# NW-JEFF/Geometric-Message-Passing

Hardware: AMD Instinct MI355X
Metric: edges/sec forward+backward, EGNN & MACE L=2, 1M-edge radius graph, 1/2/4/8 GPU (higher is better)
Workload: dtype f32

## Files before the change

### geometric-message-passing_amd/csrc/gmp_egnn.hip

```cpp
#include <mutex>
#include <set>
#include <tuple>

#include "gmp_egnn_common.h"

namespace gmp {
namespace {

template <int D, int ACT, bool MSG_MEAN, bool SAVE, bool HF, bool POSB>
__global__ __launch_bounds__(fwd_waves<HF>() * 64, fwd_waves<HF>() / 4) void egnn_fwd_kernel(
    int64_t n_nodes, int64_t n_edges, const float* __restrict__ AB, const float* __restrict__ pos,
    const int64_t* __restrict__ rowptr, const int64_t* __restrict__ recv,
    const int64_t* __restrict__ send, gmp_egnn_params P, float eps, int64_t n_waves,
    float* __restrict__ m_aggr, float* __restrict__ pos_aggr, float* __restrict__ xsave,
    float* __restrict__ rsave, int save_planes) {
  constexpr int T = Cfg<D>::T, LDW = Cfg<D>::LDW;
  extern __shared__ __attribute__((aligned(16))) float smem[];
  const float* sW2 = smem;
  const float* sW3 = smem + D * LDW;
  _Float16* hW = reinterpret_cast<_Float16*>(smem + smem_mats_off<D, fwd_waves<HF>(), HF>());
  const _Float16* hW2 = hW;
  const _Float16* hW3 = hW + HCfg<D>::MAT;
  float* sVw = smem + smem_vec_off<D, fwd_waves<HF>(), HF>();
  const float* sV = sVw;
// ... 57 lines not shown
        gemm_h2s<D, false>(hW3, ex3, m, x, li, g);
        r3 = ln_rms<D>(x, eps, ex3 + sw3);
      } else {
        load_vec<D>(x, sV, V_B3, g);
        gemm_wx<D>(sW3, m, x, li, g);
        r3 = ln_normalize<D, false>(x, eps);
      }
      if (SAVE) {
        if (save_planes == 3)
          store_row_w<D, kAuxNT>(rows_window(xsave + 2 * ED, base, ne, D), eoff, x, g);
        store3_w<kAuxNT>(rows_window(rsave, base, ne, 3), (g == 0 && c.valid) ? li * 12u : kOob,
                         r1, r2, r3);
      }
      affine_act<D, ACT>(x, sV, V_LN3W, V_LN3B, g);
      float sp = 0.f;
#pragma unroll
      for (int p = 0; p < T; ++p) {
        const f32x4 w = vec4<D>(sV, V_W4, p, g);
        sp += w[0] * x[p][0] + w[1] * x[p][1] + w[2] * x[p][2] + w[3] * x[p][3];
      }
      s_e = sum_groups(sp) + b4;
    } else if (SAVE) {
      store2_w<kAuxNT>(rows_window(rsave, base, ne, 3), (g == 0 && c.valid) ? li * 12u : kOob, r1,
                       r2);
    }

    const int head = c.valid ? (int)((c.seg0 > base) ? (c.seg0 - base) : 0) : li;
    const bool is_end = c.valid && (c.e == c.seg1 - 1);
    const bool take = (li == 0) && c.valid && (c.i == carry_node);
    float pv[3] = {c.rx * s_e, c.ry * s_e, c.rz * s_e};
    carry_apply<D, POSB>(cbuf, m, pv, take);
    seg_scan<T>(m, li, head);
    if constexpr (POSB) {
      f32x4 pw[1] = {{pv[0], pv[1], pv[2], 0.f}};
      seg_scan<1>(pw, li, head);
      pv[0] = pw[0][0]; pv[1] = pw[0][1]; pv[2] = pw[0][2];
    }
    {
      const float deg = (float)(c.seg1 - c.seg0);
      const float rdeg = HF ? __builtin_amdgcn_rcpf(deg) : 1.f / deg;
      if (MSG_MEAN) {
        const float sc = is_end ? rdeg : 1.f;
#pragma unroll
        for (int p = 0; p < T; ++p) m[p] *= sc;
      }
      const int nn = max(i1 - i0 + 1, 0);
      store_row_w<D, 0>(rows_window(m_aggr, i0, nn, D), is_end ? (unsigned)((c.i - i0) * D * 4) : kOob,
                        m, g);
      if constexpr (POSB)
        store3_w<0>(rows_window(pos_aggr, i0, nn, 3),
                    (is_end && g == 0) ? (unsigned)((c.i - i0) * 12) : kOob,
                    HF ? pv[0] * rdeg : pv[0] / deg, HF ? pv[1] * rdeg : pv[1] / deg,
                    HF ? pv[2] * rdeg : pv[2] / deg);
    }
    if (li == 15) carry_store<D, POSB>(cbuf, m, pv);
    carry_node = __builtin_amdgcn_readlane(c.i, 15);
  }
}

template <int D>
__device__ __forceinline__ void fold_max(unsigned* word, const f32x4 (&x)[D / 16], int lane) {
  float v = 0.f;
#pragma unroll
  for (int p = 0; p < D / 16; ++p)
    v = fmaxf(v, fmaxf(fmaxf(fabsf(x[p][0]), fabsf(x[p][1])), fmaxf(fabsf(x[p][2]), fabsf(x[p][3]))));
  v = fmaxf(v, dpp<0x128>(v));
  v = fmaxf(v, dpp<0x124>(v));
  v = fmaxf(v, dpp<0x122>(v));
  v = fmaxf(v, dpp<0x121>(v));
  v = max_groups(v);
  if (lane == 0) atomicMax(word, __float_as_uint(v));
}

constexpr int NVG = 8;
enum GradVec { G_LN1W = 0, G_LN1B, G_LN2W, G_LN2B, G_LN3W, G_LN3B, G_W4, G_W1D };

template <int D>
__device__ __forceinline__ float slot(const f32x4 (&x)[D / 16], int s) { return x[s >> 2][s & 3]; }
template <int D>
__device__ __forceinline__ float vslot(const float* sV, int v, int s, int g) {
  return sV[v * D + featq(s, g)];
}

template <int D, int ACT, bool MSG_MEAN, bool HF, bool AMAX, int RC, bool POSB, bool GPOS>
__global__ __launch_bounds__(kBwdWaves * 64, 2) void egnn_bwd_kernel(
    int64_t n_nodes, int64_t n_edges, const float* __restrict__ pos,
    const int64_t* __restrict__ rowptr, const int64_t* __restrict__ recv,
    const int64_t* __restrict__ send, gmp_egnn_params P, int64_t n_waves,
    const float* __restrict__ xsave, const float* __restrict__ rsave,
    const float* __restrict__ g_maggr, const float* __restrict__ g_paggr, float* __restrict__ dA,
    float* __restrict__ dpos_recv, float* __restrict__ dpre1_out, float* __restrict__ gdiff_out,
    float* __restrict__ dpre2_out, float* __restrict__ dpre3_out, float* __restrict__ partials,
    unsigned* __restrict__ amax) {
  constexpr int T = Cfg<D>::T, LDW = Cfg<D>::LDW, K = VecAcc<D>::K;
  extern __shared__ __attribute__((aligned(16))) float smem[];
  const float* sW2t = smem;
  const float* sW3t = smem + D * LDW;
  _Float16* hW = reinterpret_cast<_Float16*>(smem + smem_mats_off<D, kBwdWaves, HF>());
  const _Float16* hW2t = hW;
  const _Float16* hW3t = hW + HCfg<D>::MAT;
  float* sVw = smem + smem_vec_off<D, kBwdWaves, HF>();
  const float* sV = sVw;
  constexpr int NMAT = POSB ? 2 : 1;
  if constexpr (HF)
    load_params_hf<D, true, POSB ? 2 : 0, ACT, NMAT>(sVw, hW, smem + smem_carry_off<D, kBwdWaves, HF>(), P);
  else load_params_to_lds<D, true, NMAT>(smem, P);
  __syncthreads();
  const int sw2 = HF ? (int)sV[NV * D] : 0, sw3 = HF ? (int)sV[NV * D + 1] : 0;
  const int ex3 = HF ? (int)sV[NV * D + 3] : 0;
  (void)sW3t; (void)hW3t; (void)sw3; (void)ex3;
  const float* xr1 = xsave;
  const float* xr2 = xsave + (size_t)n_edges * D;
  unsigned* lmx = reinterpret_cast<unsigned*>(const_cast<float*>(sV) + NV * D + 10);
  if (AMAX) {
    if (threadIdx.x < 2) lmx[threadIdx.x] = 0u;
    __syncthreads();
  }

  const int lane = threadIdx.x & 63, li = lane & 15, g = lane >> 4;
  const int wid = __builtin_amdgcn_readfirstlane(threadIdx.x >> 6);
  float* cbuf = smem + smem_carry_off<D, kBwdWaves, HF>() + (wid * 4 + g) * carry_stride<D>();
  carry_clear<D>(smem + smem_carry_off<D, kBwdWaves, HF>() + wid * 4 * carry_stride<D>(), lane);
  const WaveRange wr = wave_range(rowptr, n_nodes, n_edges, n_waves, wid, kBwdWaves);
  zero_isolated<D, GPOS>(wr, rowptr, dA, dpos_recv, lane);
  const float b4 = POSB ? P.b4[0] : 0.f;
  const size_t ED = (size_t)n_edges * D;

  float vacc[NVG][K];
#pragma unroll
  for (int v = 0; v < NVG; ++v)
#pragma unroll
    for (int k = 0; k < K; ++k) vacc[v][k] = 0.f;
  float db4 = 0.f;
  int carry_node = -1;
  EdgeIJ nxt = load_ij(wr.e_lo, li, wr.e_hi, recv, send);
  asm volatile("" ::"v"(nxt.i), "v"(nxt.j));

  for (int base = wr.e_lo; base < wr.e_hi; base += 16) {
    asm volatile("" ::: "memory");
    const EdgeIJ cur = nxt;
    nxt = load_ij(base + 16, li, wr.e_hi, recv, send);
    EdgeCtx c = edge_ctx(cur, base, li, wr.e_hi, (int)n_nodes, rowptr, pos);
    const float rs1 = rsave[3 * (size_t)c.ec + 0];
    const float rs2 = rsave[3 * (size_t)c.ec + 1];
    float rs3 = 0.f, gp0 = 0.f, gp1 = 0.f, gp2 = 0.f;
    f32x4 x[T], xh2[T], z[T];
    if constexpr (POSB) {
      rs3 = rsave[3 * (size_t)c.ec + 2];
      gp0 = g_paggr[3 * c.i + 0], gp1 = g_paggr[3 * c.i + 1], gp2 = g_paggr[3 * c.i + 2];
      if constexpr (RC == 1) load_row<D>(x, rowp(xsave + ED, c.ec, D), g);
      else load_row<D>(z, rowp(xsave + 2 * ED, c.ec, D), g);
    } else {
      load_row<D>(xh2, rowp(g_maggr, c.i, D), g);
    }
    __builtin_amdgcn_sched_barrier(0);
    edge_geom<HF, true>(c);
    const float rstd1 = c.valid ? rs1 : 0.f;
    const float rstd2 = c.valid ? rs2 : 0.f;
    const float rstd3 = c.valid ? rs3 : 0.f;
    if constexpr (POSB && RC == 1) {
      if constexpr (HF) {
        affine_act<D, ACT>(x, sV, V_LN2W, V_LN2B, g);
        load_vec<D>(z, sV, V_B3S, g);
        gemm_h2s_tr<D, false>(hW3t, ex3, x, z, lane, g);
        const float r = ldexpf(rs3, -(ex3 + sw3));
#pragma unroll
        for (int p = 0; p < T; ++p) z[p] *= r;
      } else {
        affine_act<D, ACT>(x, sV, V_LN2W, V_LN2B, g);
        load_vec<D>(z, sV, V_B3, g);
        gemm_wtx<D>(sW3t, x, z, li, g);
        ln_recenter<D>(z, rs3);
      }
    }

    const float inv_deg = c.valid ? 1.f / (float)(c.seg1 - c.seg0) : 0.f;
    const float gscale = MSG_MEAN ? inv_deg : (c.valid ? 1.f : 0.f);
    const float gpx = gp0 * inv_deg;
    const float gpy = gp1 * inv_deg;
    const float gpz = gp2 * inv_deg;
    auto chunk_window = [&](int& ne, int& i0, int& i1, unsigned& eoff) {
      ne = __builtin_amdgcn_readfirstlane(min(16, wr.e_hi - base));
      i0 = __builtin_amdgcn_readfirstlane(c.i);
      i1 = __builtin_amdgcn_readlane(c.i, 15);
      eoff = c.valid ? (unsigned)(li * D * 4) : kOob;
    };
    int ne, i0, i1;
    unsigned eoff;
    float s_e = 0.f;
    if constexpr (!POSB) {
      chunk_window(ne, i0, i1, eoff);
    } else {
      const float ds = gpx * c.rx + gpy * c.ry + gpz * c.rz;
      if (g == 0) db4 += ds;

      float sp = 0.f;
#pragma unroll
      for (int p = 0; p < T; ++p) {
        const f32x4 w3 = vec4<D>(sV, V_LN3W, p, g), b3 = vec4<D>(sV, V_LN3B, p, g);
        const f32x4 w4 = vec4<D>(sV, V_W4, p, g);
#pragma unroll
        for (int q = 0; q < 4; ++q) {
          const float zz = z[p][q] * w3[q] + b3[q];
          sp += w4[q] * act_f<ACT>(zz);
          x[p][q] = ds * w4[q] * act_df<ACT>(zz);
        }
      }
// ... 12 lines not shown
      chunk_window(ne, i0, i1, eoff);
      store_row_w<D, kAuxNT>(rows_window(dpre3_out, base, ne, D), eoff, x, g);
    }

#pragma unroll
    for (int p = 0; p < T; ++p) z[p] = xh2[p] * gscale;
    load_row<D>(xh2, rowp(xr2, c.ec, D), g);
    if constexpr (POSB) {
      if constexpr (HF) gemm_h2<D, true>(hW3t, sw3, 0, x, z, li, g);
      else gemm_wx<D, 2>(sW3t, x, z, li, g);
    }
#pragma unroll
    for (int p = 0; p < T; ++p) {
      const f32x4 w = vec4<D>(sV, V_LN2W, p, g), b = vec4<D>(sV, V_LN2B, p, g);
#pragma unroll
      for (int q = 0; q < 4; ++q) z[p][q] *= act_df<ACT>(xh2[p][q] * w[q] + b[q]);
    }
    accumulate_vec<D>([&](int s) { return slot<D>(z, s) * slot<D>(xh2, s); }, vacc[G_LN2W], li);
    accumulate_vec<D>([&](int s) { return slot<D>(z, s); }, vacc[G_LN2B], li);
#pragma unroll
    for (int p = 0; p < T; ++p) z[p] *= vec4<D>(sV, V_LN2W, p, g);
    ln_backward<D>(z, xh2, rstd2);
    if (AMAX) fold_max<D>(lmx, z, lane);
    store_row_w<D, kAuxNT>(rows_window(dpre2_out, base, ne, D), eoff, z, g);

    load_row<D>(xh2, rowp(xr1, c.ec, D), g);
#pragma unroll
    for (int p = 0; p < T; ++p) x[p] = f32x4{0.f, 0.f, 0.f, 0.f};
    if constexpr (HF) gemm_h2<D, true>(hW2t, sw2, 0, z, x, li, g);
    else gemm_wx<D, 2>(sW2t, z, x, li, g);
#pragma unroll
    for (int p = 0; p < T; ++p) {
      const f32x4 w = vec4<D>(sV, V_LN1W, p, g), b = vec4<D>(sV, V_LN1B, p, g);
#pragma unroll
      for (int q = 0; q < 4; ++q) x[p][q] *= act_df<ACT>(xh2[p][q] * w[q] + b[q]);
    }
    accumulate_vec<D>([&](int s) { return slot<D>(x, s) * slot<D>(xh2, s); }, vacc[G_LN1W], li);
    accumulate_vec<D>([&](int s) { return slot<D>(x, s); }, vacc[G_LN1B], li);
#pragma unroll
    for (int p = 0; p < T; ++p) x[p] *= vec4<D>(sV, V_LN1W, p, g);
    ln_backward<D>(x, xh2, rstd1);
    store_row_w<D, kAuxNT>(rows_window(dpre1_out, base, ne, D), eoff, x, g);

    const float dist = c.dist;
    float gd[3] = {0.f, 0.f, 0.f};
    if constexpr (GPOS) {
      float dd = 0.f;
#pragma unroll
      for (int p = 0; p < T; ++p) {
        const f32x4 w = vec4<D>(sV, V_W1D, p, g);
        dd += w[0] * x[p][0] + w[1] * x[p][1] + w[2] * x[p][2] + w[3] * x[p][3];
      }
      dd = sum_groups(dd);
      accumulate_vec<D>([&](int s) { return slot<D>(x, s) * dist; }, vacc[G_W1D], li);

      const float rinv = (c.dist > 0.f) ? dd / c.dist : 0.f;
      if constexpr (POSB) {
        gd[0] = gpx * s_e + rinv * c.rx;
        gd[1] = gpy * s_e + rinv * c.ry;
        gd[2] = gpz * s_e + rinv * c.rz;
      } else {
        gd[0] = rinv * c.rx;
        gd[1] = rinv * c.ry;
        gd[2] = rinv * c.rz;
      }
      store3_w<kAuxNT>(rows_window(gdiff_out, base, ne, 3), (c.valid && g == 0) ? li * 12u : kOob,
                       gd[0], gd[1], gd[2]);
    } else {
      accumulate_vec<D>([&](int s) { return slot<D>(x, s) * dist; }, vacc[G_W1D], li);
    }

    const int head = c.valid ? (int)((c.seg0 > base) ? (c.seg0 - base) : 0) : li;
    const bool is_end = c.valid && (c.e == c.seg1 - 1);
    const bool take = (li == 0) && c.valid && (c.i == carry_node);
    carry_apply<D, GPOS>(cbuf, x, gd, take);
    seg_scan<T>(x, li, head);
    if constexpr (GPOS) {
      f32x4 pw[1] = {{gd[0], gd[1], gd[2], 0.f}};
      seg_scan<1>(pw, li, head);
      gd[0] = pw[0][0]; gd[1] = pw[0][1]; gd[2] = pw[0][2];
    }
    {
      const int nn = max(i1 - i0 + 1, 0);
      store_row_w<D, 0>(rows_window(dA, i0, nn, D), is_end ? (unsigned)((c.i - i0) * D * 4) : kOob,
                        x, g);
      if constexpr (GPOS)
        store3_w<0>(rows_window(dpos_recv, i0, nn, 3),
                    (is_end && g == 0) ? (unsigned)((c.i - i0) * 12) : kOob, gd[0], gd[1], gd[2]);
    }
    if (li == 15) carry_store<D, GPOS>(cbuf, x, gd);
    carry_node = __builtin_amdgcn_readlane(c.i, 15);
  }

  __syncthreads();
  if (AMAX && threadIdx.x == 0 && ((POSB && GPOS) || amax)) {
    atomicMax(&amax[0], lmx[0]);
    if (POSB) atomicMax(&amax[1], lmx[1]);
  }
  __syncthreads();
  float* red = smem;
  constexpr int RW = NVG * D + 1;
  for (int t = lane; t < RW; t += 64) red[wid * RW + t] = 0.f;
  __syncthreads();
  if (acc_owner<D>(li)) {
#pragma unroll
    for (int v = 0; v < NVG; ++v)
#pragma unroll
      for (int k = 0; k < K; ++k) red[wid * RW + v * D + featq(acc_slot<D>(li, k), g)] = vacc[v][k];
  }
  float t4 = db4;
#pragma unroll
  for (int off = 32; off >= 1; off >>= 1) t4 += __shfl_xor(t4, off);
  if (lane == 0) red[wid * RW + NVG * D] = t4;
  __syncthreads();
  for (int t = threadIdx.x; t < RW; t += blockDim.x) {
    float sacc = 0.f;
    for (int w = 0; w < kBwdWaves; ++w) sacc += red[w * RW + t];
    partials[(int64_t)blockIdx.x * RW + t] = sacc;
  }
}

int64_t n_waves_for(int64_t n_edges, int nwb) {
  int64_t w = ceil_div(n_edges, 128);
  const int64_t cap = (int64_t)device_cu_count() * nwb;
  if (w > cap) w = cap;
  if (w < 1) w = 1;
  return ceil_div(w, nwb) * nwb;
}

template <int D, int ACT, bool MEAN, bool POSB>
int launch_fwd(int64_t N, int64_t E, const float* AB, const float* pos, const int64_t* rowptr,
               const int64_t* recv, const int64_t* send, const gmp_egnn_params& P, float eps,
               float* m_aggr, float* pos_aggr, float* xsave, int save_planes, float* rsave,
               hipStream_t s) {
  const bool hf = !egnn_f32();
  const int nwb = hf ? fwd_waves<true>() : fwd_waves<false>();
  const int64_t W = n_waves_for(E, nwb);
  constexpr int NMAT = POSB ? 2 : 1;
  const size_t smem = hf ? smem_total<D, fwd_waves<true>(), true, NMAT>()
                         : smem_total<D, fwd_waves<false>(), false, NMAT>();
  auto k = rsave ? (hf ? egnn_fwd_kernel<D, ACT, MEAN, true, true, POSB>
                       : egnn_fwd_kernel<D, ACT, MEAN, true, false, POSB>)
                 : (hf ? egnn_fwd_kernel<D, ACT, MEAN, false, true, POSB>
                       : egnn_fwd_kernel<D, ACT, MEAN, false, false, POSB>);
  int rc = prep_kernel(k, smem);
  if (rc) return rc;
  k<<<(unsigned)(W / nwb), nwb * 64, smem, s>>>(N, E, AB, pos, rowptr, recv, send, P,
                                                           eps, W, m_aggr, pos_aggr, xsave, rsave,
                                                           save_planes);
  return launch_status();
}

template <int D, int ACT, bool MEAN, bool POSB, bool GPOS>
int launch_bwd(int64_t N, int64_t E, const float* pos, const int64_t* rowptr,
               const int64_t* recv, const int64_t* send, const gmp_egnn_params& P,
               const float* xsave, int save_planes, const float* rsave, const float* gm,
               const float* gp, float* dA, float* dpos_recv, float* dpre1, float* gdiff,
               float* dpre2, float* dpre3, float* partials, unsigned* amax, hipStream_t s) {
  const int64_t W = n_waves_for(E, kBwdWaves);
  const bool hf = !egnn_f32();
  constexpr int NMAT = POSB ? 2 : 1;
  constexpr bool FULL = POSB && GPOS;
  constexpr int RC0 = POSB ? 0 : 1;
  const size_t smem = hf ? smem_total<D, kBwdWaves, true, NMAT>()
                         : smem_total<D, kBwdWaves, false, NMAT>();
  const bool ax = !FULL || amax;
#define LAUNCH_BWD_K(RC)                                                              \
  (hf ? (ax ? egnn_bwd_kernel<D, ACT, MEAN, true, true, RC, POSB, GPOS>              \
            : egnn_bwd_kernel<D, ACT, MEAN, true, !FULL, RC, POSB, GPOS>)            \
      : (ax ? egnn_bwd_kernel<D, ACT, MEAN, false, true, RC, POSB, GPOS>             \
            : egnn_bwd_kernel<D, ACT, MEAN, false, !FULL, RC, POSB, GPOS>))
  auto k = save_planes == 3 ? LAUNCH_BWD_K(RC0) : LAUNCH_BWD_K(1);
#undef LAUNCH_BWD_K
  int rc = prep_kernel(k, smem);
  if (rc) return rc;
  k<<<(unsigned)(W / kBwdWaves), kBwdWaves * 64, smem, s>>>(N, E, pos, rowptr, recv, send, P, W,
                                                           xsave, rsave, gm, gp, dA, dpos_recv,
                                                           dpre1, gdiff, dpre2, dpre3, partials,
                                                           amax);
  return launch_status();
}

bool params_ok(const gmp_egnn_params* P) {
  return P && P->w1d && P->b1 && P->ln1_w && P->ln1_b && P->W2 && P->b2 && P->ln2_w &&
         P->ln2_b && P->W3 && P->b3 && P->ln3_w && P->ln3_b && P->w4 && P->b4;
}

}

int prep_kernel_once(const void* k, size_t smem) {
  static std::mutex mu;
  static std::set<std::tuple<int, const void*, size_t>> done;
  int dev = 0;
  if (hipGetDevice(&dev) != hipSuccess) return GMP_ERR_HIP;
  std::lock_guard<std::mutex> lk(mu);
  if (done.count({dev, k, smem})) return GMP_OK;
  const int rc = hip_check(hipFuncSetAttribute(k, hipFuncAttributeMaxDynamicSharedMemorySize,
                                               (int)smem));
  if (!rc) done.insert({dev, k, smem});
  return rc;
}

int g_egnn_f32 = 0;

bool egnn_f32() { return g_egnn_f32 == 1; }

}

using namespace gmp;

#define LAUNCH_EGNN_DISPATCH(CALL)                                                                \
  do {                                                                                         \
    if (d == 128) {                                                                            \
      if (act == 0) { if (msg_mean) CALL(128, 0, true); else CALL(128, 0, false); }            \
      else          { if (msg_mean) CALL(128, 1, true); else CALL(128, 1, false); }            \
    } else if (d == 64) {                                                                      \
      if (act == 0) { if (msg_mean) CALL(64, 0, true); else CALL(64, 0, false); }              \
      else          { if (msg_mean) CALL(64, 1, true); else CALL(64, 1, false); }              \
    } else {                                                                                   \
      if (act == 0) { if (msg_mean) CALL(32, 0, true); else CALL(32, 0, false); }              \
      else          { if (msg_mean) CALL(32, 1, true); else CALL(32, 1, false); }              \
    }                                                                                          \
  } while (0)

extern "C" {

int gmp_egnn_set_f32_mfma(int on) {
  const int prev = egnn_f32() ? 1 : 0;
  g_egnn_f32 = on ? 1 : 0;
  return prev;
}

int gmp_egnn_edge_fwd_ex_f32(int64_t n_nodes, int64_t n_edges, int64_t d, const float* AB,
                             const float* pos, const int64_t* rowptr, const int64_t* recv,
                             const int64_t* send, const gmp_egnn_params* params, int act,
                             int msg_mean, float ln_eps, float* m_aggr, float* pos_aggr,
                             float* save_xhat, int save_planes, float* save_rstd, uint32_t flags,
                             void* stream) {
  if (!(d == 32 || d == 64 || d == 128)) return GMP_ERR_UNSUPPORTED;
  GMP_CHECK_ARG((flags & ~(uint32_t)GMP_EGNN_NO_POS_BRANCH) == 0);
  const bool posb = !(flags & GMP_EGNN_NO_POS_BRANCH);
  GMP_CHECK_ARG(n_nodes >= 0 && n_edges >= 0 && (act == 0 || act == 1));
  GMP_CHECK_ARG(n_nodes < INT32_MAX && n_edges < INT32_MAX);
  GMP_CHECK_ARG(params_ok(params) && m_aggr && (pos_aggr || !posb) && rowptr);
  GMP_CHECK_ARG((save_rstd == nullptr) == (save_xhat == nullptr));
  GMP_CHECK_ARG(save_xhat == nullptr || save_planes == 2 || save_planes == 3);
  hipStream_t s = as_stream(stream);
  if (n_nodes == 0) return GMP_OK;
  int rc = GMP_OK;
  if (n_edges == 0) {
    rc = hip_check(hipMemsetAsync(m_aggr, 0, n_nodes * d * sizeof(float), s));
    if (!rc && posb) rc = hip_check(hipMemsetAsync(pos_aggr, 0, n_nodes * 3 * sizeof(float), s));
    return rc;
  }
  GMP_CHECK_ARG(AB && pos && recv && send && aligned16(AB) && aligned16(m_aggr));
  GMP_CHECK_ARG(aligned16(params->W2) && aligned16(params->W3));
  GMP_CHECK_ARG(save_xhat == nullptr || aligned16(save_xhat));
#define LAUNCH_CALL_FWD(DD, AA, MM)                                                              \
  rc = posb ? launch_fwd<DD, AA, MM, true>(n_nodes, n_edges, AB, pos, rowptr, recv, send,      \
                                           *params, ln_eps, m_aggr, pos_aggr, save_xhat,        \
                                           save_planes, save_rstd, s)                           \
            : launch_fwd<DD, AA, MM, false>(n_nodes, n_edges, AB, pos, rowptr, recv, send,     \
                                            *params, ln_eps, m_aggr, pos_aggr, save_xhat,       \
                                            save_planes, save_rstd, s)
  LAUNCH_EGNN_DISPATCH(LAUNCH_CALL_FWD);
#undef LAUNCH_CALL_FWD
  return rc;
}

int gmp_egnn_edge_fwd_f32(int64_t n_nodes, int64_t n_edges, int64_t d, const float* AB,
                          const float* pos, const int64_t* rowptr, const int64_t* recv,
                          const int64_t* send, const gmp_egnn_params* params, int act,
                          int msg_mean, float ln_eps, float* m_aggr, float* pos_aggr,
                          float* save_xhat, int save_planes, float* save_rstd, void* stream) {
  return gmp_egnn_edge_fwd_ex_f32(n_nodes, n_edges, d, AB, pos, rowptr, recv, send, params, act,
                                  msg_mean, ln_eps, m_aggr, pos_aggr, save_xhat, save_planes,
                                  save_rstd, 0u, stream);
}

int64_t gmp_egnn_edge_bwd_partials_rows(int64_t n_edges, int64_t d) {
  (void)d;
  return n_waves_for(n_edges, kBwdWaves) / kBwdWaves;
}

int gmp_egnn_edge_bwd_ex_f32(int64_t n_nodes, int64_t n_edges, int64_t d, const float* pos,
                             const int64_t* rowptr, const int64_t* recv, const int64_t* send,
                             const gmp_egnn_params* params, int act, int msg_mean,
                             const float* save_xhat, int save_planes, const float* save_rstd,
                             const float* g_m_aggr, const float* g_pos_aggr, float* dA,
                             float* dpos_recv, float* dpre1, float* gdiff, float* dpre2,
                             float* dpre3, float* vec_partials, uint32_t* amax, uint32_t flags,
                             void* stream) {
  if (!(d == 32 || d == 64 || d == 128)) return GMP_ERR_UNSUPPORTED;
  GMP_CHECK_ARG((flags & ~(uint32_t)(GMP_EGNN_NO_POS_BRANCH | GMP_EGNN_NO_POS_GRAD)) == 0);
  const bool posb = !(flags & GMP_EGNN_NO_POS_BRANCH), gpos = !(flags & GMP_EGNN_NO_POS_GRAD);
  GMP_CHECK_ARG(n_nodes >= 0 && n_edges >= 0 && (act == 0 || act == 1));
  GMP_CHECK_ARG(n_nodes < INT32_MAX && n_edges < INT32_MAX);
  GMP_CHECK_ARG(params_ok(params) && dA && (dpos_recv || !gpos) && rowptr && vec_partials);
  GMP_CHECK_ARG(save_planes == 2 || save_planes == 3);
  hipStream_t s = as_stream(stream);
  int rc = GMP_OK;
  if (n_nodes > 0 && n_edges == 0) {
    rc = hip_check(hipMemsetAsync(dA, 0, n_nodes * d * sizeof(float), s));
    if (!rc && gpos) rc = hip_check(hipMemsetAsync(dpos_recv, 0, n_nodes * 3 * sizeof(float), s));
  }
  if (rc) return rc;
  if (n_edges == 0 || n_nodes == 0) {
    return hip_check(hipMemsetAsync(
        vec_partials, 0,
        gmp_egnn_edge_bwd_partials_rows(n_edges, d) * (8 * d + 1) * sizeof(float), s));
  }
  GMP_CHECK_ARG(pos && recv && send && save_xhat && save_rstd && g_m_aggr && dpre1 && dpre2);
  GMP_CHECK_ARG(!posb || (g_pos_aggr && dpre3));
  GMP_CHECK_ARG(!gpos || gdiff);
  GMP_CHECK_ARG(aligned16(save_xhat) && aligned16(dA) && aligned16(g_m_aggr) &&
                aligned16(dpre1) && aligned16(dpre2) && (!posb || aligned16(dpre3)));
  GMP_CHECK_ARG(aligned16(params->W2) && aligned16(params->W3));
#define LAUNCH_BWD_V(DD, AA, MM, PB, GP)                                                        \
  launch_bwd<DD, AA, MM, PB, GP>(n_nodes, n_edges, pos, rowptr, recv, send, *params, save_xhat, \
                                 save_planes, save_rstd, g_m_aggr, g_pos_aggr, dA, dpos_recv,   \
                                 dpre1, gdiff, dpre2, dpre3, vec_partials, amax, s)
#define LAUNCH_CALL_BWD(DD, AA, MM)                                                              \
  rc = posb ? (gpos ? LAUNCH_BWD_V(DD, AA, MM, true, true) : LAUNCH_BWD_V(DD, AA, MM, true, false)) \
            : (gpos ? LAUNCH_BWD_V(DD, AA, MM, false, true)                                     \
                    : LAUNCH_BWD_V(DD, AA, MM, false, false))
  LAUNCH_EGNN_DISPATCH(LAUNCH_CALL_BWD);
#undef LAUNCH_CALL_BWD
#undef LAUNCH_BWD_V
  return rc;
}

int gmp_egnn_edge_bwd_amax_f32(int64_t n_nodes, int64_t n_edges, int64_t d, const float* pos,
                               const int64_t* rowptr, const int64_t* recv, const int64_t* send,
                               const gmp_egnn_params* params, int act, int msg_mean,
                               const float* save_xhat, int save_planes, const float* save_rstd,
                               const float* g_m_aggr, const float* g_pos_aggr, float* dA,
                               float* dpos_recv, float* dpre1, float* gdiff, float* dpre2,
                               float* dpre3, float* vec_partials, uint32_t* amax, void* stream) {
  return gmp_egnn_edge_bwd_ex_f32(n_nodes, n_edges, d, pos, rowptr, recv, send, params, act,
                                  msg_mean, save_xhat, save_planes, save_rstd, g_m_aggr,
                                  g_pos_aggr, dA, dpos_recv, dpre1, gdiff, dpre2, dpre3,
                                  vec_partials, amax, 0u, stream);
}

int gmp_egnn_edge_bwd_f32(int64_t n_nodes, int64_t n_edges, int64_t d, const float* pos,
                          const int64_t* rowptr, const int64_t* recv, const int64_t* send,
                          const gmp_egnn_params* params, int act, int msg_mean,
                          const float* save_xhat, int save_planes, const float* save_rstd,
                          const float* g_m_aggr, const float* g_pos_aggr, float* dA,
                          float* dpos_recv, float* dpre1, float* gdiff, float* dpre2, float* dpre3,
                          float* vec_partials, void* stream) {
  return gmp_egnn_edge_bwd_amax_f32(n_nodes, n_edges, d, pos, rowptr, recv, send, params, act,
                                    msg_mean, save_xhat, save_planes, save_rstd, g_m_aggr,
                                    g_pos_aggr, dA, dpos_recv, dpre1, gdiff, dpre2, dpre3,
                                    vec_partials, nullptr, stream);
}

}
```

### geometric-message-passing_amd/csrc/gmp_egnn_common.h

```cpp
#pragma once
#include <stdlib.h>

#include "gmp_common.h"

namespace gmp {

typedef float f32x4 __attribute__((ext_vector_type(4)));

constexpr int kFwdWaves = 12;
template <bool HF>
constexpr int fwd_waves() { return kFwdWaves; }
constexpr int kBwdWaves = 8;

template <int D>
struct Cfg {
  static constexpr int T = D / 16;
  static constexpr int N = D / 4;
  static constexpr int LDW = D + 4;
};

__device__ __forceinline__ constexpr int featq(int s, int g) { return 16 * (s >> 2) + 4 * g + (s & 3); }

enum VecId {
  V_W1D = 0, V_B1, V_LN1W, V_LN1B, V_B2, V_LN2W, V_LN2B, V_B3, V_LN3W, V_LN3B, V_W4, NVB,
// ... 119 lines not shown
  if (threadIdx.x >= 2 * D + 64 && threadIdx.x < 2 * D + 128) {
    unsigned a = 0u, b = 0u, c = 0u, e = 0u;
    for (int k = threadIdx.x - 2 * D - 64; k < D; k += 64) {
      a = max(a, __float_as_uint(fabsf(P.ln1_w[k])));
      b = max(b, __float_as_uint(fabsf(P.ln1_b[k])));
      c = max(c, __float_as_uint(fabsf(P.ln2_w[k])));
      e = max(e, __float_as_uint(fabsf(P.ln2_b[k])));
    }
    atomicMax(&mxw[2], a);
    atomicMax(&mxw[3], b);
    atomicMax(&mxw[4], c);
    atomicMax(&mxw[5], e);
  }
  __syncthreads();
  const int s2 = scale_exp(__uint_as_float(mxw[0])), s3 = scale_exp(__uint_as_float(mxw[1]));
  const float rd = sqrtf((float)D);
  const int ex2 = clamp_in_exp(scale_exp(rd * __uint_as_float(mxw[2]) + __uint_as_float(mxw[3])), s2);
  const int ex3 = clamp_in_exp(scale_exp(rd * __uint_as_float(mxw[4]) + __uint_as_float(mxw[5])), s3);
  __syncthreads();
#pragma unroll 8
  for (int i = threadIdx.x; i < NMAT * D * D; i += blockDim.x) {
    const int mat = i / (D * D), e = i - mat * D * D;
    const int o = e / D, k = e - o * D;
    const float w = ldexpf((mat ? P.W3 : P.W2)[e] - scratch[mat * D + k], mat ? s3 : s2);
    const int r = TRANSPOSE ? k : o, c = TRANSPOSE ? o : k;
    const _Float16 hi = (_Float16)w;
    _Float16* dst = hW + mat * H::MAT + r * H::LDH + hf_pos(c);
    dst[0] = hi;
    dst[H::PLANE] = (_Float16)(w - (float)hi);
  }
  const float* vsrc[NVB] = {P.w1d, P.b1, P.ln1_w, P.ln1_b, P.b2, P.ln2_w,
                            P.ln2_b, P.b3, P.ln3_w, P.ln3_b, P.w4};
  for (int i = threadIdx.x; i < NVB * D; i += blockDim.x) sV[i] = vsrc[i / D][i % D];
  for (int k = threadIdx.x; k < D; k += blockDim.x) {
    sV[V_B2S * D + k] = ldexpf(P.b2[k] - scratch[2 * D], ex2 + s2);
    sV[V_B3S * D + k] = ldexpf(P.b3[k] - scratch[2 * D + 1], ex3 + s3);
    const int e1 = ACT == GMP_ACT_RELU ? ex2 : 0;
    sV[V_LN1WS * D + k] = ldexpf(P.ln1_w[k], e1);
    sV[V_LN1BS * D + k] = ldexpf(P.ln1_b[k], e1);
  }
  if (threadIdx.x == 0) {
    sV[NV * D + 0] = (float)s2;
    sV[NV * D + 1] = (float)s3;
    sV[NV * D + 2] = (float)ex2;
    sV[NV * D + 3] = (float)ex3;
  }
}

template <int D>
__device__ __forceinline__ f32x4 vec4(const float* sV, int v, int p, int g) {
  return *reinterpret_cast<const f32x4*>(sV + v * D + 16 * p + 4 * g);
}

template <int D>
__device__ __forceinline__ void load_vec(f32x4 (&x)[D / 16], const float* sV, int v, int g) {
#pragma unroll
  for (int p = 0; p < D / 16; ++p) x[p] = vec4<D>(sV, v, p, g);
}

template <int D>
__device__ __forceinline__ void load_row(f32x4 (&x)[D / 16], const float* __restrict__ row, int g) {
#pragma unroll
  for (int p = 0; p < D / 16; ++p) x[p] = *reinterpret_cast<const f32x4*>(row + 16 * p + 4 * g);
}
template <int D>
__device__ __forceinline__ void store_row(float* __restrict__ row, const f32x4 (&x)[D / 16], int g) {
#pragma unroll
  for (int p = 0; p < D / 16; ++p) *reinterpret_cast<f32x4*>(row + 16 * p + 4 * g) = x[p];
}
template <int D>
__device__ __forceinline__ void stream_row(float* __restrict__ row, const f32x4 (&x)[D / 16], int g) {
#pragma unroll
  for (int p = 0; p < D / 16; ++p)
    __builtin_nontemporal_store(x[p], reinterpret_cast<f32x4*>(row + 16 * p + 4 * g));
}

typedef __amdgpu_buffer_rsrc_t rsrc_t;
constexpr unsigned kOob = 0x40000000u;
constexpr int kAuxNT = 2;

__device__ __forceinline__ rsrc_t rows_window(const float* base, int r0, int n, int ld) {
  return __builtin_amdgcn_make_buffer_rsrc(const_cast<float*>(base) + (size_t)(unsigned)r0 * ld, 0,
                                           n * ld * 4, 0x00020000);
}
template <int D, int AUX>
__device__ __forceinline__ void store_row_w(rsrc_t w, unsigned off, const f32x4 (&x)[D / 16], int g) {
#pragma unroll
  for (int p = 0; p < D / 16; ++p)
    __builtin_amdgcn_raw_buffer_store_b128(__builtin_bit_cast(__attribute__((ext_vector_type(4))) unsigned, x[p]),
                                           w, off + (16 * p + 4 * g) * 4, 0, AUX);
}
template <int AUX>
__device__ __forceinline__ void store2_w(rsrc_t w, unsigned off, float a, float b) {
  __builtin_amdgcn_raw_buffer_store_b32(__float_as_uint(a), w, off, 0, AUX);
  __builtin_amdgcn_raw_buffer_store_b32(__float_as_uint(b), w, off + 4, 0, AUX);
}
template <int AUX>
__device__ __forceinline__ void store3_w(rsrc_t w, unsigned off, float a, float b, float c) {
  __builtin_amdgcn_raw_buffer_store_b32(__float_as_uint(a), w, off, 0, AUX);
  __builtin_amdgcn_raw_buffer_store_b32(__float_as_uint(b), w, off + 4, 0, AUX);
  __builtin_amdgcn_raw_buffer_store_b32(__float_as_uint(c), w, off + 8, 0, AUX);
}

__device__ __forceinline__ void gemm_fence() { __builtin_amdgcn_sched_barrier(0); }
template <int D, int SPLIT = 1>
__device__ __forceinline__ void gemm_wx(const float* __restrict__ sW, const f32x4 (&x)[D / 16],
                                        f32x4 (&y)[D / 16], int i, int g) {
  constexpr int T = Cfg<D>::T, LDW = Cfg<D>::LDW;
  constexpr int TS = (T % SPLIT == 0) ? T / SPLIT : T;
#pragma unroll
  for (int p = 0; p < T; ++p) {
#pragma unroll
    for (int t0 = 0; t0 < T; t0 += TS) {
      f32x4 a[TS];
#pragma unroll
      for (int t = 0; t < TS; ++t)
        a[t] = *reinterpret_cast<const f32x4*>(sW + (16 * (t0 + t) + i) * LDW + 16 * p + 4 * g);
#pragma unroll
      for (int c = 0; c < 4; ++c)
#pragma unroll
        for (int t = 0; t < TS; ++t)
          y[t0 + t] = __builtin_amdgcn_mfma_f32_16x16x4f32(a[t][c], x[p][c], y[t0 + t], 0, 0, 0);
      gemm_fence();
    }
  }
}

typedef _Float16 h16x8 __attribute__((ext_vector_type(8)));
typedef _Float16 h16x2 __attribute__((ext_vector_type(2)));
typedef unsigned u32x4 __attribute__((ext_vector_type(4)));
constexpr int kTilesPerFence = 2;

__device__ __forceinline__ void split8(const f32x4& a, const f32x4& b, h16x8& bh, h16x8& bl) {
  const h16x2 p0 = {(_Float16)a[0], (_Float16)a[1]}, p1 = {(_Float16)a[2], (_Float16)a[3]};
  const h16x2 p2 = {(_Float16)b[0], (_Float16)b[1]}, p3 = {(_Float16)b[2], (_Float16)b[3]};
  const unsigned u0 = __builtin_bit_cast(unsigned, p0), u1 = __builtin_bit_cast(unsigned, p1);
  const unsigned u2 = __builtin_bit_cast(unsigned, p2), u3 = __builtin_bit_cast(unsigned, p3);
  unsigned l0, l1, l2, l3;
  const float one = 1.0f;
  asm("v_fma_mixlo_f16 %0, %4, %16, -%12 op_sel_hi:[0,0,1]\n\t"
      "v_fma_mixhi_f16 %0, %5, %16, -%12 op_sel:[0,0,1] op_sel_hi:[0,0,1]\n\t"
      "v_fma_mixlo_f16 %1, %6, %16, -%13 op_sel_hi:[0,0,1]\n\t"
      "v_fma_mixhi_f16 %1, %7, %16, -%13 op_sel:[0,0,1] op_sel_hi:[0,0,1]\n\t"
      "v_fma_mixlo_f16 %2, %8, %16, -%14 op_sel_hi:[0,0,1]\n\t"
      "v_fma_mixhi_f16 %2, %9, %16, -%14 op_sel:[0,0,1] op_sel_hi:[0,0,1]\n\t"
      "v_fma_mixlo_f16 %3, %10, %16, -%15 op_sel_hi:[0,0,1]\n\t"
      "v_fma_mixhi_f16 %3, %11, %16, -%15 op_sel:[0,0,1] op_sel_hi:[0,0,1]\n\t"
      "s_nop 1"
      : "=&v"(l0), "=&v"(l1), "=&v"(l2), "=&v"(l3)
      : "v"(a[0]), "v"(a[1]), "v"(a[2]), "v"(a[3]), "v"(b[0]), "v"(b[1]), "v"(b[2]), "v"(b[3]),
        "v"(u0), "v"(u1), "v"(u2), "v"(u3), "s"(one));
  bh = __builtin_bit_cast(h16x8, (u32x4){u0, u1, u2, u3});
  bl = __builtin_bit_cast(h16x8, (u32x4){l0, l1, l2, l3});
}

__device__ __forceinline__ float max_groups(float v) {
  const auto a = __builtin_amdgcn_permlane16_swap(__float_as_uint(v), __float_as_uint(v), false,
                                                  false);
  v = fmaxf(__uint_as_float(a[0]), __uint_as_float(a[1]));
  const auto b = __builtin_amdgcn_permlane32_swap(__float_as_uint(v), __float_as_uint(v), false,
                                                  false);
  return fmaxf(__uint_as_float(b[0]), __uint_as_float(b[1]));
}

template <int D, bool DYN>
__device__ __forceinline__ void gemm_h2(const _Float16* __restrict__ hW, int sw, int sx_static,
// ... 363 lines not shown
  r.i = reinterpret_cast<const int*>(recv)[2 * ec];
  r.j = reinterpret_cast<const int*>(send)[2 * ec];
  return r;
}

__device__ __forceinline__ EdgeCtx edge_ctx(EdgeIJ ij, int base, int lane_e, int e_hi,
                                            int n_nodes, const int64_t* __restrict__ rowptr,
                                            const float* __restrict__ pos) {
  EdgeCtx c;
  c.e = base + lane_e;
  c.ec = clamp_edge(c.e, e_hi);
  c.valid = c.e < e_hi;
  c.i = ((unsigned)ij.i < (unsigned)n_nodes) ? ij.i : 0;
  c.j = ((unsigned)ij.j < (unsigned)n_nodes) ? ij.j : c.i;
  const int* rp = reinterpret_cast<const int*>(rowptr);
  c.seg0 = rp[2 * c.i];
  c.seg1 = rp[2 * c.i + 2];
  c.rx = pos[3 * c.i + 0];
  c.ry = pos[3 * c.i + 1];
  c.rz = pos[3 * c.i + 2];
  c.dist = 0.f;
  c.pjx = pos[3 * c.j + 0];
  c.pjy = pos[3 * c.j + 1];
  c.pjz = pos[3 * c.j + 2];
  return c;
}
template <bool FAST = false, bool BWD = false>
__device__ __forceinline__ void edge_geom(EdgeCtx& c) {
#pragma clang fp contract(off)
  c.rx -= c.pjx;
  c.ry -= c.pjy;
  c.rz -= c.pjz;
  const float xx = c.rx * c.rx, yy = c.ry * c.ry, zz = c.rz * c.rz;
  const float q = BWD ? __builtin_fmaf(c.ry, c.ry, xx) + zz : __builtin_fmaf(c.rz, c.rz, xx + yy);
  c.dist = FAST ? __builtin_amdgcn_sqrtf(q) : sqrtf(q);
}

template <int D, bool FAST, class Ctx>
__device__ __forceinline__ void load_pre1(f32x4 (&x)[D / 16], const float* arow, const float* brow,
                                          const float* sV, Ctx& c, int g) {
  f32x4 b[D / 16];
#pragma unroll
  for (int p = 0; p < D / 16; ++p) {
    x[p] = *reinterpret_cast<const f32x4*>(arow + 16 * p + 4 * g);
    b[p] = *reinterpret_cast<const f32x4*>(brow + 16 * p + 4 * g);
  }
  __builtin_amdgcn_sched_barrier(0);
  edge_geom<FAST>(c);
  const float dist = c.dist;
#pragma unroll
  for (int p = 0; p < D / 16; ++p)
    x[p] = (x[p] + b[p]) + (vec4<D>(sV, V_W1D, p, g) * dist + vec4<D>(sV, V_B1, p, g));
}

__device__ __forceinline__ const float* rowp(const float* base, int r, int ld) {
  return base + (size_t)(unsigned)r * (size_t)ld;
}
__device__ __forceinline__ float* rowp(float* base, int r, int ld) {
  return base + (size_t)(unsigned)r * (size_t)ld;
}

struct WaveRange {
  int e_lo, e_hi, n_lo, n_hi;
};
__device__ __forceinline__ WaveRange wave_range(const int64_t* __restrict__ rowptr, int64_t n_nodes,
                                                int64_t n_edges, int64_t n_waves, int wid,
                                                int nwb) {
  const int64_t wave = (int64_t)blockIdx.x * nwb + wid;
  const int64_t nb = node_begin(rowptr, n_nodes, n_edges, wave, n_waves);
  const int64_t ne = node_begin(rowptr, n_nodes, n_edges, wave + 1, n_waves);
  WaveRange r;
  r.e_lo = (nb < ne) ? (int)rowptr[nb] : 0;
  r.e_hi = (nb < ne) ? (int)rowptr[ne] : 0;
  r.e_lo = __builtin_amdgcn_readfirstlane(r.e_lo);
  r.e_hi = __builtin_amdgcn_readfirstlane(r.e_hi);
  r.n_lo = __builtin_amdgcn_readfirstlane((int)nb);
  r.n_hi = __builtin_amdgcn_readfirstlane((int)ne);
  return r;
}

template <int D, bool R3 = true>
__device__ __forceinline__ void zero_isolated(const WaveRange& wr, const int64_t* __restrict__ rowptr,
                                              float* __restrict__ rows, float* __restrict__ rows3,
                                              int lane) {
  const int* rp = reinterpret_cast<const int*>(rowptr);
  for (int n = wr.n_lo + lane; n < wr.n_hi; n += 64) {
    if (rp[2 * n] == rp[2 * n + 2]) {
      float4* r = reinterpret_cast<float4*>(rows + (size_t)n * D);
#pragma unroll
      for (int k = 0; k < D / 4; ++k) r[k] = float4{0.f, 0.f, 0.f, 0.f};
      if (R3) {
        rows3[3 * (size_t)n] = 0.f;
        rows3[3 * (size_t)n + 1] = 0.f;
        rows3[3 * (size_t)n + 2] = 0.f;
      }
    }
  }
}


bool egnn_f32();

int prep_kernel_once(const void* k, size_t smem);
template <class K>
inline int prep_kernel(K k, size_t smem) {
  return prep_kernel_once((const void*)k, smem);
}

inline bool aligned16(const void* p) { return reinterpret_cast<uintptr_t>(p) % 16 == 0; }

}
```

### geometric-message-passing_amd/csrc/gmp_index.hip

```cpp
#include <hipcub/hipcub.hpp>

#include <map>
#include <mutex>
#include <utility>

#include "gmp_common.h"

namespace gmp {

thread_local int g_last_hip_error = 0;

int device_cu_count() {
  static int cus = 0;
  if (cus == 0) {
    int dev = 0;
    hipDeviceProp_t prop;
    if (hipGetDevice(&dev) == hipSuccess && hipGetDeviceProperties(&prop, dev) == hipSuccess)
      cus = prop.multiProcessorCount;
    if (cus <= 0) cus = 256;
  }
  return cus;
}

namespace {

constexpr size_t kAlign = 256;
inline size_t align_up(size_t x) { return (x + kAlign - 1) / kAlign * kAlign; }

int key_bits(int64_t n_seg) {
  int b = 1;
  while ((int64_t(1) << b) <= n_seg) ++b;
  return b;
}

size_t cub_sort_bytes(int64_t n) {
  size_t bytes = 0;
  (void)hipcub::DeviceRadixSort::SortPairs(nullptr, bytes, (const uint32_t*)nullptr, (uint32_t*)nullptr,
                                     (const uint32_t*)nullptr, (uint32_t*)nullptr, (int)n, 0, 32,
                                     (hipStream_t)0);
  return bytes;
}

__global__ void csr_prepare_keys(const int64_t* __restrict__ index, int64_t n, int64_t n_seg,
                                 uint32_t* __restrict__ keys, uint32_t* __restrict__ vals,
                                 int32_t* __restrict__ err_flag) {
  for (int64_t i = blockIdx.x * (int64_t)blockDim.x + threadIdx.x; i < n;
       i += (int64_t)gridDim.x * blockDim.x) {
    int64_t k = index[i];
    bool ok = (k >= 0) && (k < n_seg);
    if (!ok && err_flag) *err_flag = 1;
    keys[i] = ok ? (uint32_t)k : (uint32_t)n_seg;
    vals[i] = (uint32_t)i;
  }
}

__global__ void csr_finish(const uint32_t* __restrict__ keys_sorted,
                           const uint32_t* __restrict__ vals_sorted, int64_t n, int64_t n_seg,
                           const int64_t* __restrict__ payload, int64_t* __restrict__ perm,
                           int64_t* __restrict__ rowptr, int64_t* __restrict__ index_sorted,
                           int64_t* __restrict__ payload_out) {
  for (int64_t k = blockIdx.x * (int64_t)blockDim.x + threadIdx.x; k <= n;
       k += (int64_t)gridDim.x * blockDim.x) {
    int64_t prev = (k == 0) ? -1 : (int64_t)keys_sorted[k - 1];
    int64_t cur = (k == n) ? n_seg : (int64_t)keys_sorted[k];
    for (int64_t s = prev + 1; s <= cur && s <= n_seg; ++s) rowptr[s] = k;
    if (k < n) {
      int64_t p = vals_sorted[k];
      if (perm) perm[k] = p;
      if (index_sorted) index_sorted[k] = (cur < n_seg) ? cur : -1;
      if (payload_out) payload_out[k] = payload[p];
    }
  }
}

template <int VEC>
__global__ void gather_rows_kernel(const float* __restrict__ src, int64_t n_rows, int64_t F,
                                   const int64_t* __restrict__ index, int64_t n_index,
                                   float* __restrict__ out, int32_t* __restrict__ err_flag) {
  const int64_t fv = F / VEC;
  const int64_t total = n_index * fv;
  for (int64_t t = blockIdx.x * (int64_t)blockDim.x + threadIdx.x; t < total;
       t += (int64_t)gridDim.x * blockDim.x) {
    int64_t e = t / fv, c = t - e * fv;
    int64_t r = index[e];
    if constexpr (VEC == 4) {
      float4 v = make_float4(0.f, 0.f, 0.f, 0.f);
      if (r >= 0 && r < n_rows) v = reinterpret_cast<const float4*>(src + r * F)[c];
      else if (err_flag) *err_flag = 1;
      reinterpret_cast<float4*>(out + e * F)[c] = v;
    } else {
      float v = 0.f;
      if (r >= 0 && r < n_rows) v = src[r * F + c];
      else if (err_flag) *err_flag = 1;
      out[e * F + c] = v;
    }
  }
}

struct RedVal {
  float v;
  int64_t arg;
};

template <int REDUCE>
__device__ __forceinline__ void red_combine(float& acc, int64_t& arg, float x, int64_t xa) {
  if (REDUCE == GMP_REDUCE_MAX) {
    if (x > acc || (x == acc && xa < arg)) { acc = x; arg = xa; }
  } else {
    acc += x;
  }
}

template <int VEC, int REDUCE>
__device__ __forceinline__ void wave_reduce_rows(const float* __restrict__ src, int64_t F,
                                                 const int64_t* __restrict__ perm, int64_t k_beg,
                                                 int64_t k_end, int64_t n_items, int64_t c,
                                                 int lpr, float (&acc)[VEC], int64_t (&arg)[VEC]) {
  const int lane = threadIdx.x & 63;
  const int R = 64 / lpr, sub = lane / lpr;
#pragma unroll
  for (int v = 0; v < VEC; ++v) {
    acc[v] = (REDUCE == GMP_REDUCE_MAX) ? -INFINITY : 0.f;
    arg[v] = n_items;
  }
  const bool active = c < F / VEC;
  int64_t k = k_beg + sub;
  for (; k + 3 * R < k_end; k += 4 * R) {
    int64_t it[4];
    float x[4][VEC];
#pragma unroll
    for (int u = 0; u < 4; ++u) it[u] = perm ? perm[k + u * R] : (k + u * R);
#pragma unroll
    for (int u = 0; u < 4; ++u) {
      const float* p = src + it[u] * F + c * VEC;
      if (!active) {
#pragma unroll
        for (int v = 0; v < VEC; ++v) x[u][v] = 0.f;
      } else if constexpr (VEC == 4) {
        float4 q = *reinterpret_cast<const float4*>(p);
        x[u][0] = q.x; x[u][1] = q.y; x[u][2] = q.z; x[u][3] = q.w;
      } else if constexpr (VEC == 2) {
        float2 q = *reinterpret_cast<const float2*>(p);
        x[u][0] = q.x; x[u][1] = q.y;
      } else {
        x[u][0] = p[0];
      }
    }
#pragma unroll
    for (int u = 0; u < 4; ++u)
#pragma unroll
      for (int v = 0; v < VEC; ++v) red_combine<REDUCE>(acc[v], arg[v], x[u][v], it[u]);
  }
  for (; k < k_end; k += R) {
    const int64_t i = perm ? perm[k] : k;
    if (active) {
      const float* p = src + i * F + c * VEC;
#pragma unroll
      for (int v = 0; v < VEC; ++v) red_combine<REDUCE>(acc[v], arg[v], p[v], i);
    }
  }
  for (int m = lpr; m < 64; m <<= 1) {
#pragma unroll
    for (int v = 0; v < VEC; ++v) {
      const float ox = __shfl_xor(acc[v], m);
      const int64_t oa = __shfl_xor(arg[v], m);
      if (REDUCE == GMP_REDUCE_MAX) {
        if (ox > acc[v] || (ox == acc[v] && oa < arg[v])) { acc[v] = ox; arg[v] = oa; }
      } else {
        const bool upper = (lane & m) != 0;
        acc[v] = upper ? ox + acc[v] : acc[v] + ox;
      }
    }
  }
}

__device__ __forceinline__ int lanes_per_row(int64_t cpr) {
  int l = 1;
  while (l < cpr && l < 64) l <<= 1;
  return l;
}

template <int VEC, int REDUCE>
__global__ __launch_bounds__(256) void segment_reduce_wave(
    const float* __restrict__ src, int64_t n_items, int64_t F, const int64_t* __restrict__ perm,
    const int64_t* __restrict__ rowptr, int64_t n_seg, float* __restrict__ out,
    int64_t* __restrict__ argmax) {
  const int lane = threadIdx.x & 63;
  const int64_t seg = blockIdx.x * (int64_t)(blockDim.x / 64) + (threadIdx.x >> 6);
  if (seg >= n_seg) return;
  const int64_t k0 = rowptr[seg], k1 = rowptr[seg + 1];
  const int64_t cpr = F / VEC;
  const int lpr = lanes_per_row(cpr);
  for (int64_t cb = 0; cb < cpr; cb += 64) {
    const int64_t c = cb + lane % lpr;
    float acc[VEC];
    int64_t arg[VEC];
    wave_reduce_rows<VEC, REDUCE>(src, F, perm, k0, k1, n_items, c, lpr, acc, arg);
    const int64_t cnt = k1 - k0;
    if (lane < lpr && c < cpr) {
#pragma unroll
      for (int v = 0; v < VEC; ++v) {
        float r = acc[v];
        if (REDUCE == GMP_REDUCE_MEAN) r = r / (float)(cnt > 0 ? cnt : 1);
        if (REDUCE == GMP_REDUCE_MAX && cnt == 0) r = 0.f;
        out[seg * F + c * VEC + v] = r;
        if (REDUCE == GMP_REDUCE_MAX && argmax) argmax[seg * F + c * VEC + v] = arg[v];
      }
    }
  }
}

template <int VEC, int REDUCE>
__global__ __launch_bounds__(256) void segment_reduce_split(
    const float* __restrict__ src, int64_t n_items, int64_t F, const int64_t* __restrict__ perm,
    const int64_t* __restrict__ rowptr, int64_t n_seg, int64_t S, float* __restrict__ partial) {
  __shared__ float red[4][256];
  const int lane = threadIdx.x & 63, w = threadIdx.x >> 6;
  const int64_t seg = blockIdx.x / S, part = blockIdx.x % S;
  const int64_t k0 = rowptr[seg], k1 = rowptr[seg + 1], len = k1 - k0;
  const int64_t pb = k0 + len * part / S, pe = k0 + len * (part + 1) / S;
  const int64_t wb = pb + (pe - pb) * w / 4, we = pb + (pe - pb) * (w + 1) / 4;
  const int64_t cpr = F / VEC;
  const int lpr = lanes_per_row(cpr);
  for (int64_t cb = 0; cb < cpr; cb += 64) {
    const int64_t c = cb + lane % lpr;
    float acc[VEC];
    int64_t arg[VEC];
    wave_reduce_rows<VEC, REDUCE>(src, F, perm, wb, we, n_items, c, lpr, acc, arg);
    if (lane < lpr) {
#pragma unroll
      for (int v = 0; v < VEC; ++v) red[w][lane * VEC + v] = acc[v];
    }
    __syncthreads();
    if (w == 0 && lane < lpr && c < cpr) {
#pragma unroll
      for (int v = 0; v < VEC; ++v) {
        const float t = ((red[0][lane * VEC + v] + red[1][lane * VEC + v]) + red[2][lane * VEC + v]) +
                        red[3][lane * VEC + v];
        partial[(seg * S + part) * F + c * VEC + v] = t;
      }
    }
    __syncthreads();
  }
}

template <int REDUCE>
__global__ void segment_split_finish(const float* __restrict__ partial, const int64_t* __restrict__ rowptr,
                                     int64_t n_seg, int64_t S, int64_t F, float* __restrict__ out) {
  for (int64_t t = blockIdx.x * (int64_t)blockDim.x + threadIdx.x; t < n_seg * F;
       t += (int64_t)gridDim.x * blockDim.x) {
    const int64_t seg = t / F, f = t - seg * F;
    float s = 0.f;
    for (int64_t p = 0; p < S; ++p) s += partial[(seg * S + p) * F + f];
    if (REDUCE == GMP_REDUCE_MEAN) {
      const int64_t cnt = rowptr[seg + 1] - rowptr[seg];
      s = s / (float)(cnt > 0 ? cnt : 1);
    }
    out[t] = s;
  }
}

template <int REDUCE>
// ... 83 lines not shown

using namespace gmp;

extern "C" {

int gmp_abi_version(void) { return GMP_ABI_VERSION; }

const char* gmp_error_string(int code) {
  switch (code) {
    case GMP_OK: return "ok";
    case GMP_ERR_ARG: return "invalid argument";
    case GMP_ERR_HIP: return "HIP runtime error";
    case GMP_ERR_UNSUPPORTED: return "unsupported shape for this kernel";
    case GMP_ERR_WORKSPACE: return "workspace too small";
    default: return "unknown error";
  }
}

int gmp_last_hip_error(void) { return g_last_hip_error; }

size_t gmp_csr_workspace_size(int64_t n_items, int64_t n_seg) {
  (void)n_seg;
  if (n_items <= 0) return kAlign;
  size_t n = (size_t)n_items;
  return 4 * align_up(n * sizeof(uint32_t)) + align_up(cub_sort_bytes(n_items)) + kAlign;
}

int gmp_csr_build(const int64_t* index, int64_t n_items, int64_t n_seg, const int64_t* payload,
                  int64_t* perm, int64_t* rowptr, int64_t* index_sorted, int64_t* payload_out,
                  int32_t* err_flag, void* workspace, size_t workspace_bytes, void* stream) {
  GMP_CHECK_ARG(n_items >= 0 && n_seg >= 0 && rowptr != nullptr);
  GMP_CHECK_ARG(n_items < (int64_t(1) << 31) && n_seg < (int64_t(1) << 31) - 1);
  GMP_CHECK_ARG(n_items == 0 || index != nullptr);
  GMP_CHECK_ARG(payload_out == nullptr || payload != nullptr);
  hipStream_t s = as_stream(stream);
  if (n_items == 0) {
    int rc = hip_check(hipMemsetAsync(rowptr, 0, (n_seg + 1) * sizeof(int64_t), s));
    return rc;
  }
  if (workspace_bytes < gmp_csr_workspace_size(n_items, n_seg) || workspace == nullptr)
    return GMP_ERR_WORKSPACE;
  char* ws = reinterpret_cast<char*>(
      (reinterpret_cast<uintptr_t>(workspace) + kAlign - 1) / kAlign * kAlign);
  size_t nb = align_up((size_t)n_items * sizeof(uint32_t));
  uint32_t* keys_in = reinterpret_cast<uint32_t*>(ws);
  uint32_t* keys_out = reinterpret_cast<uint32_t*>(ws + nb);
  uint32_t* vals_in = reinterpret_cast<uint32_t*>(ws + 2 * nb);
  uint32_t* vals_out = reinterpret_cast<uint32_t*>(ws + 3 * nb);
  void* temp = ws + 4 * nb;
  size_t temp_bytes = cub_sort_bytes(n_items);

  csr_prepare_keys<<<grid_for(n_items, 256), 256, 0, s>>>(index, n_items, n_seg, keys_in, vals_in,
                                                          err_flag);
  int rc = launch_status();
  if (rc) return rc;
  rc = hip_check(hipcub::DeviceRadixSort::SortPairs(temp, temp_bytes, keys_in, keys_out, vals_in,
                                                    vals_out, (int)n_items, 0, key_bits(n_seg), s));
  if (rc) return rc;
  csr_finish<<<grid_for(n_items + 1, 256), 256, 0, s>>>(keys_out, vals_out, n_items, n_seg,
                                                        payload, perm, rowptr, index_sorted,
                                                        payload_out);
  return launch_status();
}

int gmp_gather_rows_f32(const float* src, int64_t n_rows, int64_t F, const int64_t* index,
                        int64_t n_index, float* out, int32_t* err_flag, void* stream) {
  GMP_CHECK_ARG(n_rows >= 0 && F >= 0 && n_index >= 0);
  if (n_index == 0 || F == 0) return GMP_OK;
  GMP_CHECK_ARG(src && index && out);
  hipStream_t s = as_stream(stream);
  bool v4 = (F % 4 == 0) && (reinterpret_cast<uintptr_t>(src) % 16 == 0) &&
            (reinterpret_cast<uintptr_t>(out) % 16 == 0);
  if (v4) {
    gather_rows_kernel<4><<<grid_for(n_index * F / 4, 256), 256, 0, s>>>(src, n_rows, F, index,
                                                                         n_index, out, err_flag);
  } else {
    gather_rows_kernel<1><<<grid_for(n_index * F, 256), 256, 0, s>>>(src, n_rows, F, index,
                                                                     n_index, out, err_flag);
  }
  return launch_status();
}

static int64_t split_parts(int64_t n_items, int64_t n_seg, int reduce) {
  if (reduce == GMP_REDUCE_MAX || n_seg <= 0) return 1;
  const int64_t avg = n_items / n_seg;
  int64_t S = avg < 2048 ? 1 : ceil_div(avg, 1024);
  if (n_seg < 2048 && n_items >= 16384)
    S = std::max<int64_t>(S, std::min<int64_t>(ceil_div(2048, n_seg), 64));
  return S > 4096 ? 4096 : S;
}

size_t gmp_segment_reduce_workspace_size(int64_t n_items, int64_t n_seg, int64_t F, int reduce) {
  const int64_t S = split_parts(n_items, n_seg, reduce);
  return S > 1 ? (size_t)(n_seg * S * F) * sizeof(float) : 0;
}

int gmp_segment_reduce_f32(const float* src, int64_t n_items, int64_t F, const int64_t* perm,
                           const int64_t* rowptr, int64_t n_seg, int reduce, float* out,
                           int64_t* argmax, void* workspace, size_t workspace_bytes,
                           void* stream) {
  GMP_CHECK_ARG(n_items >= 0 && F >= 0 && n_seg >= 0);
  GMP_CHECK_ARG(reduce == GMP_REDUCE_SUM || reduce == GMP_REDUCE_MEAN || reduce == GMP_REDUCE_MAX);
  if (n_seg == 0 || F == 0) return GMP_OK;
  GMP_CHECK_ARG(rowptr && out && (n_items == 0 || src));
  hipStream_t s = as_stream(stream);
  const bool a16 = (reinterpret_cast<uintptr_t>(src) % 16 == 0);
  const bool a8 = (reinterpret_cast<uintptr_t>(src) % 8 == 0);
  const int vec = (F % 4 == 0 && a16) ? 4 : (F % 2 == 0 && a8) ? 2 : 1;
  const int64_t S = split_parts(n_items, n_seg, reduce);
  if (S > 1 && workspace && workspace_bytes >= gmp_segment_reduce_workspace_size(n_items, n_seg, F, reduce)) {
    float* part = reinterpret_cast<float*>(workspace);
    const unsigned g = (unsigned)(n_seg * S);
#define LAUNCH_SPLIT(V, RED) segment_reduce_split<V, RED><<<g, 256, 0, s>>>(src, n_items, F, perm, rowptr, n_seg, S, part)
    if (reduce == GMP_REDUCE_SUM) {
      if (vec == 4) LAUNCH_SPLIT(4, GMP_REDUCE_SUM); else if (vec == 2) LAUNCH_SPLIT(2, GMP_REDUCE_SUM); else LAUNCH_SPLIT(1, GMP_REDUCE_SUM);
    } else {
      if (vec == 4) LAUNCH_SPLIT(4, GMP_REDUCE_MEAN); else if (vec == 2) LAUNCH_SPLIT(2, GMP_REDUCE_MEAN); else LAUNCH_SPLIT(1, GMP_REDUCE_MEAN);
    }
#undef LAUNCH_SPLIT
    int rc = launch_status();
    if (rc) return rc;
    if (reduce == GMP_REDUCE_SUM)
      segment_split_finish<GMP_REDUCE_SUM><<<grid_for(n_seg * F, 256), 256, 0, s>>>(part, rowptr, n_seg, S, F, out);
    else
      segment_split_finish<GMP_REDUCE_MEAN><<<grid_for(n_seg * F, 256), 256, 0, s>>>(part, rowptr, n_seg, S, F, out);
    return launch_status();
  }
#define LAUNCH_SEG_LAUNCH(VEC, RED)                                                            \
  segment_reduce_wave<VEC, RED><<<(unsigned)ceil_div(n_seg, 4), 256, 0, s>>>(              \
      src, n_items, F, perm, rowptr, n_seg, out, argmax)
#define LAUNCH_SEG_DISPATCH(RED)                                                               \
  do {                                                                                      \
    if (F < 4 && n_items < 64 * n_seg)                                                      \
      segment_reduce_thread<RED><<<grid_for(n_seg * F, 256), 256, 0, s>>>(                 \
          src, n_items, F, perm, rowptr, n_seg, out, argmax);                               \
    else if (vec == 4) LAUNCH_SEG_LAUNCH(4, RED);                                              \
    else if (vec == 2) LAUNCH_SEG_LAUNCH(2, RED);                                              \
    else LAUNCH_SEG_LAUNCH(1, RED);                                                            \
  } while (0)
  if (reduce == GMP_REDUCE_SUM) LAUNCH_SEG_DISPATCH(GMP_REDUCE_SUM);
  else if (reduce == GMP_REDUCE_MEAN) LAUNCH_SEG_DISPATCH(GMP_REDUCE_MEAN);
  else LAUNCH_SEG_DISPATCH(GMP_REDUCE_MAX);
#undef LAUNCH_SEG_DISPATCH
#undef LAUNCH_SEG_LAUNCH
  return launch_status();
}

int gmp_segment_reduce_bwd_f32(const float* grad_out, int64_t n_seg, int64_t F,
                               const int64_t* index, int64_t n_items, const int64_t* rowptr,
                               int reduce, const int64_t* argmax, float* grad_src, void* stream) {
  GMP_CHECK_ARG(n_items >= 0 && F >= 0 && n_seg >= 0);
  GMP_CHECK_ARG(reduce == GMP_REDUCE_SUM || reduce == GMP_REDUCE_MEAN || reduce == GMP_REDUCE_MAX);
  if (n_items == 0 || F == 0) return GMP_OK;
  GMP_CHECK_ARG(grad_out && index && grad_src);
  GMP_CHECK_ARG(reduce != GMP_REDUCE_MEAN || rowptr);
  GMP_CHECK_ARG(reduce != GMP_REDUCE_MAX || argmax);
  hipStream_t s = as_stream(stream);
  const bool vec4 = reduce != GMP_REDUCE_MAX && F % 4 == 0 && n_items * F / 4 < INT32_MAX &&
                    n_seg < INT32_MAX && reinterpret_cast<uintptr_t>(grad_out) % 16 == 0 &&
                    reinterpret_cast<uintptr_t>(grad_src) % 16 == 0;
  if (vec4) {
    const int total = (int)(n_items * F / 4);
    const int gv = grid_for(total, 256);
    auto go = reinterpret_cast<const float4*>(grad_out);
    auto gs = reinterpret_cast<float4*>(grad_src);
    if (reduce == GMP_REDUCE_SUM)
      segment_reduce_bwd_vec4_kernel<GMP_REDUCE_SUM><<<gv, 256, 0, s>>>(go, (int)n_seg, (int)(F / 4),
                                                                        index, total, rowptr, gs);
    else
      segment_reduce_bwd_vec4_kernel<GMP_REDUCE_MEAN><<<gv, 256, 0, s>>>(go, (int)n_seg, (int)(F / 4),
                                                                         index, total, rowptr, gs);
    return launch_status();
  }
  int g = grid_for(n_items * F, 256);
  if (reduce == GMP_REDUCE_SUM)
    segment_reduce_bwd_kernel<GMP_REDUCE_SUM><<<g, 256, 0, s>>>(grad_out, n_seg, F, index, n_items,
                                                                rowptr, argmax, grad_src);
  else if (reduce == GMP_REDUCE_MEAN)
    segment_reduce_bwd_kernel<GMP_REDUCE_MEAN><<<g, 256, 0, s>>>(grad_out, n_seg, F, index,
                                                                 n_items, rowptr, argmax, grad_src);
  else
    segment_reduce_bwd_kernel<GMP_REDUCE_MAX><<<g, 256, 0, s>>>(grad_out, n_seg, F, index, n_items,
                                                                rowptr, argmax, grad_src);
  return launch_status();
}

}
```

### geometric-message-passing_amd/csrc/torch/gmp_torch.cpp

```cpp
#include <ATen/hip/impl/HIPGuardImplMasqueradingAsCUDA.h>
#include <ATen/hip/impl/HIPStreamMasqueradingAsCUDA.h>
#include <ATen/ATen.h>
#include <torch/library.h>

#include <algorithm>
#include <string>
#include <vector>

#include "../../../include/gmp.h"

namespace {

using at::Tensor;
using c10::optional;

thread_local int g_op_device = -1;

struct OpGuard {
  c10::hip::HIPGuardMasqueradingAsCUDA guard;
  int prev;
  static c10::Device dev_of(const Tensor& t, const char* op) {
    TORCH_CHECK(t.defined() && t.is_cuda(), "gmp.", op,
                ": inputs must be HIP device tensors (no CPU fallback)");
    return t.device();
// ... 192 lines not shown
      P[l].W1n = w1->data_ptr<float>();
      P[l].ld1 = w1->stride(0);
    }
  }
  const size_t bytes = gmp_egnn_node_image_bytes(d);
  TORCH_CHECK(bytes > 0, "gmp.egnn_node_image: d must be 32, 64 or 128");
  Tensor img = at::empty({L, (int64_t)bytes}, W0s[0].options().dtype(at::kByte));
  check_rc(gmp_egnn_node_image_f32(d, L, P.data(), img.data_ptr(), cur_stream()),
           "gmp_egnn_node_image_f32");
  return img;
}

std::tuple<Tensor, Tensor, Tensor, Tensor> egnn_node_fwd(
    const Tensor& h, const Tensor& m_aggr, const std::vector<Tensor>& vecs, const Tensor& image,
    bool with_ab, int64_t act, bool residual, double eps, bool train) {
  OpGuard g(h, "egnn_node_fwd");
  f32(h, "h");
  f32(m_aggr, "m_aggr");
  TORCH_CHECK(h.dim() == 2 && m_aggr.sizes() == h.sizes(), "gmp.egnn_node_fwd: h, m_aggr (N, d)");
  const int64_t N = h.size(0), d = h.size(1);
  TORCH_CHECK(vecs.size() == 6, "gmp.egnn_node_fwd: 6 parameter vectors expected");
  for (int k = 0; k < 6; ++k) {
    f32(vecs[k], "egnn_node parameter");
    numel(vecs[k], d, "egnn_node parameter");
  }
  TORCH_CHECK(image.scalar_type() == at::kByte && image.is_contiguous() &&
                  image.numel() == (int64_t)gmp_egnn_node_image_bytes(d) &&
                  image.device() == h.device(),
              "gmp.egnn_node_fwd: image must be one layer's row of egnn_node_image");
  gmp_egnn_node_params P{};
  P.b0 = fp(vecs[0]); P.ln1_w = fp(vecs[1]); P.ln1_b = fp(vecs[2]);
  P.b3 = fp(vecs[3]); P.ln2_w = fp(vecs[4]); P.ln2_b = fp(vecs[5]);
  Tensor ho = at::empty({N, d}, h.options());
  Tensor abo = at::empty({with_ab ? N : 0, 2 * d}, h.options());
  Tensor xh = at::empty({train ? 2 : 0, N, d}, h.options());
  Tensor rs = at::empty({train ? 2 : 0, N}, h.options());
  check_rc(gmp_egnn_node_fwd_f32(N, d, fp(h), fp(m_aggr), &P, image.data_ptr(), (int)act,
                                 residual ? 1 : 0, (float)eps, fp(ho),
                                 with_ab ? fp(abo) : nullptr, train ? fp(xh) : nullptr,
                                 train ? fp(rs) : nullptr, cur_stream()),
           "gmp_egnn_node_fwd_f32");
  return {ho, abo, xh, rs};
}

void egnn_graph_checks(const Tensor& pos, const Tensor& rowptr, const Tensor& recv,
                       const Tensor& send) {
  f32(pos, "pos");
  i64(rowptr, "rowptr");
  i64(recv, "recv");
  i64(send, "send");
  TORCH_CHECK(pos.dim() == 2 && pos.size(1) == 3, "gmp.egnn: pos must be (N, 3)");
  numel(rowptr, pos.size(0) + 1, "rowptr");
  numel(send, recv.numel(), "send");
}

std::tuple<Tensor, Tensor, Tensor, Tensor> egnn_edge_fwd(
    const Tensor& AB, const Tensor& pos, const Tensor& rowptr, const Tensor& recv,
    const Tensor& send, const std::vector<Tensor>& params, int64_t act, bool msg_mean, double eps,
    bool train, int64_t xhat_planes, bool need_pos) {
  OpGuard g(AB, "egnn_edge_fwd");
  TORCH_CHECK(xhat_planes == 2 || xhat_planes == 3, "gmp.egnn_edge_fwd: xhat_planes is 2 or 3");
  f32(AB, "AB");
  egnn_graph_checks(pos, rowptr, recv, send);
  TORCH_CHECK(AB.dim() == 2 && AB.size(1) % 2 == 0 && AB.size(0) == pos.size(0),
              "gmp.egnn_edge_fwd: AB must be (N, 2d)");
  const int64_t N = pos.size(0), E = recv.numel(), d = AB.size(1) / 2;
  gmp_egnn_params P = egnn_params(params, d);
  Tensor m = at::empty({N, d}, fopt(AB)), pa = at::empty({need_pos ? N : 0, 3}, fopt(AB));
  Tensor xh = at::empty({train ? xhat_planes : 0, E, d}, fopt(AB));
  Tensor rs = at::empty({train ? E : 0, 3}, fopt(AB));
  check_rc(gmp_egnn_edge_fwd_ex_f32(N, E, d, fp(AB), fp(pos), ip(rowptr), ip(recv), ip(send), &P,
                                    (int)act, msg_mean, (float)eps, fp(m),
                                    need_pos ? fp(pa) : nullptr, train ? fp(xh) : nullptr,
                                    (int)xhat_planes, train ? fp(rs) : nullptr,
                                    need_pos ? 0u : GMP_EGNN_NO_POS_BRANCH, cur_stream()),
           "gmp_egnn_edge_fwd_ex_f32");
  return {m, pa, xh, rs};
}

std::tuple<Tensor, Tensor, Tensor, Tensor, Tensor, Tensor, Tensor> egnn_edge_bwd(
    const Tensor& pos, const Tensor& rowptr, const Tensor& recv, const Tensor& send,
    const std::vector<Tensor>& params, int64_t act, bool msg_mean, const Tensor& xhat,
    const Tensor& rstd, const Tensor& g_m, const Tensor& g_p, const optional<Tensor>& amax,
    bool pos_branch, bool pos_grad) {
  OpGuard g(pos, "egnn_edge_bwd");
  egnn_graph_checks(pos, rowptr, recv, send);
  f32(xhat, "xhat");
  f32(rstd, "rstd");
  f32(g_m, "g_m_aggr");
  f32(g_p, "g_pos_aggr");
  TORCH_CHECK(xhat.dim() == 3 && (xhat.size(0) == 2 || xhat.size(0) == 3),
              "gmp.egnn_edge_bwd: xhat must be the forward's (2 or 3, E, d) planes");
  const int64_t N = pos.size(0), E = recv.numel(), d = xhat.size(2);
  shape(xhat, {xhat.size(0), E, d}, "xhat");
  shape(rstd, {E, 3}, "rstd");
  shape(g_m, {N, d}, "g_m_aggr");
  if (pos_branch) shape(g_p, {N, 3}, "g_pos_aggr");
  gmp_egnn_params P = egnn_params(params, d);
  if (amax.has_value()) {
    i32(*amax, "amax");
    TORCH_CHECK(amax->numel() >= 2, "gmp.egnn_edge_bwd: amax has 2 words");
  }
  auto o = fopt(pos);
  Tensor dA = at::empty({N, d}, o), dpr = at::empty({pos_grad ? N : 0, 3}, o);
  Tensor dp1 = at::empty({E, d}, o), gd = at::empty({pos_grad ? E : 0, 3}, o);
  Tensor dp2 = at::empty({E, d}, o), dp3 = at::empty({pos_branch ? E : 0, d}, o);
  Tensor part = at::empty({gmp_egnn_edge_bwd_partials_rows(E, d), 8 * d + 1}, o);
  check_rc(gmp_egnn_edge_bwd_ex_f32(
               N, E, d, fp(pos), ip(rowptr), ip(recv), ip(send), &P, (int)act, msg_mean,
               E > 0 ? fp(xhat) : nullptr, (int)xhat.size(0), fp(rstd), fp(g_m),
               pos_branch ? fp(g_p) : nullptr, fp(dA), pos_grad ? fp(dpr) : nullptr, fp(dp1),
               pos_grad ? fp(gd) : nullptr, fp(dp2), pos_branch ? fp(dp3) : nullptr, fp(part),
               amax.has_value() ? reinterpret_cast<uint32_t*>(amax->data_ptr<int32_t>())
                                : nullptr,
               (pos_branch ? 0u : GMP_EGNN_NO_POS_BRANCH) | (pos_grad ? 0u : GMP_EGNN_NO_POS_GRAD),
               cur_stream()),
           "gmp_egnn_edge_bwd_ex_f32");
  return {dA, dpr, dp1, gd, dp2, dp3, part};
}

Tensor cfconv_aggregate(const Tensor& x, const Tensor& xidx, const Tensor& w, const Tensor& perm,
                        const Tensor& rowptr, int64_t n_seg, const optional<Tensor>& escale) {
  OpGuard g(x, "cfconv_aggregate");
  f32(x, "x");
  f32(w, "w");
  i64(xidx, "xidx");
  i64(perm, "perm");
  i64(rowptr, "rowptr");
  TORCH_CHECK(x.dim() == 2 && w.dim() == 2 && w.size(1) == x.size(1),
              "gmp.cfconv_aggregate: x (N, F), w (E, F)");
  const int64_t E = w.size(0);
  numel(xidx, E, "xidx");
  numel(perm, E, "perm");
  numel(rowptr, n_seg + 1, "rowptr");
  opt_f32(escale, {E}, "escale");
  Tensor out = at::empty({n_seg, x.size(1)}, x.options());
  Tensor err = at::zeros({1}, x.options().dtype(at::kInt));
  check_rc(gmp_cfconv_aggregate_scaled_f32(fp(x), x.size(0), ip(xidx), fp(w), cfp(escale), E,
                                           x.size(1), ip(perm), ip(rowptr), n_seg, fp(out),
                                           err.data_ptr<int32_t>(), cur_stream()),
           "gmp_cfconv_aggregate_scaled_f32");
  return out;
}

Tensor cfconv_wgrad(const Tensor& gr, const Tensor& gidx, const Tensor& x, const Tensor& xidx,
                    const optional<Tensor>& escale) {
  OpGuard g(gr, "cfconv_wgrad");
  f32(gr, "g");
  f32(x, "x");
  i64(gidx, "gidx");
  i64(xidx, "xidx");
  TORCH_CHECK(gr.dim() == 2 && x.dim() == 2 && gr.size(1) == x.size(1),
              "gmp.cfconv_wgrad: g (N, F), x (N, F)");
  const int64_t E = gidx.numel();
  numel(xidx, E, "xidx");
  opt_f32(escale, {E}, "escale");
  Tensor dw = at::empty({E, x.size(1)}, x.options());
  Tensor err = at::zeros({1}, x.options().dtype(at::kInt));
  check_rc(gmp_cfconv_wgrad_scaled_f32(fp(gr), gr.size(0), ip(gidx), fp(x), x.size(0), ip(xidx),
                                       cfp(escale), E, x.size(1), fp(dw),
                                       err.data_ptr<int32_t>(), cur_stream()),
           "gmp_cfconv_wgrad_scaled_f32");
  return dw;
}

Tensor ssp_fwd(const Tensor& x, double shift) {
  OpGuard g(x, "ssp_fwd");
  f32(x, "x");
  Tensor y = at::empty_like(x);
  check_rc(gmp_ssp_fwd_f32(fp(x), x.numel(), (float)shift, fp(y), cur_stream()), "gmp_ssp_fwd_f32");
  return y;
}

Tensor ssp_bwd(const Tensor& x, const Tensor& gy) {
  OpGuard g(x, "ssp_bwd");
  f32(x, "x");
  f32(gy, "grad_y");
  shape(gy, x.sizes(), "grad_y");
  Tensor gx = at::empty_like(x);
  check_rc(gmp_ssp_bwd_f32(fp(x), fp(gy), x.numel(), fp(gx), cur_stream()), "gmp_ssp_bwd_f32");
  return gx;
}

std::tuple<Tensor, Tensor> cfconv_cgrad(const Tensor& gr, const Tensor& gidx, const Tensor& x,
                                        const Tensor& xidx, const Tensor& w,
                                        const optional<Tensor>& escale) {
  OpGuard g(gr, "cfconv_cgrad");
  f32(gr, "g");
  f32(x, "x");
  f32(w, "w");
  i64(gidx, "gidx");
  i64(xidx, "xidx");
  TORCH_CHECK(gr.dim() == 2 && x.dim() == 2 && w.dim() == 2 && gr.size(1) == x.size(1) &&
                  w.size(1) == x.size(1),
              "gmp.cfconv_cgrad: g (N, F), x (N, F), w (E, F)");
  const int64_t E = w.size(0);
  numel(gidx, E, "gidx");
  numel(xidx, E, "xidx");
  opt_f32(escale, {E}, "escale");
  Tensor dc = at::empty({E}, x.options());
  Tensor err = at::zeros({1}, x.options().dtype(at::kInt));
// ... 1558 lines not shown
Tensor triplet_interact1_fwd(const Tensor& src, const Tensor& S, const Tensor& w,
                             const Tensor& gidx, const optional<Tensor>& perm,
                             const Tensor& rowptr) {
  OpGuard g(src, "triplet_interact1_fwd");
  interact1_args(S, w);
  const int64_t T = S.size(0), I = w.size(0);
  const int64_t* pp = interact_fwd_args("triplet_interact1_fwd", src, T, I, gidx, perm, rowptr);
  const int64_t n_seg = rowptr.numel() - 1;
  Tensor out = at::empty({n_seg, I}, src.options());
  check_rc(gmp_triplet_interact1_fwd_f32(n_seg, src.size(0), T, I, (int)S.size(1), fp(src), fp(S),
                                         fp(w), ip(gidx), pp, ip(rowptr), fp(out), cur_stream()),
           "gmp_triplet_interact1_fwd_f32");
  return out;
}

std::tuple<Tensor, Tensor> triplet_interact1_bwd(const Tensor& gm, const Tensor& xd,
                                                 const Tensor& S, const Tensor& w,
                                                 const Tensor& idx_kj, const Tensor& offs) {
  OpGuard g(gm, "triplet_interact1_bwd");
  interact1_args(S, w);
  const int64_t T = S.size(0), I = w.size(0), b = S.size(1);
  const int64_t E = interact_bwd_args("triplet_interact1_bwd", gm, xd, T, I, idx_kj, offs);
  TORCH_CHECK(b <= 16, "gmp.triplet_interact1_bwd: basis_emb_size <= 16");
  auto o = gm.options();
  Tensor gS = at::empty({T, b}, o), gw = at::empty({I, b}, o);
  Tensor part = at::empty({gmp_triplet_interact1_bwd_partial_rows(E), I * b}, o);
  check_rc(gmp_triplet_interact1_bwd_f32(E, T, I, (int)b, fp(gm), fp(xd), fp(S), fp(w),
                                         ip(idx_kj), ip(offs), fp(gS), fp(gw), fp(part),
                                         cur_stream()),
           "gmp_triplet_interact1_bwd_f32");
  return {gS, gw};
}

namespace meta {
std::tuple<Tensor, Tensor, Tensor, Tensor, Tensor> csr_build(const Tensor& index, int64_t n_seg,
                                                             const optional<Tensor>& payload) {
  auto o = index.options();
  const int64_t n = index.numel();
  return {at::empty({n}, o), at::empty({n_seg + 1}, o), at::empty({n}, o),
          at::empty({payload.has_value() ? n : 0}, o), at::empty({1}, o.dtype(at::kInt))};
}
Tensor gather_rows(const Tensor& src, const Tensor& index) {
  return at::empty({index.numel(), src.size(1)}, src.options());
}
std::tuple<Tensor, Tensor> segment_reduce(const Tensor& src, const optional<Tensor>&,
                                          const Tensor& rowptr, int64_t n_seg,
                                          const std::string& reduce) {
  const bool mx = reduce_code(reduce) == GMP_REDUCE_MAX;
  return {at::empty({n_seg, src.size(1)}, src.options()),
          at::empty({mx ? n_seg : 0, src.size(1)}, rowptr.options())};
}
Tensor segment_reduce_bwd(const Tensor& grad_out, const Tensor&, const Tensor&, const std::string&,
                          const optional<Tensor>&, int64_t n_items) {
  return at::empty({n_items, grad_out.size(1)}, grad_out.options());
}
std::tuple<Tensor, Tensor, Tensor, Tensor> egnn_edge_fwd(const Tensor& AB, const Tensor& pos,
                                                         const Tensor&, const Tensor& recv,
                                                         const Tensor&, const std::vector<Tensor>&,
                                                         int64_t, bool, double, bool train,
                                                         int64_t xhat_planes, bool need_pos) {
  const int64_t N = pos.size(0), E = recv.numel(), d = AB.size(1) / 2;
  auto o = AB.options();
  return {at::empty({N, d}, o), at::empty({need_pos ? N : 0, 3}, o),
          at::empty({train ? xhat_planes : 0, E, d}, o), at::empty({train ? E : 0, 3}, o)};
}
Tensor egnn_node_image(const std::vector<Tensor>& W0s, const std::vector<Tensor>&,
                       const std::vector<optional<Tensor>>&) {
  const int64_t d = W0s[0].size(0);
  return at::empty({(int64_t)W0s.size(), (int64_t)gmp_egnn_node_image_bytes(d)},
                   W0s[0].options().dtype(at::kByte));
}
std::tuple<Tensor, Tensor, Tensor, Tensor> egnn_node_fwd(const Tensor& h, const Tensor&,
                                                         const std::vector<Tensor>&, const Tensor&,
                                                         bool with_ab, int64_t, bool, double,
                                                         bool train) {
  const int64_t N = h.size(0), d = h.size(1);
  auto o = h.options();
  return {at::empty({N, d}, o), at::empty({with_ab ? N : 0, 2 * d}, o),
          at::empty({train ? 2 : 0, N, d}, o), at::empty({train ? 2 : 0, N}, o)};
}
std::tuple<Tensor, Tensor, Tensor, Tensor, Tensor, Tensor, Tensor> egnn_edge_bwd(
    const Tensor& pos, const Tensor&, const Tensor& recv, const Tensor&,
    const std::vector<Tensor>&, int64_t, bool, const Tensor& xhat, const Tensor&, const Tensor&,
    const Tensor&, const optional<Tensor>&, bool pos_branch, bool pos_grad) {
  const int64_t N = pos.size(0), E = recv.numel(), d = xhat.size(2);
  auto o = pos.options();
  return {at::empty({N, d}, o), at::empty({pos_grad ? N : 0, 3}, o), at::empty({E, d}, o),
          at::empty({pos_grad ? E : 0, 3}, o), at::empty({E, d}, o),
          at::empty({pos_branch ? E : 0, d}, o),
          at::empty({gmp_egnn_edge_bwd_partials_rows(E, d), 8 * d + 1}, o)};
}
Tensor cfconv_aggregate(const Tensor& x, const Tensor&, const Tensor&, const Tensor&,
                        const Tensor&, int64_t n_seg, const optional<Tensor>&) {
  return at::empty({n_seg, x.size(1)}, x.options());
}
Tensor cfconv_wgrad(const Tensor&, const Tensor& gidx, const Tensor& x, const Tensor&,
                    const optional<Tensor>&) {
  return at::empty({gidx.numel(), x.size(1)}, x.options());
}
Tensor ssp_fwd(const Tensor& x, double) { return at::empty_like(x); }
Tensor ssp_bwd(const Tensor& x, const Tensor&) { return at::empty_like(x); }
std::tuple<Tensor, Tensor> cfconv_cgrad(const Tensor&, const Tensor&, const Tensor& x,
                                        const Tensor&, const Tensor& w, const optional<Tensor>&) {
  return {at::empty({w.size(0)}, x.options()), at::empty({1}, x.options().dtype(at::kInt))};
}
std::tuple<Tensor, Tensor> ssp_bwd2(const Tensor& x, const Tensor&, const Tensor&) {
  return {at::empty_like(x), at::empty_like(x)};
}
std::tuple<Tensor, Tensor, Tensor> ln_act_fwd(const Tensor& x, const Tensor&, const Tensor&, double,
                                              int64_t) {
  return {at::empty_like(x), at::empty_like(x), at::empty({x.numel() / x.size(-1)}, x.options())};
}
std::tuple<Tensor, Tensor> ln_act_bwd(const Tensor&, const Tensor& xhat, const Tensor&,
                                      const Tensor&, const Tensor&, int64_t) {
  return {at::empty_like(xhat), at::empty({2 * xhat.size(-1)}, xhat.options())};
}
Tensor edge_xyz_dot(const Tensor& A, const Tensor&) {
  return at::empty({A.size(1) / 3}, A.options());
}
Tensor vec_norm_fwd(const Tensor& v) { return at::empty_like(v); }
Tensor vec_norm_bwd(const Tensor& v, const Tensor&) { return at::empty_like(v); }
Tensor xyz_norm_fwd(const Tensor& vh) { return at::empty({vh.size(0), vh.size(2)}, vh.options()); }
Tensor xyz_norm_bwd(const Tensor& vh, const Tensor&) { return at::empty_like(vh); }
std::tuple<Tensor, Tensor> edge_featurize(const Tensor& pos, const Tensor& ei,
                                          at::ArrayRef<double> w, double, double, double,
                                          int64_t lmax, const optional<Tensor>&) {
  return {at::empty({ei.size(1), (lmax + 1) * (lmax + 1)}, pos.options()),
          at::empty({ei.size(1), (int64_t)w.size()}, pos.options())};
}
Tensor edge_featurize_bwd(const Tensor& pos, const Tensor& ei, at::ArrayRef<double>, double,
                          double, double, const optional<Tensor>&, const optional<Tensor>&,
                          int64_t, const optional<Tensor>&) {
  return at::empty({ei.size(1), 3}, pos.options());
}
std::tuple<Tensor, Tensor> edge_featurize_gvp(const Tensor& pos, const Tensor& ei,
                                              at::ArrayRef<double> w, double, double, double) {
  return {at::empty({ei.size(1), (int64_t)w.size()}, pos.options()),
          at::empty({ei.size(1), 3}, pos.options())};
}
Tensor edge_featurize_gvp_bwd(const Tensor& pos, const Tensor& ei, at::ArrayRef<double>, double,
                              double, double, const optional<Tensor>&, const optional<Tensor>&) {
  return at::empty({ei.size(1), 3}, pos.options());
}
std::tuple<Tensor, Tensor, Tensor> schnet_featurize(const Tensor& pos, const Tensor& ei,
                                                    const Tensor& offsets, double, double,
                                                    const optional<Tensor>&) {
  const int64_t E = ei.size(1);
  return {at::empty({E}, pos.options()), at::empty({E, offsets.numel()}, pos.options()),
          at::empty({E}, pos.options())};
}
Tensor schnet_featurize_bwd(const Tensor& pos, const Tensor& ei, const Tensor&, double, double,
                            const optional<Tensor>&, const optional<Tensor>&,
                            const optional<Tensor>&, const optional<Tensor>&) {
  return at::empty({ei.size(1), 3}, pos.options());
}
Tensor edge_shift_vectors(const Tensor& sidx, const Tensor& cell, const optional<Tensor>&) {
  return at::empty({sidx.size(0), 3}, cell.options());
}
std::tuple<Tensor, Tensor, Tensor, Tensor> schnet_featurize_bwd2(
    const Tensor& pos, const Tensor& ei, const Tensor& offsets, double, double,
    const optional<Tensor>&, const optional<Tensor>&, const optional<Tensor>&, const Tensor&,
    bool want_dist, bool want_rbf, bool want_cut, bool want_vec, const optional<Tensor>&) {
  const int64_t E = ei.size(1);
  auto o = pos.options();
  return {at::empty({want_dist ? E : 0}, o), at::empty({want_rbf ? E : 0, offsets.numel()}, o),
          at::empty({want_cut ? E : 0}, o), at::empty({want_vec ? E : 0, 3}, o)};
}
Tensor gate_fwd(const Tensor& x, const Tensor& out_map, double, double) {
  return at::empty({x.size(0), out_map.size(0)}, x.options());
}
Tensor gate_bwd(const Tensor& x, const Tensor&, const Tensor&, double, double) {
  return at::empty_like(x);
}
// ... 178 lines not shown
    const Tensor& jb, const Tensor& angle, const Tensor&, const Tensor&, const Tensor&,
    const Tensor& w1t, const Tensor& w2t, int64_t n, int64_t k, int64_t, int64_t, int64_t,
    const Tensor&, const Tensor&, bool want_geometry) {
  const int64_t Tg = want_geometry ? angle.numel() : 0;
  auto o = jb.options();
  return {at::empty_like(w1t), at::empty_like(w2t), at::empty({Tg, n * k}, o), at::empty({Tg}, o),
          at::empty({Tg}, o)};
}
Tensor triplet_interact_fwd(const Tensor& src, const Tensor&, const Tensor&, const Tensor& wa,
                            const Tensor&, const Tensor&, const optional<Tensor>&,
                            const Tensor& rowptr) {
  return at::empty({rowptr.numel() - 1, wa.size(0)}, src.options());
}
std::tuple<Tensor, Tensor, Tensor, Tensor> triplet_interact_bwd(
    const Tensor&, const Tensor&, const Tensor& S, const Tensor& P, const Tensor& wa,
    const Tensor& wt, const Tensor&, const Tensor&) {
  return {at::empty_like(S), at::empty_like(P), at::empty_like(wa), at::empty_like(wt)};
}
constexpr auto& dime_edge_basis_fwd = sph_edge_basis_fwd;
constexpr auto& dime_edge_basis_bwd = sph_edge_basis_bwd;
Tensor dime_triplet_proj_fwd(const Tensor& sbe, const Tensor& angle, const Tensor&, const Tensor&,
                             const Tensor&, int64_t, int64_t, int64_t L, int64_t b) {
  return at::empty({L, angle.numel(), b}, sbe.options());
}
Tensor dime_triplet_emb(const Tensor& sbe, const Tensor& angle, const Tensor&, const Tensor&,
                        int64_t n, int64_t k) {
  return at::empty({angle.numel(), n * k}, sbe.options());
}
std::tuple<Tensor, Tensor, Tensor> dime_triplet_proj_bwd(
    const Tensor& sbe, const Tensor& angle, const Tensor&, const Tensor&, const Tensor& wt,
    int64_t n, int64_t k, int64_t, int64_t, const Tensor&, bool want_geometry) {
  const int64_t Tg = want_geometry ? angle.numel() : 0;
  auto o = sbe.options();
  return {at::empty_like(wt), at::empty({Tg, n * k}, o), at::empty({Tg}, o)};
}
std::tuple<Tensor, Tensor, Tensor, Tensor> dime_edge_basis_bwd2(
    const Tensor& dist, const Tensor& freq, const Tensor& zeros, const Tensor&, double, int64_t,
    const optional<Tensor>&, const optional<Tensor>&, const optional<Tensor>&,
    const optional<Tensor>&) {
  const int64_t E = dist.numel(), k = freq.numel();
  auto o = dist.options();
  return {at::empty({E, k}, o), at::empty({E, zeros.numel()}, o), at::empty({E}, o),
          at::empty({k}, o)};
}
std::tuple<Tensor, Tensor, Tensor, Tensor> dime_triplet_proj_bwd2(
    const Tensor& sbe, const Tensor& angle, const Tensor&, const Tensor&, const Tensor& wt,
    int64_t n, int64_t k, int64_t L, int64_t b, const Tensor&, const optional<Tensor>&,
    const optional<Tensor>&, const optional<Tensor>&, bool want_geometry) {
  const int64_t T = angle.numel(), Tg = want_geometry ? T : 0;
  auto o = sbe.options();
  return {at::empty({L, T, b}, o), at::empty_like(wt), at::empty({Tg, n * k}, o),
          at::empty({Tg}, o)};
}
Tensor triplet_interact1_fwd(const Tensor& src, const Tensor&, const Tensor& w, const Tensor&,
                             const optional<Tensor>&, const Tensor& rowptr) {
  return at::empty({rowptr.numel() - 1, w.size(0)}, src.options());
}
std::tuple<Tensor, Tensor> triplet_interact1_bwd(const Tensor&, const Tensor&, const Tensor& S,
                                                 const Tensor& w, const Tensor&, const Tensor&) {
  return {at::empty_like(S), at::empty_like(w)};
}
}

}

TORCH_LIBRARY(gmp, m) {
  m.def("csr_build(Tensor index, int n_seg, Tensor? payload=None) -> "
        "(Tensor perm, Tensor rowptr, Tensor sorted, Tensor payload_sorted, Tensor err)");
  m.def("gather_rows(Tensor src, Tensor index) -> Tensor");
  m.def("segment_reduce(Tensor src, Tensor? perm, Tensor rowptr, int n_seg, str reduce) -> "
        "(Tensor out, Tensor argmax)");
  m.def("segment_reduce_bwd(Tensor grad_out, Tensor index, Tensor rowptr, str reduce, "
        "Tensor? argmax, int n_items) -> Tensor");
  m.def("egnn_edge_fwd(Tensor AB, Tensor pos, Tensor rowptr, Tensor recv, Tensor send, "
        "Tensor[] params, int act, bool msg_mean, float eps, bool train, int xhat_planes=2, "
        "bool need_pos=True) -> "
        "(Tensor m_aggr, Tensor pos_aggr, Tensor xhat, Tensor rstd)");
  m.def("egnn_node_image(Tensor[] W0s, Tensor[] W3s, Tensor?[] W1ns) -> Tensor");
  m.def("egnn_node_fwd(Tensor h, Tensor m_aggr, Tensor[] vecs, Tensor image, bool with_ab, "
        "int act, bool residual, float eps, bool train) -> (Tensor h_out, Tensor ab, "
        "Tensor xhat, Tensor rstd)");
  m.def("egnn_edge_bwd(Tensor pos, Tensor rowptr, Tensor recv, Tensor send, Tensor[] params, "
        "int act, bool msg_mean, Tensor xhat, Tensor rstd, Tensor g_m_aggr, Tensor g_pos_aggr, "
        "Tensor(a!)? amax=None, bool pos_branch=True, bool pos_grad=True) -> (Tensor dA, "
        "Tensor dpos_recv, "
        "Tensor dpre1, Tensor gdiff, Tensor dpre2, Tensor dpre3, Tensor partials)");
  m.def("cfconv_aggregate(Tensor x, Tensor xidx, Tensor w, Tensor perm, Tensor rowptr, "
        "int n_seg, Tensor? escale=None) -> Tensor");
  m.def("cfconv_wgrad(Tensor g, Tensor gidx, Tensor x, Tensor xidx, Tensor? escale=None) -> "
        "Tensor");
  m.def("ssp_fwd(Tensor x, float shift) -> Tensor");
  m.def("ssp_bwd(Tensor x, Tensor grad_y) -> Tensor");
  m.def("cfconv_cgrad(Tensor g, Tensor gidx, Tensor x, Tensor xidx, Tensor w, "
        "Tensor? escale=None) -> (Tensor dc, Tensor err)");
  m.def("ssp_bwd2(Tensor x, Tensor grad_y, Tensor a) -> (Tensor gg, Tensor gx)");
  m.def("ln_act_fwd(Tensor x, Tensor gamma, Tensor beta, float eps, int act) -> "
        "(Tensor y, Tensor xhat, Tensor rstd)");
  m.def("ln_act_bwd(Tensor grad_y, Tensor xhat, Tensor rstd, Tensor gamma, Tensor beta, "
        "int act) -> (Tensor grad_x, Tensor grad_gamma_beta)");
  m.def("vec_norm_fwd(Tensor v) -> Tensor");
  m.def("vec_norm_bwd(Tensor v, Tensor grad_out) -> Tensor");
  m.def("xyz_norm_fwd(Tensor vh) -> Tensor");
  m.def("xyz_norm_bwd(Tensor vh, Tensor grad_out) -> Tensor");
  m.def("edge_featurize(Tensor pos, Tensor edge_index, float[] bessel_weights, float prefactor, "
        "float r_max, float p, int lmax=2, Tensor? shift=None) -> (Tensor sh, Tensor radial)");
  m.def("edge_featurize_bwd(Tensor pos, Tensor edge_index, float[] bessel_weights, "
        "float prefactor, float r_max, float p, Tensor? g_sh, Tensor? g_radial, int lmax=2, "
        "Tensor? shift=None) -> Tensor");
  m.def("edge_featurize_gvp(Tensor pos, Tensor edge_index, float[] bessel_weights, "
        "float prefactor, float r_max, float p) -> (Tensor radial, Tensor unit)");
  m.def("edge_featurize_gvp_bwd(Tensor pos, Tensor edge_index, float[] bessel_weights, "
        "float prefactor, float r_max, float p, Tensor? g_radial, Tensor? g_unit) -> Tensor");
  m.def("schnet_featurize(Tensor pos, Tensor edge_index, Tensor offsets, float coeff, "
        "float cutoff, Tensor? shift=None) -> (Tensor dist, Tensor rbf, Tensor cut)");
  m.def("schnet_featurize_bwd(Tensor pos, Tensor edge_index, Tensor offsets, float coeff, "
        "float cutoff, Tensor? g_dist, Tensor? g_rbf, Tensor? g_cut, Tensor? shift=None) -> "
        "Tensor");
  m.def("edge_shift_vectors(Tensor edge_shift_idx, Tensor cell, Tensor? edge_graph=None) -> "
        "Tensor");
  m.def("schnet_featurize_bwd2(Tensor pos, Tensor edge_index, Tensor offsets, float coeff, "
        "float cutoff, Tensor? g_dist, Tensor? g_rbf, Tensor? g_cut, Tensor a_vec, "
        "bool want_dist=True, bool want_rbf=True, bool want_cut=True, bool want_vec=True, "
        "Tensor? shift=None) -> (Tensor gg_dist, Tensor gg_rbf, Tensor gg_cut, Tensor h_vec)");
  m.def("gate_fwd(Tensor x, Tensor out_map, float c_act, float c_gate) -> Tensor");
  m.def("gate_bwd(Tensor x, Tensor grad_y, Tensor in_map, float c_act, float c_gate) -> Tensor");
  m.def("irreps_bn_fwd(Tensor x, Tensor col_chan, Tensor chan_col, Tensor chan_info, "
        "Tensor weight, Tensor? bias, Tensor(a!) running_mean, Tensor(b!) running_var, "
        "bool training, float momentum, float eps) -> (Tensor y, Tensor shift, Tensor invstd)");
  m.def("irreps_bn_bwd(Tensor x, Tensor grad_y, Tensor col_chan, Tensor chan_col, "
        "Tensor chan_info, Tensor weight, Tensor shift, Tensor invstd, bool training, "
        "int n_scalar) -> (Tensor grad_x, Tensor grad_weight, Tensor grad_bias)");
  m.def("symmetric_contraction_fwd(Tensor x, Tensor plan, int rows, Tensor coef) -> Tensor");
  m.def("symmetric_contraction_bwd(Tensor x, Tensor plan, int rows, Tensor coef, Tensor gout) "
        "-> (Tensor dx, Tensor dcoef_partials)");
  m.def("tp_edge_z(int[] desc, Tensor paths, Tensor cg, Tensor x, Tensor sh, Tensor src_sorted, "
        "Tensor perm, int e0, int e1) -> Tensor");
  m.def("tp_edge_z_bwd(int[] desc, Tensor paths, Tensor cg, Tensor x, Tensor sh, "
        "Tensor src_sorted, Tensor perm, int e0, int e1, Tensor dz) -> "
        "(Tensor dx_edge, Tensor dY_edge)");
  m.def("tp_conv_fwd(int layout, int[] desc, Tensor paths, Tensor cg, Tensor x, Tensor sh, "
        "Tensor W, Tensor src_sorted, Tensor perm, int c0, int c1, Tensor(a!) msg) -> ()");
  m.def("tp_conv_bwd(int layout, int[] desc, Tensor paths, Tensor cg, Tensor x, Tensor sh, "
        "Tensor W, Tensor recv_sorted, Tensor src_sorted, Tensor perm, int c0, int c1, "
        "Tensor gout, Tensor(a!) dx_edge, Tensor(b!) dY_edge) -> Tensor dW");
  m.def("tp_node_outer(Tensor eoff, Tensor Z, Tensor A, int w) -> (Tensor S, Tensor Sb)");
  m.def("tp_node_apply(Tensor eoff, Tensor Z, Tensor A, Tensor T, Tensor Tb, Tensor(a!) dA, "
        "Tensor(b!) dZ) -> ()");
  m.def("tp_split_w2(Tensor W2, Tensor b2, int off, int mul1, int mul_out, bool fwd) -> Tensor");
  m.def("tp_gemm_x3(Tensor A1, int K1, Tensor? A2, int K2, Tensor Bp, int ldb, int N, "
        "Tensor(a!) C, int c_offset, int cgrp, int cldg, int cldr, int cldn, bool accumulate) "
        "-> ()");
  m.def("tp_gemm_x3_widen(Tensor A, Tensor Bp, int N) -> Tensor");
  m.def("outer_sum_cols(Tensor A, Tensor B) -> Tensor");
  m.def("edge_outer_sum(Tensor A, Tensor B) -> (Tensor C, Tensor colsum)");
  m.def("edge_outer_sum_ex(Tensor A, Tensor B, Tensor(a!) C, Tensor(b!)? colsum, int act, "
        "Tensor? w, Tensor? b) -> ()");
  m.def("edge_outer_sum_ex2(Tensor A, Tensor B1, Tensor B2, Tensor(a!) C, Tensor(b!)? colsum) "
        "-> ()");
  m.def("edge_outer_sum_act(Tensor A, Tensor X, Tensor w, Tensor b, int act, Tensor? amax=None) "
        "-> (Tensor C, Tensor colsum)");
  m.def("egnn_node_bwd(Tensor g, Tensor xhat, Tensor rstd, Tensor W0, Tensor W3, Tensor[] vecs, "
        "int act, bool residual) -> Tensor[]");
  m.def("gvp_ff_fwd(Tensor s, Tensor v, Tensor[] W) -> Tensor[]");
  m.def("gvp_ff_bwd(Tensor v, Tensor[] W, Tensor gate1, Tensor B2, Tensor s2, Tensor ds, "
        "Tensor dv) -> Tensor[]");
  m.def("gvp_layer_fwd(Tensor s, Tensor v, Tensor[] W, bool relu) -> (Tensor s_out, "
        "Tensor v_out)");
  m.def("gvp_layer_bwd(Tensor s, Tensor v, Tensor[] W, Tensor ds, Tensor dv, bool relu, "
        "bool want_factors=True) -> "
        "Tensor[]");
  m.def("gvp_layer_fwd_agg(Tensor s, Tensor v, Tensor[] W, Tensor? perm, Tensor skey, "
        "Tensor rowptr, int n_nodes, str reduce) -> (Tensor s_agg, Tensor v_agg)");
  m.def("gvp_layer_bwd_agg(Tensor s, Tensor v, Tensor[] W, Tensor ds, Tensor dv, Tensor index, "
        "Tensor rowptr, str reduce, bool relu, bool want_factors=True) -> Tensor[]");
  m.def("edge_xyz_dot(Tensor A, Tensor v) -> Tensor");
  m.def("gvp_edge_embed_fwd(Tensor radial, Tensor unit, Tensor[] W, float eps) "
        "-> (Tensor es, Tensor ev)");
  m.def("gvp_edge_embed_bwd(Tensor radial, Tensor unit, Tensor[] W, float eps, Tensor grad_es, "
        "Tensor grad_ev) -> Tensor");
  m.def("gvp_msg0_fwd(Tensor send, Tensor recv, Tensor P, Tensor Q, Tensor es, Tensor ev, "
        "Tensor[] W) -> (Tensor s_out, Tensor v_out)");
  m.def("gvp_msg0_bwd(Tensor send, Tensor recv, Tensor P, Tensor Q, Tensor es, Tensor ev, "
        "Tensor[] W, Tensor ds, Tensor dv, bool want_factors=True) -> Tensor[]");
  m.def("gvp_msg0_bwd_agg(Tensor send, Tensor recv, Tensor P, Tensor Q, Tensor es, Tensor ev, "
        "Tensor[] W, Tensor ds, Tensor dv, Tensor? perm, Tensor rowptr, int n_nodes, "
        "bool want_factors=True) -> Tensor[]");
  m.def("sph_edge_basis_fwd(Tensor dist, Tensor freq, Tensor zeros, Tensor norm, float cutoff, "
        "int envelope_exponent) -> (Tensor rbf, Tensor jb)");
  m.def("sph_edge_basis_bwd(Tensor dist, Tensor freq, Tensor zeros, Tensor norm, float cutoff, "
        "int envelope_exponent, Tensor? grad_rbf, Tensor? grad_jb) -> "
        "(Tensor grad_dist, Tensor grad_freq)");
  m.def("sph_triplet_proj_fwd(Tensor jb, Tensor angle, Tensor torsion, Tensor idx_kj, Tensor pref, "
        "Tensor w_sbf1_t, Tensor w_t1_t, int num_spherical, int num_radial, int n_layers, int ba, "
        "int bt) -> (Tensor S, Tensor P)");
  m.def("sph_triplet_emb(Tensor jb, Tensor angle, Tensor torsion, Tensor idx_kj, Tensor pref, "
        "int num_spherical, int num_radial) -> (Tensor angle_emb, Tensor torsion_emb)");
  m.def("sph_triplet_proj_bwd(Tensor jb, Tensor angle, Tensor torsion, Tensor idx_kj, Tensor pref, "
        "Tensor w_sbf1_t, Tensor w_t1_t, int num_spherical, int num_radial, int n_layers, int ba, "
        "int bt, Tensor grad_S, Tensor grad_P, bool want_geometry) -> (Tensor grad_w_sbf1_t, "
        "Tensor grad_w_t1_t, Tensor grad_jb_rows, Tensor grad_angle, Tensor grad_torsion)");
  m.def("triplet_interact_fwd(Tensor src, Tensor S, Tensor P, Tensor w_sbf2, Tensor w_t2, "
        "Tensor gather_idx, Tensor? perm, Tensor rowptr) -> Tensor");
  m.def("triplet_interact_bwd(Tensor grad_m, Tensor xd, Tensor S, Tensor P, Tensor w_sbf2, "
        "Tensor w_t2, Tensor idx_kj, Tensor offsets) -> (Tensor grad_S, Tensor grad_P, "
        "Tensor grad_w_sbf2, Tensor grad_w_t2)");
  m.def("dime_edge_basis_fwd(Tensor dist, Tensor freq, Tensor zeros, Tensor norm, float cutoff, "
        "int envelope_exponent) -> (Tensor rbf, Tensor sbe)");
  m.def("dime_edge_basis_bwd(Tensor dist, Tensor freq, Tensor zeros, Tensor norm, float cutoff, "
        "int envelope_exponent, Tensor? grad_rbf, Tensor? grad_sbe) -> "
        "(Tensor grad_dist, Tensor grad_freq)");
  m.def("dime_triplet_proj_fwd(Tensor sbe, Tensor angle, Tensor idx_kj, Tensor pref, "
        "Tensor w_sbf1_t, int num_spherical, int num_radial, int n_layers, int b) -> Tensor");
  m.def("dime_triplet_emb(Tensor sbe, Tensor angle, Tensor idx_kj, Tensor pref, "
        "int num_spherical, int num_radial) -> Tensor");
  m.def("dime_triplet_proj_bwd(Tensor sbe, Tensor angle, Tensor idx_kj, Tensor pref, "
        "Tensor w_sbf1_t, int num_spherical, int num_radial, int n_layers, int b, Tensor grad_S, "
        "bool want_geometry) -> (Tensor grad_w_sbf1_t, Tensor grad_sbe_rows, Tensor grad_angle)");
  m.def("dime_edge_basis_bwd2(Tensor dist, Tensor freq, Tensor zeros, Tensor norm, float cutoff, "
        "int envelope_exponent, Tensor? grad_rbf, Tensor? grad_sbe, Tensor? a_dist, "
        "Tensor? a_freq) -> (Tensor gg_rbf, Tensor gg_sbe, Tensor h_dist, Tensor h_freq)");
  m.def("dime_triplet_proj_bwd2(Tensor sbe, Tensor angle, Tensor idx_kj, Tensor pref, "
        "Tensor w_sbf1_t, int num_spherical, int num_radial, int n_layers, int b, Tensor grad_S, "
        "Tensor? a_sbe, Tensor? a_angle, Tensor? a_w_sbf1_t, bool want_geometry) -> "
        "(Tensor gg_S, Tensor h_w_sbf1_t, Tensor h_sbe_rows, Tensor h_angle)");
  m.def("triplet_interact1_fwd(Tensor src, Tensor S, Tensor w_sbf2, Tensor gather_idx, "
        "Tensor? perm, Tensor rowptr) -> Tensor");
  m.def("triplet_interact1_bwd(Tensor grad_m, Tensor xd, Tensor S, Tensor w_sbf2, Tensor idx_kj, "
        "Tensor offsets) -> (Tensor grad_S, Tensor grad_w_sbf2)");
}

#define GMP_IMPL(m, ns)                                                    \
  m.impl("csr_build", ns csr_build);                                      \
  m.impl("gather_rows", ns gather_rows);                                  \
  m.impl("segment_reduce", ns segment_reduce);                            \
  m.impl("segment_reduce_bwd", ns segment_reduce_bwd);                    \
  m.impl("egnn_edge_fwd", ns egnn_edge_fwd);                              \
  m.impl("egnn_node_fwd", ns egnn_node_fwd);                              \
  m.impl("egnn_node_image", ns egnn_node_image);                          \
  m.impl("egnn_edge_bwd", ns egnn_edge_bwd);                              \
  m.impl("cfconv_aggregate", ns cfconv_aggregate);                        \
  m.impl("cfconv_wgrad", ns cfconv_wgrad);                                \
  m.impl("ssp_fwd", ns ssp_fwd);                                          \
  m.impl("ssp_bwd", ns ssp_bwd);                                          \
  m.impl("cfconv_cgrad", ns cfconv_cgrad);                                \
  m.impl("ssp_bwd2", ns ssp_bwd2);                                        \
  m.impl("ln_act_fwd", ns ln_act_fwd);                                    \
  m.impl("ln_act_bwd", ns ln_act_bwd);                                    \
  m.impl("edge_xyz_dot", ns edge_xyz_dot);                                \
  m.impl("gvp_edge_embed_fwd", ns gvp_edge_embed_fwd);                    \
  m.impl("gvp_edge_embed_bwd", ns gvp_edge_embed_bwd);                    \
  m.impl("vec_norm_fwd", ns vec_norm_fwd);                                \
  m.impl("vec_norm_bwd", ns vec_norm_bwd);                                \
  m.impl("xyz_norm_fwd", ns xyz_norm_fwd);                                \
  m.impl("xyz_norm_bwd", ns xyz_norm_bwd);                                \
  m.impl("edge_featurize", ns edge_featurize);                            \
  m.impl("edge_featurize_bwd", ns edge_featurize_bwd);                    \
  m.impl("edge_featurize_gvp", ns edge_featurize_gvp);                    \
  m.impl("edge_featurize_gvp_bwd", ns edge_featurize_gvp_bwd);            \
  m.impl("schnet_featurize", ns schnet_featurize);                        \
  m.impl("schnet_featurize_bwd", ns schnet_featurize_bwd);                \
  m.impl("schnet_featurize_bwd2", ns schnet_featurize_bwd2);              \
  m.impl("edge_shift_vectors", ns edge_shift_vectors);                    \
  m.impl("gate_fwd", ns gate_fwd);                                        \
  m.impl("gate_bwd", ns gate_bwd);                                        \
  m.impl("irreps_bn_fwd", ns irreps_bn_fwd);                              \
  m.impl("irreps_bn_bwd", ns irreps_bn_bwd);                              \
  m.impl("symmetric_contraction_fwd", ns symmetric_contraction_fwd);      \
  m.impl("symmetric_contraction_bwd", ns symmetric_contraction_bwd);      \
  m.impl("tp_edge_z", ns tp_edge_z);                                      \
  m.impl("tp_edge_z_bwd", ns tp_edge_z_bwd);                              \
  m.impl("tp_conv_fwd", ns tp_conv_fwd);                                  \
  m.impl("tp_conv_bwd", ns tp_conv_bwd);                                  \
  m.impl("tp_node_outer", ns tp_node_outer);                              \
  m.impl("tp_node_apply", ns tp_node_apply);                              \
  m.impl("tp_split_w2", ns tp_split_w2);                                  \
  m.impl("tp_gemm_x3", ns tp_gemm_x3);                                    \
  m.impl("tp_gemm_x3_widen", ns tp_gemm_x3_widen);                        \
  m.impl("outer_sum_cols", ns outer_sum_cols);                            \
  m.impl("edge_outer_sum", ns edge_outer_sum);                            \
  m.impl("edge_outer_sum_ex", ns edge_outer_sum_ex);                      \
  m.impl("edge_outer_sum_ex2", ns edge_outer_sum_ex2);                    \
  m.impl("edge_outer_sum_act", ns edge_outer_sum_act);                    \
  m.impl("egnn_node_bwd", ns egnn_node_bwd);                              \
  m.impl("gvp_ff_fwd", ns gvp_ff_fwd);                                    \
  m.impl("gvp_ff_bwd", ns gvp_ff_bwd);                                    \
  m.impl("gvp_layer_fwd", ns gvp_layer_fwd);                              \
  m.impl("gvp_layer_bwd", ns gvp_layer_bwd);                              \
  m.impl("gvp_layer_bwd_agg", ns gvp_layer_bwd_agg);                      \
  m.impl("gvp_layer_fwd_agg", ns gvp_layer_fwd_agg);                      \
  m.impl("gvp_msg0_bwd_agg", ns gvp_msg0_bwd_agg);                        \
  m.impl("gvp_msg0_fwd", ns gvp_msg0_fwd);                                \
  m.impl("gvp_msg0_bwd", ns gvp_msg0_bwd);                                \
  m.impl("sph_edge_basis_fwd", ns sph_edge_basis_fwd);                    \
  m.impl("sph_edge_basis_bwd", ns sph_edge_basis_bwd);                    \
  m.impl("sph_triplet_proj_fwd", ns sph_triplet_proj_fwd);                \
  m.impl("sph_triplet_emb", ns sph_triplet_emb);                          \
  m.impl("sph_triplet_proj_bwd", ns sph_triplet_proj_bwd);                \
  m.impl("triplet_interact_fwd", ns triplet_interact_fwd);                \
  m.impl("triplet_interact_bwd", ns triplet_interact_bwd);                \
  m.impl("dime_edge_basis_fwd", ns dime_edge_basis_fwd);                  \
  m.impl("dime_edge_basis_bwd", ns dime_edge_basis_bwd);                  \
  m.impl("dime_triplet_proj_fwd", ns dime_triplet_proj_fwd);              \
  m.impl("dime_triplet_emb", ns dime_triplet_emb);                        \
  m.impl("dime_triplet_proj_bwd", ns dime_triplet_proj_bwd);              \
  m.impl("dime_edge_basis_bwd2", ns dime_edge_basis_bwd2);                \
  m.impl("dime_triplet_proj_bwd2", ns dime_triplet_proj_bwd2);            \
  m.impl("triplet_interact1_fwd", ns triplet_interact1_fwd);              \
  m.impl("triplet_interact1_bwd", ns triplet_interact1_bwd);

TORCH_LIBRARY_IMPL(gmp, CUDA, m) { GMP_IMPL(m, ) }
TORCH_LIBRARY_IMPL(gmp, CPU, m) { GMP_IMPL(m, ) }
TORCH_LIBRARY_IMPL(gmp, Meta, m) { GMP_IMPL(m, meta::) }
```

### geometric-message-passing_amd/gmp_amd/_lib.py

```python
import ctypes
import os

import torch

_HERE = os.path.dirname(os.path.abspath(__file__))
LIB_PATH = os.environ.get("GMP_LIB", os.path.join(_HERE, "libgmp.so"))

c_i64 = ctypes.c_int64
c_int = ctypes.c_int
c_vp = ctypes.c_void_p
c_f32 = ctypes.c_float
c_size = ctypes.c_size_t

GMP_OK, GMP_ERR_ARG, GMP_ERR_HIP, GMP_ERR_UNSUPPORTED, GMP_ERR_WORKSPACE = 0, -1, -2, -3, -4
REDUCE = {"sum": 0, "add": 0, "mean": 1, "max": 2}
ACT = {"relu": 0, "swish": 1, "silu": 1}
EGNN_NO_POS_BRANCH, EGNN_NO_POS_GRAD = 1, 2
(WGRAD_ROUTE_ZERO, WGRAD_ROUTE_X3, WGRAD_ROUTE_QUAD, WGRAD_ROUTE_SQUARE_F32,
 WGRAD_ROUTE_RECT_F32, WGRAD_ROUTE_LIBRARY) = range(1, 7)


class GmpEgnnParams(ctypes.Structure):
    _fields_ = [(n, c_vp) for n in (
        "w1d", "b1", "ln1_w", "ln1_b", "W2", "b2", "ln2_w", "ln2_b", "W3", "b3", "ln3_w", "ln3_b",
# ... 102 lines not shown
    "gmp_edge_outer_sum_ex_workspace_size": (c_size, [c_i64, c_i64, c_i64]),
    "gmp_edge_outer_sum_ex_route": (c_int, [c_i64, c_i64, c_i64, c_i64, c_i64, c_int]),
    "gmp_edge_outer_sum_ex_f32": (c_int, [c_i64, c_i64, c_i64, c_vp, c_i64, c_vp, c_i64, c_int,
                                          c_vp, c_vp, c_vp, c_i64, c_vp, c_vp, c_size, c_vp]),
    "gmp_edge_outer_sum_rect_workspace_size": (c_size, [c_i64, c_i64, c_i64]),
    "gmp_edge_xyz_dot_workspace_size": (c_size, [c_i64]),
    "gmp_edge_xyz_dot_f32": (c_int, [c_i64, c_i64, c_vp, c_vp, c_vp, c_vp, c_size, c_vp]),
    "gmp_edge_outer_sum_rect_f32": (c_int, [c_i64, c_i64, c_i64, c_vp, c_vp, c_vp, c_vp, c_vp,
                                            c_size, c_vp]),
    "gmp_tp_node_outer_f32": (c_int, [c_i64, c_i64, c_i64, c_vp, c_vp, c_vp, c_vp, c_vp, c_vp]),
    "gmp_tp_node_apply_f32": (c_int, [c_i64, c_i64, c_i64, c_vp, c_vp, c_vp, c_vp, c_vp, c_vp,
                                      c_vp, c_vp]),
    "gmp_tp_apply_set_x3": (c_int, [c_int]),
    "gmp_tp_split_w2_f32": (c_int, [c_i64, c_i64, c_i64, c_vp, c_vp, c_vp, c_vp, c_vp]),
    "gmp_tp_gemm_x3_f32": (c_int, [c_i64, c_i64, c_i64, c_vp, c_i64, c_i64, c_vp, c_i64, c_vp,
                                   c_i64, c_i64, c_vp, c_i64, c_i64, c_i64, c_i64, c_int, c_vp]),
    "gmp_tp_gemm_x3_widen_f32": (c_int, [c_i64, c_i64, c_i64, c_vp, c_i64, c_vp, c_i64, c_i64,
                                         c_vp, c_i64, c_vp]),
    "gmp_outer_sum_cols_workspace_size": (c_size, [c_i64, c_i64, c_i64]),
    "gmp_outer_sum_cols_f32": (c_int, [c_i64, c_i64, c_i64, c_vp, c_i64, c_vp, c_i64, c_vp,
                                       c_i64, c_vp, c_size, c_vp]),
    "gmp_gvp_layer_fwd_f32": (c_int, [c_i64, c_int] + [c_vp] * 10 + [c_vp]),
    "gmp_gvp_layer_bwd_f32": (c_int, [c_i64, c_int] + [c_vp] * 19 + [c_vp]),
    "gmp_gvp_layer_bwd_agg_f32": (c_int, [c_i64, c_i64, c_int, c_vp, c_vp, c_int] + [c_vp] * 19
                                  + [c_vp]),
    "gmp_gvp_layer_fwd_agg_f32": (c_int, [c_i64, c_i64, c_int] + [c_vp] * 13 + [c_vp]),
    "gmp_gvp_msg0_bwd_agg_f32": (c_int, [c_i64, c_i64] + [c_vp] * 30 + [c_vp]),
    "gmp_gvp_msg0_fwd_f32": (c_int, [c_i64] + [c_vp] * 15 + [c_vp]),
    "gmp_gvp_ff_fwd_f32": (c_int, [c_i64] + [c_vp] * 21 + [c_vp]),
    "gmp_egnn_node_bwd_partial_rows": (c_i64, [c_i64]),
    "gmp_egnn_node_bwd_f32": (c_int, [c_i64, c_i64, c_int, c_int] + [c_vp] * 13 + [c_vp]),
    "gmp_gvp_ff_bwd_f32": (c_int, [c_i64] + [c_vp] * 25 + [c_vp]),
    "gmp_gvp_edge_embed_fwd_f32": (c_int, [c_i64, c_i64, c_i64] + [c_vp] * 10 + [c_f32, c_vp,
                                                                                 c_vp, c_vp]),
    "gmp_gvp_edge_embed_bwd_workspace_size": (c_size, [c_i64]),
    "gmp_gvp_edge_embed_bwd_f32": (c_int, [c_i64, c_i64, c_i64] + [c_vp] * 10 + [c_f32, c_vp,
                                                                                 c_vp, c_vp, c_vp,
                                                                                 c_size, c_vp]),
    "gmp_gvp_msg0_bwd_f32": (c_int, [c_i64] + [c_vp] * 24 + [c_vp]),
    "gmp_radius_cells_f32": (c_int, [c_vp, c_vp, c_i64, c_vp, c_f32, c_vp, c_vp, c_vp]),
    "gmp_radius_count_f32": (c_int, [c_vp, c_vp, c_i64, c_f32, c_i64, c_vp, c_f32, c_vp, c_vp,
                                     c_vp, c_vp, c_vp, c_vp]),
    "gmp_radius_fill_f32": (c_int, [c_vp, c_vp, c_i64, c_f32, c_i64, c_vp, c_f32, c_vp, c_vp,
                                    c_vp, c_vp, c_vp, c_vp, c_vp]),
    "gmp_batch_collate": (c_int, [c_vp, c_i64, c_vp, c_vp, c_i64, c_i64, c_vp, c_vp, c_vp, c_vp]),
    "gmp_triplet_count": (c_int, [c_vp, c_vp, c_i64, c_i64, c_vp, c_vp, c_vp, c_vp, c_vp]),
    "gmp_triplet_fill_f32": (c_int, [c_vp, c_vp, c_i64, c_i64, c_vp, c_vp, c_vp, c_vp, c_i64,
                                     c_int, c_vp, c_vp, c_vp, c_vp, c_vp, c_vp]),
    "gmp_triplet_torsion_bwd_f32": (c_int, [c_vp, c_vp, c_i64, c_vp, c_vp, c_vp, c_i64, c_vp,
                                            c_vp, c_vp, c_vp]),
    "gmp_ln_act_fwd_f32": (c_int, [c_i64, c_i64, c_vp, c_vp, c_vp, c_f32, c_int, c_vp, c_vp,
                                   c_vp, c_vp]),
    "gmp_ln_act_bwd_workspace_size": (c_size, [c_i64, c_i64]),
    "gmp_ln_act_bwd_partial_rows": (c_i64, [c_i64]),
    "gmp_vec_norm_fwd_f32": (c_int, [c_i64, c_i64, c_vp, c_vp, c_vp]),
    "gmp_vec_norm_bwd_f32": (c_int, [c_i64, c_i64, c_vp, c_vp, c_vp, c_vp]),
    "gmp_xyz_norm_fwd_f32": (c_int, [c_i64, c_i64, c_vp, c_vp, c_vp]),
    "gmp_xyz_norm_bwd_f32": (c_int, [c_i64, c_i64, c_vp, c_vp, c_vp, c_vp]),
    "gmp_sum_rows_f32": (c_int, [c_vp, c_i64, c_i64, c_vp, c_vp]),
    "gmp_ln_act_bwd_f32": (c_int, [c_i64, c_i64, c_vp, c_vp, c_vp, c_vp, c_vp, c_int, c_vp, c_vp,
                                   c_vp, c_size, c_vp]),
    "gmp_sc_groups": (c_int, [c_i64]),
    "gmp_sc_route": (c_int, [c_i64, c_int, c_int, c_int, c_int, ctypes.POINTER(c_i64)]),
    "gmp_symmetric_contraction_fwd_f32": (c_int, [c_i64, c_int, c_int, c_int, c_int, c_vp, c_vp,
                                                  c_vp, c_vp, c_vp]),
    "gmp_symmetric_contraction_bwd_f32": (c_int, [c_i64, c_int, c_int, c_int, c_int, c_vp, c_vp,
                                                  c_vp, c_vp, c_vp, c_vp, c_vp]),
    "gmp_egnn_node_image_bytes": (c_size, [c_i64]),
    "gmp_egnn_node_image_f32": (c_int, [c_i64, c_i64, ctypes.POINTER(GmpEgnnNodeParams), c_vp,
                                        c_vp]),
    "gmp_egnn_node_fwd_f32": (c_int, [c_i64, c_i64, c_vp, c_vp, ctypes.POINTER(GmpEgnnNodeParams),
                                      c_vp, c_int, c_int, c_f32, c_vp, c_vp, c_vp, c_vp, c_vp]),
    "gmp_egnn_edge_bwd_f32": (c_int, [c_i64, c_i64, c_i64, c_vp, c_vp, c_vp, c_vp,
                                      ctypes.POINTER(GmpEgnnParams), c_int, c_int, c_vp, c_int]
                              + [c_vp] * 11),
    "gmp_cfconv_cgrad_f32": (c_int, [c_vp, c_i64, c_vp, c_vp, c_i64, c_vp, c_vp, c_vp, c_i64,
                                     c_i64, c_vp, c_vp, c_vp]),
    "gmp_egnn_edge_fwd_ex_f32": (c_int, [c_i64, c_i64, c_i64, c_vp, c_vp, c_vp, c_vp, c_vp,
                                         ctypes.POINTER(GmpEgnnParams), c_int, c_int, c_f32, c_vp,
                                         c_vp, c_vp, c_int, c_vp, ctypes.c_uint32, c_vp]),
    "gmp_egnn_edge_bwd_ex_f32": (c_int, [c_i64, c_i64, c_i64, c_vp, c_vp, c_vp, c_vp,
                                         ctypes.POINTER(GmpEgnnParams), c_int, c_int, c_vp, c_int]
                                 + [c_vp] * 11 + [ctypes.c_uint32, c_vp]),
    "gmp_ssp_bwd2_f32": (c_int, [c_vp, c_vp, c_vp, c_i64, c_vp, c_vp, c_vp]),
    "gmp_schnet_featurize_bwd2_f32": (c_int, [c_vp, c_i64, c_vp, c_i64, c_int, c_vp, c_f32, c_f32]
                                      + [c_vp] * 9),
    "gmp_featurize_shift_workspace_size": (c_size, [c_i64]),
    "gmp_edge_featurize_lmax_ex_f32": (c_int, [c_vp, c_vp, c_i64, c_int, c_int, c_vp, c_f32,
                                               c_f32, c_f32, c_vp, c_vp, c_size] + [c_vp] * 5),
    "gmp_edge_featurize_lmax_bwd_ex_f32": (c_int, [c_vp, c_vp, c_i64, c_int, c_int, c_vp, c_f32,
                                                   c_f32, c_f32, c_vp, c_vp, c_size]
                                           + [c_vp] * 4),
    "gmp_schnet_featurize_ex_f32": (c_int, [c_vp, c_vp, c_i64, c_int, c_vp, c_f32, c_f32, c_vp,
                                            c_vp, c_size] + [c_vp] * 4),
    "gmp_schnet_featurize_bwd_ex_f32": (c_int, [c_vp, c_vp, c_i64, c_int, c_vp, c_f32, c_f32,
                                                c_vp, c_vp, c_size] + [c_vp] * 5),
    "gmp_schnet_featurize_bwd2_ex_f32": (c_int, [c_vp, c_i64, c_vp, c_i64, c_int, c_vp, c_f32,
                                                 c_f32, c_vp, c_vp, c_size] + [c_vp] * 9),
    "gmp_radius_pbc_sort_capacity": (c_int, []),
    "gmp_radius_pbc_bins_f32": (c_int, [c_vp, c_vp, c_i64, c_i64] + [c_vp] * 7),
    "gmp_radius_pbc_count_f32": (c_int, [c_vp, c_vp, c_i64, c_i64, c_f32] + [c_vp] * 10),
    "gmp_radius_pbc_fill_f32": (c_int, [c_vp, c_vp, c_i64, c_i64, c_f32] + [c_vp] * 12),
    "gmp_edge_shift_vectors_f32": (c_int, [c_vp, c_vp, c_vp, c_i64, c_i64, c_vp, c_vp]),
    "gmp_sph_edge_basis_fwd_f32": (c_int, [c_vp, c_i64, c_f32, c_int, c_vp, c_int, c_vp, c_vp,
                                           c_int, c_vp, c_vp, c_vp]),
    "gmp_sph_edge_basis_bwd_partial_rows": (c_i64, [c_i64]),
    "gmp_sph_edge_basis_bwd_f32": (c_int, [c_vp, c_i64, c_f32, c_int, c_vp, c_int, c_vp, c_vp,
                                           c_int] + [c_vp] * 6),
    "gmp_sph_triplet_proj_fwd_f32": (c_int, [c_i64, c_i64, c_int, c_int] + [c_vp] * 6
                                     + [c_int, c_int, c_vp, c_int, c_vp, c_vp, c_vp]),
    "gmp_sph_triplet_emb_f32": (c_int, [c_i64, c_i64, c_int, c_int] + [c_vp] * 8),
    "gmp_sph_triplet_proj_bwd_partial_rows": (c_i64, [c_i64]),
    "gmp_sph_triplet_proj_bwd_f32": (c_int, [c_i64, c_i64, c_int, c_int] + [c_vp] * 6
                                     + [c_int, c_int, c_vp, c_int] + [c_vp] * 8),
    "gmp_triplet_interact_fwd_f32": (c_int, [c_i64, c_i64, c_i64, c_i64, c_int, c_int]
                                     + [c_vp] * 10),
    "gmp_triplet_interact_bwd_partial_rows": (c_i64, [c_i64]),
    "gmp_triplet_interact_bwd_f32": (c_int, [c_i64, c_i64, c_i64, c_int, c_int] + [c_vp] * 13),
    "gmp_dime_edge_basis_fwd_f32": (c_int, [c_vp, c_i64, c_f32, c_int, c_vp, c_int, c_vp, c_vp,
                                            c_int, c_vp, c_vp, c_vp]),
    "gmp_dime_edge_basis_bwd_partial_rows": (c_i64, [c_i64]),
    "gmp_dime_edge_basis_bwd_f32": (c_int, [c_vp, c_i64, c_f32, c_int, c_vp, c_int, c_vp, c_vp,
                                            c_int] + [c_vp] * 6),
    "gmp_dime_triplet_proj_fwd_f32": (c_int, [c_i64, c_i64, c_int, c_int] + [c_vp] * 5
                                      + [c_int, c_int, c_vp, c_vp]),
    "gmp_dime_triplet_emb_f32": (c_int, [c_i64, c_i64, c_int, c_int] + [c_vp] * 6),
    "gmp_dime_triplet_proj_bwd_partial_rows": (c_i64, [c_i64]),
    "gmp_dime_triplet_proj_bwd_f32": (c_int, [c_i64, c_i64, c_int, c_int] + [c_vp] * 5
                                      + [c_int, c_int] + [c_vp] * 6),
    "gmp_triplet_geom_bwd2_f32": (c_int, [c_vp, c_vp, c_i64, c_vp, c_vp, c_i64, c_int]
                                  + [c_vp] * 8),
    "gmp_dime_edge_basis_bwd2_partial_rows": (c_i64, [c_i64]),
    "gmp_dime_edge_basis_bwd2_f32": (c_int, [c_vp, c_i64, c_f32, c_int, c_vp, c_int, c_vp, c_vp,
                                             c_int] + [c_vp] * 10),
    "gmp_dime_triplet_proj_bwd2_partial_rows": (c_i64, [c_i64]),
    "gmp_dime_triplet_proj_bwd2_f32": (c_int, [c_i64, c_i64, c_int, c_int] + [c_vp] * 5
                                       + [c_int, c_int] + [c_vp] * 10),
    "gmp_triplet_interact1_fwd_f32": (c_int, [c_i64, c_i64, c_i64, c_i64, c_int] + [c_vp] * 8),
    "gmp_triplet_interact1_bwd_partial_rows": (c_i64, [c_i64]),
    "gmp_triplet_interact1_bwd_f32": (c_int, [c_i64, c_i64, c_i64, c_int] + [c_vp] * 10),
    "gmp_triplet_count_pbc": (c_int, [c_vp, c_vp, c_i64, c_i64] + [c_vp] * 7),
    "gmp_triplet_fill_pbc_f32": (c_int, [c_vp, c_vp, c_i64, c_i64] + [c_vp] * 5
                                 + [c_i64, c_vp, c_vp, c_vp, c_vp]),
    "gmp_triplet_vec_bwd_f32": (c_int, [c_vp, c_i64, c_vp, c_vp, c_i64] + [c_vp] * 4),
    "gmp_triplet_vec_bwd2_f32": (c_int, [c_vp, c_i64, c_vp, c_vp, c_i64] + [c_vp] * 7),
    "gmp_triplet_dat_pbc_f32": (c_int, [c_vp, c_i64, c_vp, c_vp, c_vp, c_i64] + [c_vp] * 4),
    "gmp_triplet_dat_vec_bwd_f32": (c_int, [c_vp, c_i64, c_vp, c_vp, c_vp, c_vp, c_i64]
                                    + [c_vp] * 5),
}

ABI_VERSION = 6
_lib = None
TORCH_LIB_PATH = os.environ.get("GMP_TORCH_LIB", os.path.join(_HERE, "libgmp_torch.so"))
_torch_ops = None


class GmpError(RuntimeError):
    pass


def torch_ops():
    global _torch_ops
    if _torch_ops is None:
        load()
        if not os.path.exists(TORCH_LIB_PATH):
            raise GmpError(f"libgmp_torch.so not found at {TORCH_LIB_PATH}: build it first "
# ... 33 lines not shown
```

### geometric-message-passing_amd/gmp_amd/ops.py

```python
import ctypes


import torch
from torch.autograd.function import once_differentiable

from . import _lib
from ._lib import check


def _p(t):
    return None if t is None else ctypes.c_void_p(t.data_ptr())


def _stream():
    return ctypes.c_void_p(torch.cuda.current_stream().cuda_stream)


KERNEL_TIMERS = None
KERNEL_TIMER_NAMES = None


class _timed:
    def __init__(self, name):
        self.name = name
# ... 16 lines not shown
def kernel_time_ms(name):
    evs = (KERNEL_TIMERS or {}).get(name, [])
    if not evs:
        return None
    torch.cuda.synchronize()
    return sum(a.elapsed_time(b) for a, b in evs) / len(evs)


def _need_cuda(*ts):
    for t in ts:
        if t is not None and not t.is_cuda:
            raise _lib.GmpError("gmp_amd ops run on the MI355X only: got a CPU tensor "
                                "(no CPU fallback in the product path)")


def _f32c(t):
    if t.dtype != torch.float32:
        raise _lib.GmpError(f"expected float32, got {t.dtype}")
    return t.contiguous()


def _i64c(t):
    if t.dtype != torch.int64:
        t = t.long()
    return t.contiguous()


class CSR:

    __slots__ = ("index", "n_seg", "perm", "rowptr", "sorted", "payload_sorted", "err")

    def __init__(self, index, n_seg, payload=None):
        index = _i64c(index)
        _need_cuda(index)
        self.index = index
        self.n_seg = int(n_seg)
        pl = _i64c(payload) if payload is not None else None
        self.perm, self.rowptr, self.sorted, pls, self.err = _lib.torch_ops().csr_build(
            index, self.n_seg, pl)
        self.payload_sorted = pls if pl is not None else None

    def counts(self):
        return self.rowptr[1:] - self.rowptr[:-1]

    def check_range(self):
        if int(self.err.item()) != 0:
            raise IndexError("index out of range in gmp CSR build")


_CSR_CACHE = []


def _tkey(t):
    if t is None:
        return None
    return (t.data_ptr(), tuple(t.shape), tuple(t.stride()), t.dtype, t.device, t._version)


def get_csr(index, n_seg, payload=None):
    if compiling():
        return CSR(index, n_seg, payload)
    key = (_tkey(index), int(n_seg), _tkey(payload))
    for k, (kk, _, _, csr) in enumerate(_CSR_CACHE):
        if kk == key:
            _CSR_CACHE.insert(0, _CSR_CACHE.pop(k))
            return csr
    csr = CSR(index, n_seg, payload)
    _CSR_CACHE.insert(0, (key, index, payload, csr))
    del _CSR_CACHE[16:]
    return csr


def clear_cache():
    _CSR_CACHE.clear()


def gather_rows(src2d, index):
    src2d = _f32c(src2d)
    index = _i64c(index)
    _need_cuda(src2d, index)
    return _lib.torch_ops().gather_rows(src2d, index)


def segment_reduce(src2d, csr, reduce="sum", use_perm=True):
    src2d = _f32c(src2d)
    _need_cuda(src2d)
    out, argmax = _lib.torch_ops().segment_reduce(src2d, csr.perm if use_perm else None,
                                                  csr.rowptr, csr.n_seg, reduce)
    return out, (argmax if reduce == "max" else None)


def edge_outer_sum(A, B):
    A, B = _f32c(A), _f32c(B)
    _need_cuda(A, B)
    with _timed("edge_outer_sum"):
        return _lib.torch_ops().edge_outer_sum(A, B)


def edge_outer_sum_act(A, X, w, b, act, amax=None):
    A, X, w, b = _f32c(A), _f32c(X), _f32c(w), _f32c(b)
    _need_cuda(A, X, w, b)
    with _timed("edge_outer_sum"):
        return _lib.torch_ops().edge_outer_sum_act(A, X, w, b, _lib.ACT[act], amax)


def outer_sum_into(A, B, C, colsum=None, act=None, w=None, b=None):
    _need_cuda(A, B, C)
    a = -1 if act is None else _lib.ACT[act]
    with _timed("edge_outer_sum"):
        _lib.torch_ops().edge_outer_sum_ex(A, B, C, colsum, a, w, b)


def outer_sum_into2(A, B1, B2, C, colsum=None):
    _need_cuda(A, B1, B2, C)
    with _timed("edge_outer_sum"):
        _lib.torch_ops().edge_outer_sum_ex2(A, B1, B2, C, colsum)


def edge_outer_sum_rect(A, B):
    A, B = _f32c(A), _f32c(B)
    _need_cuda(A, B)
    m, n = A.shape[1], B.shape[1]
    mp, np_ = -(-m // 16) * 16, -(-n // 16) * 16
    if mp != m:
        A = torch.nn.functional.pad(A, (0, mp - m))
    if np_ != n:
        B = torch.nn.functional.pad(B, (0, np_ - n))
    C = torch.empty((mp, np_), dtype=torch.float32, device=A.device)
    cs = torch.empty(mp, dtype=torch.float32, device=A.device)
    bn = 144 if np_ <= 144 else 128
    for m0 in range(0, mp, 128):
        for n0 in range(0, np_, bn):
            outer_sum_into(A[:, m0:m0 + 128], B[:, n0:n0 + bn], C[m0:m0 + 128, n0:n0 + bn],
                           cs[m0:m0 + 128] if n0 == 0 else None)
    if (mp, np_) != (m, n):
        return C[:m, :n].contiguous(), cs[:m]
    return C, cs


DEFER_WEIGHT_GRADS = True
_SIDE_STREAMS = {}
_PENDING = []
_CB_QUEUED = [False]
_KEEPALIVE = []


def _side_stream(device):
    st = _SIDE_STREAMS.get(device)
    if st is None:
        st = _SIDE_STREAMS[device] = torch.cuda.Stream(device=device)
    return st


def _flush_deferred():
    _CB_QUEUED[0] = False
    if not _PENDING:
        return
    main = torch.cuda.current_stream()
    for st in _SIDE_STREAMS.values():
        main.wait_stream(st)
    _KEEPALIVE.clear()
    for p, g in _PENDING:
        g.record_stream(main)
        if p.grad is None:
            p.grad = g if g.stride() == p.stride() else g.contiguous()
        else:
            p.grad.add_(g)
# ... 338 lines not shown
        C = _f32c(C.detach().reshape(-1))
    ei = _i64c(edge_index)
    return CFConvAggregateFn.apply(x, W, ei[0], ei[1], x.shape[0], C)


def edge_vec_to_pos_grad(g_vec, edge_index, n):
    plus, _ = segment_reduce(g_vec, get_csr(edge_index[0], n), "sum")
    minus, _ = segment_reduce(g_vec, get_csr(edge_index[1], n), "sum")
    return plus - minus


class GvpEdgeFeaturizeFn(torch.autograd.Function):

    @staticmethod
    def forward(ctx, pos, edge_index, host_consts):
        w, pref, r_max, p = host_consts
        pos, ei = _f32c(pos), _i64c(edge_index)
        _need_cuda(pos, ei)
        with _timed("edge_featurize"):
            rad, unit = _lib.torch_ops().edge_featurize_gvp(pos, ei, [float(v) for v in w], pref,
                                                            r_max, p)
        ctx.save_for_backward(pos, ei)
        ctx.host = host_consts
        return rad, unit

    @staticmethod
    @once_differentiable
    def backward(ctx, g_rad, g_unit):
        if not ctx.needs_input_grad[0]:
            return None, None, None
        pos, ei = ctx.saved_tensors
        w, pref, r_max, p = ctx.host
        g_vec = _lib.torch_ops().edge_featurize_gvp_bwd(
            pos, ei, [float(v) for v in w], pref, r_max, p,
            _f32c(g_rad) if g_rad is not None else None,
            _f32c(g_unit) if g_unit is not None else None)
        return edge_vec_to_pos_grad(g_vec, ei, pos.shape[0]), None, None


def _needs(ctx, k):
    return len(ctx.needs_input_grad) > k and ctx.needs_input_grad[k]


class SchNetFeaturizeFn(torch.autograd.Function):

    @staticmethod
    def forward(ctx, pos, edge_index, offsets, coeff, cutoff, shift=None):
        pos, ei, off = _f32c(pos), _i64c(edge_index), _f32c(offsets)
        _need_cuda(pos, ei, off)
        sh = _f32c(shift) if shift is not None else None
        with _timed("edge_featurize"):
            d, rbf, cut = _lib.torch_ops().schnet_featurize(pos, ei, off, float(coeff),
                                                            float(cutoff), sh)
        ctx.save_for_backward(pos, ei, off, sh)
        ctx.coeff, ctx.cutoff = float(coeff), float(cutoff)
        return d, rbf, cut

    @staticmethod
    @once_differentiable
    def backward(ctx, g_d, g_rbf, g_cut):
        need_pos, need_shift = ctx.needs_input_grad[0], _needs(ctx, 5)
        if not (need_pos or need_shift):
            return None, None, None, None, None, None
        pos, ei, off, sh = ctx.saved_tensors
        opt = [_f32c(t) if t is not None else None for t in (g_d, g_rbf, g_cut)]
        g_vec = _lib.torch_ops().schnet_featurize_bwd(pos, ei, off, ctx.coeff, ctx.cutoff, *opt,
                                                      sh)
        return (edge_vec_to_pos_grad(g_vec, ei, pos.shape[0]) if need_pos else None, None, None,
                None, None, g_vec if need_shift else None)


class EgnnGraph:

    def __init__(self, edge_index, num_nodes):
        ei = _i64c(edge_index)
        _need_cuda(ei)
        self.num_nodes = int(num_nodes)
        self.num_edges = ei.shape[1]
        self.recv_csr = CSR(ei[1], self.num_nodes, payload=ei[0])
        self.recv = self.recv_csr.sorted
        self.send = self.recv_csr.payload_sorted
        self.rowptr = self.recv_csr.rowptr
        self.send_csr = CSR(self.send, self.num_nodes)

    def check_range(self):
        self.recv_csr.check_range()
        self.send_csr.check_range()


_EGNN_GRAPHS = []


def egnn_graph(edge_index, num_nodes):
    if compiling():
        return EgnnGraph(edge_index, num_nodes)
    for k, (t, ver, n, g) in enumerate(_EGNN_GRAPHS):
        if t is edge_index and ver == edge_index._version and n == num_nodes:
            return g
    g = EgnnGraph(edge_index, num_nodes)
    _EGNN_GRAPHS.insert(0, (edge_index, edge_index._version, num_nodes, g))
    del _EGNN_GRAPHS[8:]
    return g


_EGNN_PARAM_NAMES = ("w1d", "b1", "ln1_w", "ln1_b", "W2", "b2", "ln2_w", "ln2_b", "W3", "b3",
                     "ln3_w", "ln3_b", "w4", "b4")


def _egnn_params(tensors):
    return _lib.GmpEgnnParams(*[t.data_ptr() for t in tensors])


EGNN_XHAT_PLANES = 2

EGNN_SKIP_DEAD_POS = True


class EgnnMessageFn(torch.autograd.Function):

    @staticmethod
    def forward(ctx, h, pos, graph, act, msg_mean, eps, W1, b1, ln1w, ln1b, W2, b2, ln2w, ln2b,
                W3, b3, ln3w, ln3b, w4, b4, grad_mode=True, AB=None, need_pos=True):
        h, pos = _f32c(h), _f32c(pos)
        _need_cuda(h, pos, W1)
        N, d = h.shape
        E = graph.num_edges
        if AB is None:
            Wcat = torch.cat([W1[:, :d], W1[:, d:2 * d]], 0)
            AB = h.mm(Wcat.t())
        params = tuple(_f32c(t) for t in (W1[:, 2 * d], b1, ln1w, ln1b, W2, b2, ln2w, ln2b, W3,
                                          b3, ln3w, ln3b, w4, b4))
        train = bool(grad_mode) and any(ctx.needs_input_grad)
        ctx.set_materialize_grads(False)
        fwd_pos = bool(need_pos) or not EGNN_SKIP_DEAD_POS
        with _timed("egnn_edge_fwd"):
            m_aggr, pos_aggr, xhat, rstd = _lib.torch_ops().egnn_edge_fwd(
                AB, pos, graph.rowptr, graph.recv, graph.send, list(params), _lib.ACT[act],
                bool(msg_mean), float(eps), train, EGNN_XHAT_PLANES, fwd_pos)
        ctx.graph, ctx.act, ctx.msg_mean, ctx.N = graph, act, msg_mean, N
        ctx.fwd_pos = fwd_pos
        if train:
            ctx.save_for_backward(h, pos, xhat, rstd, W1, *params)
        return m_aggr, (pos_aggr if need_pos else None)

    @staticmethod
    @once_differentiable
    def backward(ctx, g_m, g_p):
        h, pos, xhat, rstd, W1, *params = ctx.saved_tensors
        graph = ctx.graph
        N, d = ctx.N, xhat.shape[2]
        E = graph.num_edges
        dev = pos.device
        f = dict(dtype=torch.float32, device=dev)
        pos_branch = ctx.fwd_pos and not (EGNN_SKIP_DEAD_POS and g_p is None)
        pos_grad = ctx.needs_input_grad[1] or not EGNN_SKIP_DEAD_POS
        g_m = torch.zeros((N, d), **f) if g_m is None else _f32c(g_m)
        if not pos_branch:
            g_p = torch.empty((0, 3), **f)
        else:
            g_p = torch.zeros((N, 3), **f) if g_p is None else _f32c(g_p)
        amax = torch.zeros(2, dtype=torch.int32, device=dev)
        with _timed("egnn_edge_bwd"):
            dA, dpos_recv, dpre1, gdiff, dpre2, dpre3, partials = \
                _lib.torch_ops().egnn_edge_bwd(pos, graph.rowptr, graph.recv, graph.send,
                                               list(params), _lib.ACT[ctx.act],
                                               bool(ctx.msg_mean), xhat, rstd, g_m, g_p, amax,
                                               pos_branch, pos_grad)
        xh1, xh2 = xhat[0], xhat[1]
        dB, _ = segment_reduce(dpre1, graph.send_csr, "sum")
        W1t = W1[:, :2 * d].t().contiguous()
        dh = _mm_wt(dA, W1t[:d])
        dh.addmm_(dB, W1t[d:].t())
        dpos = None
        if pos_grad:
            dpos_send, _ = segment_reduce(gdiff, graph.send_csr, "sum")
            dpos = dpos_recv - dpos_send

        (_, b1, ln1w, ln1b, W2, b2, ln2w, ln2b, W3, b3, ln3w, ln3b, w4, b4) = params
        dW2, db2 = edge_outer_sum_act(dpre2, xh1, ln1w, ln1b, ctx.act, amax[0:1])
        if pos_branch:
            dW3, db3 = edge_outer_sum_act(dpre3, xh2, ln2w, ln2b, ctx.act, amax[1:2])
        else:
            dW3, db3 = torch.zeros((d, d), **f), torch.zeros(d, **f)
        with side_work(h, dA, dB, partials) as sw:
            dW1 = torch.empty((d, 2 * d + 1), **f)
            db1 = torch.empty(d, **f)
            outer_sum_into(dA, h, dW1[:, :d], db1)
            outer_sum_into(dB, h, dW1[:, d:2 * d])
            v = partials.sum(0)
            dln1w, dln1b, dln2w, dln2b, dln3w, dln3b, dw4, dw1d = v[:8 * d].view(8, d).unbind(0)
            dW1[:, 2 * d].copy_(dw1d)
            grads = (dW1, db1, dln1w, dln1b, dW2, db2, dln2w, dln2b, dW3, db3, dln3w, dln3b,
                     dw4.view(1, d), v[8 * d:8 * d + 1])
        targets = (W1,) + tuple(params[1:])
        return (dh, dpos, None, None, None, None) + sw.deliver(ctx.needs_input_grad, 6, targets,
                                                               grads) + (None, None, None)


def egnn_exact_mode():
    lib = _lib.load()
    prev = lib.gmp_egnn_set_f32_mfma(0)
    lib.gmp_egnn_set_f32_mfma(prev)
    return bool(prev)


def egnn_node_images(layers, next_layers):
    with torch.no_grad():
        return _lib.torch_ops().egnn_node_image(
            [_f32c(l.mlp_upd[0].weight) for l in layers], [_f32c(l.mlp_upd[3].weight) for l in layers],
            [None if n is None else n.mlp_msg[0].weight for n in next_layers])


EGNN_NODE_BWD_FUSED = True


class EgnnNodeFn(torch.autograd.Function):

    @staticmethod
    def forward(ctx, h, m, W0, b0, ln1w, ln1b, W3, b3, ln2w, ln2b, image, with_ab, act, residual,
                eps, grad_mode):
        h, m = _f32c(h), _f32c(m)
        _need_cuda(h, m, W0)
        vecs = [_f32c(t) for t in (b0, ln1w, ln1b, b3, ln2w, ln2b)]
        train = bool(grad_mode) and any(ctx.needs_input_grad)
        with _timed("egnn_node_fwd"):
            ho, ab, xhat, rstd = _lib.torch_ops().egnn_node_fwd(
                h, m, vecs, image, bool(with_ab), _lib.ACT[act], bool(residual), float(eps), train)
        ctx.act, ctx.residual = act, bool(residual)
        if train:
            ctx.save_for_backward(h, m, xhat, rstd, _f32c(W0), vecs[0], vecs[1], vecs[2],
                                  _f32c(W3), vecs[3], vecs[4], vecs[5])
        ctx.mark_non_differentiable(ab)
        return ho, (ab if with_ab else None)

    @staticmethod
    @once_differentiable
    def backward(ctx, g, _g_ab):
        h, m, xhat, rstd, W0, b0, ln1w, ln1b, W3, b3, ln2w, ln2b = ctx.saved_tensors
        d = h.shape[1]
        g = _f32c(g)
        tops = _lib.torch_ops()
        a = _LN_ACT[ctx.act]
        if EGNN_NODE_BWD_FUSED and a in (0, 1) and d in (32, 64, 128):
            with _timed("egnn_node_bwd"):
                dh, dm, dpre1, dpre2, gb = tops.egnn_node_bwd(g, xhat, rstd, W0, W3,
                                                              [ln1w, ln1b, ln2w, ln2b], a,
                                                              ctx.residual)
            gb1, gb2 = gb[:2 * d], gb[2 * d:]
            dh = dh if ctx.needs_input_grad[0] else None
            dm = dm if ctx.needs_input_grad[1] else None
        else:
            dpre2, gb2 = tops.ln_act_bwd(g, xhat[1], rstd[1], ln2w, ln2b, a)
            dx1 = _dx(dpre2, W3)
            dpre1, gb1 = tops.ln_act_bwd(dx1, xhat[0], rstd[0], ln1w, ln1b, a)
            dh = _dx(dpre1, W0[:, :d]) if ctx.needs_input_grad[0] else None
            if dh is not None and ctx.residual:
                dh += g
            dm = _dx(dpre1, W0[:, d:]) if ctx.needs_input_grad[1] else None
        with side_work(dpre1, dpre2, h, m, xhat) as sw:
            dW0 = torch.empty_like(W0)
            db0 = torch.empty_like(b0)
            outer_sum_into(dpre1, h, dW0[:, :d], db0)
            outer_sum_into(dpre1, m, dW0[:, d:], None)
            dW3 = torch.empty_like(W3)
            db3 = torch.empty_like(b3)
            outer_sum_into(dpre2, xhat[0], dW3, db3, ctx.act, ln1w, ln1b)
        grads = (dW0, db0, gb1[:d], gb1[d:], dW3, db3, gb2[:d], gb2[d:])
        return ((dh, dm) + sw.deliver(ctx.needs_input_grad, 2,
                                      (W0, b0, ln1w, ln1b, W3, b3, ln2w, ln2b), grads)
                + (None, None, None, None, None, None))

# ... 780 lines not shown
```

### include/gmp.h

```cpp
#ifndef GMP_H_
#define GMP_H_

#include <stddef.h>
#include <stdint.h>

#ifdef __cplusplus
extern "C" {
#endif

#define GMP_ABI_VERSION 6

enum {
  GMP_OK = 0,
  GMP_ERR_ARG = -1,
  GMP_ERR_HIP = -2,
  GMP_ERR_UNSUPPORTED = -3,
  GMP_ERR_WORKSPACE = -4
};

enum { GMP_REDUCE_SUM = 0, GMP_REDUCE_MEAN = 1, GMP_REDUCE_MAX = 2 };
enum { GMP_ACT_RELU = 0, GMP_ACT_SILU = 1 };

int gmp_abi_version(void);
const char* gmp_error_string(int code);
// ... 18 lines not shown
                               int reduce, const int64_t* argmax, float* grad_src, void* stream);

typedef struct gmp_egnn_params {
  const float* w1d;
  const float* b1;
  const float* ln1_w;
  const float* ln1_b;
  const float* W2;
  const float* b2;
  const float* ln2_w;
  const float* ln2_b;
  const float* W3;
  const float* b3;
  const float* ln3_w;
  const float* ln3_b;
  const float* w4;
  const float* b4;
} gmp_egnn_params;

int gmp_egnn_set_f32_mfma(int on);
int gmp_egnn_edge_fwd_f32(int64_t n_nodes, int64_t n_edges, int64_t d, const float* AB,
                          const float* pos, const int64_t* rowptr, const int64_t* recv,
                          const int64_t* send, const gmp_egnn_params* params, int act,
                          int msg_mean, float ln_eps, float* m_aggr, float* pos_aggr,
                          float* save_xhat, int save_planes, float* save_rstd, void* stream);
#define GMP_EGNN_NO_POS_BRANCH 1u
#define GMP_EGNN_NO_POS_GRAD 2u
int gmp_egnn_edge_fwd_ex_f32(int64_t n_nodes, int64_t n_edges, int64_t d, const float* AB,
                             const float* pos, const int64_t* rowptr, const int64_t* recv,
                             const int64_t* send, const gmp_egnn_params* params, int act,
                             int msg_mean, float ln_eps, float* m_aggr, float* pos_aggr,
                             float* save_xhat, int save_planes, float* save_rstd, uint32_t flags,
                             void* stream);

typedef struct gmp_egnn_node_params {
  const float* W0;
  const float* b0;
  const float* ln1_w;
  const float* ln1_b;
  const float* W3;
  const float* b3;
  const float* ln2_w;
  const float* ln2_b;
  const float* W1n;
  int64_t ld1;
} gmp_egnn_node_params;
size_t gmp_egnn_node_image_bytes(int64_t d);
int gmp_egnn_node_image_f32(int64_t d, int64_t n_layers, const gmp_egnn_node_params* params,
                            void* images, void* stream);
int gmp_egnn_node_fwd_f32(int64_t n_nodes, int64_t d, const float* h, const float* m_aggr,
                          const gmp_egnn_node_params* params, const void* image, int act,
                          int residual, float ln_eps, float* h_out, float* ab_out,
                          float* save_xhat, float* save_rstd, void* stream);

int64_t gmp_egnn_node_bwd_partial_rows(int64_t n_nodes);
int gmp_egnn_node_bwd_f32(int64_t n_nodes, int64_t d, int act, int residual, const float* grad_h,
                          const float* save_xhat, const float* save_rstd, const float* W0,
                          const float* W3, const float* ln1_w, const float* ln1_b,
                          const float* ln2_w, const float* ln2_b, float* dh, float* dm,
                          float* dpre1, float* dpre2, float* partials, void* stream);
int64_t gmp_egnn_edge_bwd_partials_rows(int64_t n_edges, int64_t d);
int gmp_egnn_edge_bwd_f32(int64_t n_nodes, int64_t n_edges, int64_t d, const float* pos,
                          const int64_t* rowptr, const int64_t* recv, const int64_t* send,
                          const gmp_egnn_params* params, int act, int msg_mean,
                          const float* save_xhat, int save_planes, const float* save_rstd,
                          const float* g_m_aggr, const float* g_pos_aggr, float* dA,
                          float* dpos_recv, float* dpre1, float* gdiff, float* dpre2, float* dpre3,
                          float* vec_partials, void* stream);
int gmp_egnn_edge_bwd_amax_f32(int64_t n_nodes, int64_t n_edges, int64_t d, const float* pos,
                               const int64_t* rowptr, const int64_t* recv, const int64_t* send,
                               const gmp_egnn_params* params, int act, int msg_mean,
                               const float* save_xhat, int save_planes, const float* save_rstd,
                               const float* g_m_aggr, const float* g_pos_aggr, float* dA,
                               float* dpos_recv, float* dpre1, float* gdiff, float* dpre2,
                               float* dpre3, float* vec_partials, uint32_t* amax, void* stream);
int gmp_egnn_edge_bwd_ex_f32(int64_t n_nodes, int64_t n_edges, int64_t d, const float* pos,
                             const int64_t* rowptr, const int64_t* recv, const int64_t* send,
                             const gmp_egnn_params* params, int act, int msg_mean,
                             const float* save_xhat, int save_planes, const float* save_rstd,
                             const float* g_m_aggr, const float* g_pos_aggr, float* dA,
                             float* dpos_recv, float* dpre1, float* gdiff, float* dpre2,
                             float* dpre3, float* vec_partials, uint32_t* amax, uint32_t flags,
                             void* stream);

int gmp_wgrad_set_f32_mfma(int on);
size_t gmp_edge_outer_sum_workspace_size(int64_t K, int64_t d);
int gmp_edge_outer_sum_f32(int64_t K, int64_t d, const float* A, const float* B, float* C,
                           float* colsum_A, void* workspace, size_t workspace_bytes,
                           void* stream);
int gmp_edge_outer_sum_act_f32(int64_t K, int64_t d, const float* A, const float* X,
                               const float* w, const float* b, int act, float* C,
                               float* colsum_A, void* workspace, size_t workspace_bytes,
                               void* stream);
int gmp_edge_outer_sum_act_hf_f32(int64_t K, int64_t d, const float* A, const float* X,
                                  const float* w, const float* b, int act, const uint32_t* amax_A,
                                  float* C, float* colsum_A, void* workspace,
                                  size_t workspace_bytes, void* stream);

size_t gmp_edge_outer_sum_rect_workspace_size(int64_t K, int64_t m, int64_t n);
size_t gmp_edge_xyz_dot_workspace_size(int64_t K);
int gmp_edge_xyz_dot_f32(int64_t K, int64_t C, const float* A, const float* v, float* out,
                         void* workspace, size_t workspace_bytes, void* stream);
int gmp_edge_outer_sum_rect_f32(int64_t K, int64_t m, int64_t n, const float* A, const float* B,
                                float* C, float* colsum_A, void* workspace,
                                size_t workspace_bytes, void* stream);
int gmp_edge_outer_sum_ex2_f32(int64_t K, int64_t m, int64_t n1, int64_t n2, const float* A,
                               int64_t lda, const float* B1, int64_t ldb1, const float* B2,
                               int64_t ldb2, float* C, int64_t ldc, float* colsum_A,
                               void* workspace, size_t workspace_bytes, void* stream);
size_t gmp_edge_outer_sum_ex_workspace_size(int64_t K, int64_t m, int64_t n);
enum {
  GMP_WGRAD_ROUTE_ZERO = 1,
  GMP_WGRAD_ROUTE_X3 = 2,
  GMP_WGRAD_ROUTE_QUAD = 3,
  GMP_WGRAD_ROUTE_SQUARE_F32 = 4,
  GMP_WGRAD_ROUTE_RECT_F32 = 5,
  GMP_WGRAD_ROUTE_LIBRARY = 6
};
int gmp_edge_outer_sum_ex_route(int64_t K, int64_t m, int64_t n, int64_t lda, int64_t ldb,
                                int act);
int gmp_edge_outer_sum_ex_f32(int64_t K, int64_t m, int64_t n, const float* A, int64_t lda,
                              const float* B, int64_t ldb, int act, const float* w, const float* b,
                              float* C, int64_t ldc, float* colsum_A, void* workspace,
                              size_t workspace_bytes, void* stream);

int gmp_edge_featurize_f32(const float* pos, const int64_t* edge_index, int64_t n_edges,
                           int num_bessel, const float* bessel_weights, float prefactor,
                           float r_max, float p_cutoff, float* vec_out, float* len_out,
                           float* sh_out, float* radial_out, void* stream);
int gmp_edge_featurize_bwd_f32(const float* pos, const int64_t* edge_index, int64_t n_edges,
                               int num_bessel, const float* bessel_weights, float prefactor,
                               float r_max, float p_cutoff, const float* g_sh,
                               const float* g_radial, float* g_vec, void* stream);
int gmp_edge_featurize_lmax_f32(const float* pos, const int64_t* edge_index, int64_t n_edges,
                                int lmax, int num_bessel, const float* bessel_weights,
                                float prefactor, float r_max, float p_cutoff, float* vec_out,
                                float* len_out, float* sh_out, float* radial_out, void* stream);
int gmp_edge_featurize_lmax_bwd_f32(const float* pos, const int64_t* edge_index,
                                    int64_t n_edges, int lmax, int num_bessel,
                                    const float* bessel_weights, float prefactor, float r_max,
                                    float p_cutoff, const float* g_sh, const float* g_radial,
                                    float* g_vec, void* stream);
size_t gmp_featurize_shift_workspace_size(int64_t n_edges);
int gmp_edge_featurize_lmax_ex_f32(const float* pos, const int64_t* edge_index, int64_t n_edges,
                                   int lmax, int num_bessel, const float* bessel_weights,
                                   float prefactor, float r_max, float p_cutoff,
                                   const float* shift, void* workspace, size_t workspace_bytes,
                                   float* vec_out, float* len_out, float* sh_out,
                                   float* radial_out, void* stream);
int gmp_edge_featurize_lmax_bwd_ex_f32(const float* pos, const int64_t* edge_index,
                                       int64_t n_edges, int lmax, int num_bessel,
                                       const float* bessel_weights, float prefactor, float r_max,
                                       float p_cutoff, const float* shift, void* workspace,
                                       size_t workspace_bytes, const float* g_sh,
                                       const float* g_radial, float* g_vec, void* stream);
int gmp_edge_featurize_gvp_f32(const float* pos, const int64_t* edge_index, int64_t n_edges,
                               int num_bessel, const float* bessel_weights, float prefactor,
                               float r_max, float p_cutoff, float* len_out, float* radial_out,
                               float* unit_out, void* stream);
int gmp_edge_featurize_gvp_bwd_f32(const float* pos, const int64_t* edge_index, int64_t n_edges,
                                   int num_bessel, const float* bessel_weights, float prefactor,
                                   float r_max, float p_cutoff, const float* g_radial,
                                   const float* g_unit, float* g_vec, void* stream);
int gmp_schnet_featurize_f32(const float* pos, const int64_t* edge_index, int64_t n_edges,
                             int num_gaussians, const float* offsets, float coeff, float cutoff,
                             float* dist_out, float* rbf_out, float* cut_out, void* stream);
// ... 406 lines not shown
```

Measured before the change: 126.3 million.

## Fuse EGNN sender-side backward reductions into one kernel writing interleaved dA|dB buffer

The edge backward kernel can now write dA with a leading dimension of 2d, so dA and dB share one [N,2d] buffer. A new send-side kernel reduces dpre1 per sender node into the dB half and, in the same pass, sums gdiff and subtracts it from dpos_recv to produce dpos. This replaces two separate segment_reduce launches and an elementwise subtract. The dh product becomes a single matmul over the concatenated buffer, and the dW1 outer sum becomes a single call followed by a transpose copy. The fused route only applies when the reduction is not split across parts and takes the per-thread path, and it adds an extra copy for the dW1 layout.

```diff
diff --git a/geometric-message-passing_amd/csrc/gmp_egnn.hip b/geometric-message-passing_amd/csrc/gmp_egnn.hip
--- a/geometric-message-passing_amd/csrc/gmp_egnn.hip
+++ b/geometric-message-passing_amd/csrc/gmp_egnn.hip
@@ -163,17 +163,19 @@
   return sV[v * D + featq(s, g)];
 }
 
-template <int D, int ACT, bool MSG_MEAN, bool HF, bool AMAX, int RC, bool POSB, bool GPOS>
+template <int D, int ACT, bool MSG_MEAN, bool HF, bool AMAX, int RC, bool POSB, bool GPOS,
+          bool WIDE = false>
 __global__ __launch_bounds__(kBwdWaves * 64, 2) void egnn_bwd_kernel(
     int64_t n_nodes, int64_t n_edges, const float* __restrict__ pos,
     const int64_t* __restrict__ rowptr, const int64_t* __restrict__ recv,
     const int64_t* __restrict__ send, gmp_egnn_params P, int64_t n_waves,
     const float* __restrict__ xsave, const float* __restrict__ rsave,
     const float* __restrict__ g_maggr, const float* __restrict__ g_paggr, float* __restrict__ dA,
-    float* __restrict__ dpos_recv, float* __restrict__ dpre1_out, float* __restrict__ gdiff_out,
-    float* __restrict__ dpre2_out, float* __restrict__ dpre3_out, float* __restrict__ partials,
-    unsigned* __restrict__ amax) {
+    float* __restrict__ dpos_recv, float* __restrict__ dpre1_out,
+    float* __restrict__ gdiff_out, float* __restrict__ dpre2_out, float* __restrict__ dpre3_out,
+    float* __restrict__ partials, unsigned* __restrict__ amax) {
   constexpr int T = Cfg<D>::T, LDW = Cfg<D>::LDW, K = VecAcc<D>::K;
+  constexpr int LDA = WIDE ? 2 * D : D;
   extern __shared__ __attribute__((aligned(16))) float smem[];
   const float* sW2t = smem;
   const float* sW3t = smem + D * LDW;
@@ -203,7 +205,7 @@
   float* cbuf = smem + smem_carry_off<D, kBwdWaves, HF>() + (wid * 4 + g) * carry_stride<D>();
   carry_clear<D>(smem + smem_carry_off<D, kBwdWaves, HF>() + wid * 4 * carry_stride<D>(), lane);
   const WaveRange wr = wave_range(rowptr, n_nodes, n_edges, n_waves, wid, kBwdWaves);
-  zero_isolated<D, GPOS>(wr, rowptr, dA, dpos_recv, lane);
+  zero_isolated<D, GPOS>(wr, rowptr, dA, dpos_recv, lane, LDA);
   const float b4 = POSB ? P.b4[0] : 0.f;
   const size_t ED = (size_t)n_edges * D;
 
@@ -382,8 +384,8 @@
     }
     {
       const int nn = max(i1 - i0 + 1, 0);
-      store_row_w<D, 0>(rows_window(dA, i0, nn, D), is_end ? (unsigned)((c.i - i0) * D * 4) : kOob,
-                        x, g);
+      store_row_w<D, 0>(WIDE ? rows_window_ld(dA, i0, nn, LDA, D) : rows_window(dA, i0, nn, D),
+                        is_end ? (unsigned)((c.i - i0) * LDA * 4) : kOob, x, g);
       if constexpr (GPOS)
         store3_w<0>(rows_window(dpos_recv, i0, nn, 3),
                     (is_end && g == 0) ? (unsigned)((c.i - i0) * 12) : kOob, gd[0], gd[1], gd[2]);
@@ -455,8 +457,9 @@
 int launch_bwd(int64_t N, int64_t E, const float* pos, const int64_t* rowptr,
                const int64_t* recv, const int64_t* send, const gmp_egnn_params& P,
                const float* xsave, int save_planes, const float* rsave, const float* gm,
-               const float* gp, float* dA, float* dpos_recv, float* dpre1, float* gdiff,
-               float* dpre2, float* dpre3, float* partials, unsigned* amax, hipStream_t s) {
+               const float* gp, float* dA, bool wide, float* dpos_recv, float* dpre1,
+               float* gdiff, float* dpre2, float* dpre3, float* partials, unsigned* amax,
+               hipStream_t s) {
   const int64_t W = n_waves_for(E, kBwdWaves);
   const bool hf = !egnn_f32();
   constexpr int NMAT = POSB ? 2 : 1;
@@ -470,7 +473,13 @@
             : egnn_bwd_kernel<D, ACT, MEAN, true, !FULL, RC, POSB, GPOS>)            \
       : (ax ? egnn_bwd_kernel<D, ACT, MEAN, false, true, RC, POSB, GPOS>             \
             : egnn_bwd_kernel<D, ACT, MEAN, false, !FULL, RC, POSB, GPOS>))
-  auto k = save_planes == 3 ? LAUNCH_BWD_K(RC0) : LAUNCH_BWD_K(1);
+#define LAUNCH_BWD_KW(RC)                                                             \
+  (hf ? egnn_bwd_kernel<D, ACT, MEAN, true, true, RC, POSB, GPOS, true>              \
+      : egnn_bwd_kernel<D, ACT, MEAN, false, true, RC, POSB, GPOS, true>)
+  if (wide && !ax) return GMP_ERR_UNSUPPORTED;
+  auto k = wide ? (save_planes == 3 ? LAUNCH_BWD_KW(RC0) : LAUNCH_BWD_KW(1))
+                : (save_planes == 3 ? LAUNCH_BWD_K(RC0) : LAUNCH_BWD_K(1));
+#undef LAUNCH_BWD_KW
 #undef LAUNCH_BWD_K
   int rc = prep_kernel(k, smem);
   if (rc) return rc;
@@ -583,15 +592,16 @@
   return n_waves_for(n_edges, kBwdWaves) / kBwdWaves;
 }
 
-int gmp_egnn_edge_bwd_ex_f32(int64_t n_nodes, int64_t n_edges, int64_t d, const float* pos,
+int gmp_egnn_edge_bwd_ld_f32(int64_t n_nodes, int64_t n_edges, int64_t d, const float* pos,
                              const int64_t* rowptr, const int64_t* recv, const int64_t* send,
                              const gmp_egnn_params* params, int act, int msg_mean,
                              const float* save_xhat, int save_planes, const float* save_rstd,
                              const float* g_m_aggr, const float* g_pos_aggr, float* dA,
-                             float* dpos_recv, float* dpre1, float* gdiff, float* dpre2,
-                             float* dpre3, float* vec_partials, uint32_t* amax, uint32_t flags,
-                             void* stream) {
+                             int64_t ld_dA, float* dpos_recv, float* dpre1, float* gdiff,
+                             float* dpre2, float* dpre3, float* vec_partials, uint32_t* amax,
+                             uint32_t flags, void* stream) {
   if (!(d == 32 || d == 64 || d == 128)) return GMP_ERR_UNSUPPORTED;
+  if (!(ld_dA == d || ld_dA == 2 * d)) return GMP_ERR_UNSUPPORTED;
   GMP_CHECK_ARG((flags & ~(uint32_t)(GMP_EGNN_NO_POS_BRANCH | GMP_EGNN_NO_POS_GRAD)) == 0);
   const bool posb = !(flags & GMP_EGNN_NO_POS_BRANCH), gpos = !(flags & GMP_EGNN_NO_POS_GRAD);
   GMP_CHECK_ARG(n_nodes >= 0 && n_edges >= 0 && (act == 0 || act == 1));
@@ -601,7 +611,7 @@
   hipStream_t s = as_stream(stream);
   int rc = GMP_OK;
   if (n_nodes > 0 && n_edges == 0) {
-    rc = hip_check(hipMemsetAsync(dA, 0, n_nodes * d * sizeof(float), s));
+    rc = hip_check(hipMemset2DAsync(dA, ld_dA * sizeof(float), 0, d * sizeof(float), n_nodes, s));
     if (!rc && gpos) rc = hip_check(hipMemsetAsync(dpos_recv, 0, n_nodes * 3 * sizeof(float), s));
   }
   if (rc) return rc;
@@ -618,8 +628,8 @@
   GMP_CHECK_ARG(aligned16(params->W2) && aligned16(params->W3));
 #define LAUNCH_BWD_V(DD, AA, MM, PB, GP)                                                        \
   launch_bwd<DD, AA, MM, PB, GP>(n_nodes, n_edges, pos, rowptr, recv, send, *params, save_xhat, \
-                                 save_planes, save_rstd, g_m_aggr, g_pos_aggr, dA, dpos_recv,   \
-                                 dpre1, gdiff, dpre2, dpre3, vec_partials, amax, s)
+                                 save_planes, save_rstd, g_m_aggr, g_pos_aggr, dA, ld_dA != d,  \
+                                 dpos_recv, dpre1, gdiff, dpre2, dpre3, vec_partials, amax, s)
 #define LAUNCH_CALL_BWD(DD, AA, MM)                                                              \
   rc = posb ? (gpos ? LAUNCH_BWD_V(DD, AA, MM, true, true) : LAUNCH_BWD_V(DD, AA, MM, true, false)) \
             : (gpos ? LAUNCH_BWD_V(DD, AA, MM, false, true)                                     \
@@ -628,6 +638,20 @@
 #undef LAUNCH_CALL_BWD
 #undef LAUNCH_BWD_V
   return rc;
+}
+
+int gmp_egnn_edge_bwd_ex_f32(int64_t n_nodes, int64_t n_edges, int64_t d, const float* pos,
+                             const int64_t* rowptr, const int64_t* recv, const int64_t* send,
+                             const gmp_egnn_params* params, int act, int msg_mean,
+                             const float* save_xhat, int save_planes, const float* save_rstd,
+                             const float* g_m_aggr, const float* g_pos_aggr, float* dA,
+                             float* dpos_recv, float* dpre1, float* gdiff, float* dpre2,
+                             float* dpre3, float* vec_partials, uint32_t* amax, uint32_t flags,
+                             void* stream) {
+  return gmp_egnn_edge_bwd_ld_f32(n_nodes, n_edges, d, pos, rowptr, recv, send, params, act,
+                                  msg_mean, save_xhat, save_planes, save_rstd, g_m_aggr,
+                                  g_pos_aggr, dA, d, dpos_recv, dpre1, gdiff, dpre2, dpre3,
+                                  vec_partials, amax, flags, stream);
 }
 
 int gmp_egnn_edge_bwd_amax_f32(int64_t n_nodes, int64_t n_edges, int64_t d, const float* pos,
diff --git a/geometric-message-passing_amd/csrc/gmp_egnn_common.h b/geometric-message-passing_amd/csrc/gmp_egnn_common.h
--- a/geometric-message-passing_amd/csrc/gmp_egnn_common.h
+++ b/geometric-message-passing_amd/csrc/gmp_egnn_common.h
@@ -225,6 +225,10 @@
 __device__ __forceinline__ rsrc_t rows_window(const float* base, int r0, int n, int ld) {
   return __builtin_amdgcn_make_buffer_rsrc(const_cast<float*>(base) + (size_t)(unsigned)r0 * ld, 0,
                                            n * ld * 4, 0x00020000);
+}
+__device__ __forceinline__ rsrc_t rows_window_ld(const float* base, int r0, int n, int ld, int w) {
+  return __builtin_amdgcn_make_buffer_rsrc(const_cast<float*>(base) + (size_t)(unsigned)r0 * ld, 0,
+                                           n > 0 ? ((n - 1) * ld + w) * 4 : 0, 0x00020000);
 }
 template <int D, int AUX>
 __device__ __forceinline__ void store_row_w(rsrc_t w, unsigned off, const f32x4 (&x)[D / 16], int g) {
@@ -754,11 +758,11 @@
 template <int D, bool R3 = true>
 __device__ __forceinline__ void zero_isolated(const WaveRange& wr, const int64_t* __restrict__ rowptr,
                                               float* __restrict__ rows, float* __restrict__ rows3,
-                                              int lane) {
+                                              int lane, int ld = D) {
   const int* rp = reinterpret_cast<const int*>(rowptr);
   for (int n = wr.n_lo + lane; n < wr.n_hi; n += 64) {
     if (rp[2 * n] == rp[2 * n + 2]) {
-      float4* r = reinterpret_cast<float4*>(rows + (size_t)n * D);
+      float4* r = reinterpret_cast<float4*>(rows + (size_t)n * ld);
 #pragma unroll
       for (int k = 0; k < D / 4; ++k) r[k] = float4{0.f, 0.f, 0.f, 0.f};
       if (R3) {
diff --git a/geometric-message-passing_amd/csrc/gmp_egnn_send.hip b/geometric-message-passing_amd/csrc/gmp_egnn_send.hip
--- /dev/null
+++ b/geometric-message-passing_amd/csrc/gmp_egnn_send.hip
@@ -0,0 +1,120 @@
+#include "gmp_common.h"
+#include "gmp_segred.h"
+
+namespace gmp {
+namespace {
+
+constexpr int kSendWaves = 4;
+
+__device__ __forceinline__ float lane_value(float x, int j) {
+  return __int_as_float(__builtin_amdgcn_readlane(__float_as_int(x), j));
+}
+
+template <int D, bool GPOS>
+__global__ __launch_bounds__(kSendWaves * 64) void egnn_send_bwd_kernel(
+    const float* __restrict__ dpre1, const float* __restrict__ gdiff,
+    const float* __restrict__ dpos_recv, const int64_t* __restrict__ perm,
+    const int64_t* __restrict__ rowptr, int64_t n_nodes, int64_t n_edges, float* __restrict__ dB,
+    int64_t ld_dB, float* __restrict__ dpos) {
+  const int lane = threadIdx.x & 63;
+  const int wid = __builtin_amdgcn_readfirstlane(threadIdx.x >> 6);
+  const int64_t seg = blockIdx.x * (int64_t)kSendWaves + wid;
+  if (seg >= n_nodes) return;
+  int64_t k0 = rowptr[seg], k1 = rowptr[seg + 1];
+  k0 = k0 < 0 ? 0 : (k0 > n_edges ? n_edges : k0);
+  k1 = k1 < k0 ? k0 : (k1 > n_edges ? n_edges : k1);
+
+  float gx = 0.f, gy = 0.f, gz = 0.f, pr = 0.f;
+  if constexpr (GPOS) {
+    if (k0 + lane < k1) {
+      const float* q = gdiff + perm[k0 + lane] * 3;
+      gx = q[0]; gy = q[1]; gz = q[2];
+    }
+    if (lane < 3) pr = dpos_recv[seg * 3 + lane];
+  }
+
+  constexpr int CPR = D / 4;
+  {
+    float acc[4];
+    int64_t arg[4];
+    wave_reduce_rows<4, GMP_REDUCE_SUM>(dpre1, D, perm, k0, k1, n_edges, lane % CPR, CPR, acc,
+                                        arg);
+    if (lane < CPR)
+      *reinterpret_cast<float4*>(dB + seg * ld_dB + lane * 4) =
+          float4{acc[0], acc[1], acc[2], acc[3]};
+  }
+
+  if constexpr (GPOS) {
+    float ax = 0.f, ay = 0.f, az = 0.f;
+    for (int64_t kb = k0; kb < k1; kb += 64) {
+      if (kb != k0) {
+        gx = gy = gz = 0.f;
+        if (kb + lane < k1) {
+          const float* q = gdiff + perm[kb + lane] * 3;
+          gx = q[0]; gy = q[1]; gz = q[2];
+        }
+      }
+      const int cnt = (int)(k1 - kb < 64 ? k1 - kb : 64);
+      for (int j = 0; j < cnt; ++j) {
+        ax += lane_value(gx, j);
+        ay += lane_value(gy, j);
+        az += lane_value(gz, j);
+      }
+    }
+    const float a = lane == 0 ? ax : (lane == 1 ? ay : az);
+    if (lane < 3) dpos[seg * 3 + lane] = pr - a;
+  }
+}
+
+bool send_route_ok(int64_t n_nodes, int64_t n_edges, int64_t d) {
+  if (!(d == 32 || d == 64 || d == 128)) return false;
+  if (n_nodes == 0) return true;
+  if (segment_split_parts(n_edges, n_nodes, GMP_REDUCE_SUM) != 1) return false;
+  return segment_thread_path(n_edges, n_nodes, 3);
+}
+
+}
+}
+
+using namespace gmp;
+
+extern "C" {
+
+int gmp_egnn_send_bwd_route(int64_t n_nodes, int64_t n_edges, int64_t d) {
+  if (n_nodes < 0 || n_edges < 0) return GMP_ERR_ARG;
+  return send_route_ok(n_nodes, n_edges, d) ? 1 : 0;
+}
+
+int gmp_egnn_send_bwd_f32(int64_t n_nodes, int64_t n_edges, int64_t d, const float* dpre1,
+                          const float* gdiff, const float* dpos_recv, const int64_t* perm,
+                          const int64_t* rowptr, float* dB, int64_t ld_dB, float* dpos,
+                          void* stream) {
+  GMP_CHECK_ARG(n_nodes >= 0 && n_edges >= 0);
+  GMP_CHECK_ARG(n_nodes < INT32_MAX && n_edges < INT32_MAX);
+  const bool gpos = dpos != nullptr;
+  if (!send_route_ok(n_nodes, n_edges, d)) return GMP_ERR_UNSUPPORTED;
+  if (n_nodes == 0) return GMP_OK;
+  GMP_CHECK_ARG(rowptr && dB && ld_dB >= d && ld_dB % 4 == 0);
+  GMP_CHECK_ARG(reinterpret_cast<uintptr_t>(dB) % 16 == 0);
+  GMP_CHECK_ARG(!gpos || dpos_recv);
+  GMP_CHECK_ARG(n_edges == 0 || (dpre1 && perm && (!gpos || gdiff)));
+  GMP_CHECK_ARG(reinterpret_cast<uintptr_t>(dpre1) % 16 == 0);
+  hipStream_t s = as_stream(stream);
+  const unsigned grid = (unsigned)ceil_div(n_nodes, kSendWaves);
+#define LAUNCH_SEND(DD)                                                                        \
+  do {                                                                                         \
+    if (gpos)                                                                                  \
+      egnn_send_bwd_kernel<DD, true><<<grid, kSendWaves * 64, 0, s>>>(                         \
+          dpre1, gdiff, dpos_recv, perm, rowptr, n_nodes, n_edges, dB, ld_dB, dpos);           \
+    else                                                                                       \
+      egnn_send_bwd_kernel<DD, false><<<grid, kSendWaves * 64, 0, s>>>(                        \
+          dpre1, gdiff, dpos_recv, perm, rowptr, n_nodes, n_edges, dB, ld_dB, dpos);           \
+  } while (0)
+  if (d == 128) LAUNCH_SEND(128);
+  else if (d == 64) LAUNCH_SEND(64);
+  else LAUNCH_SEND(32);
+#undef LAUNCH_SEND
+  return launch_status();
+}
+
+}
diff --git a/geometric-message-passing_amd/csrc/gmp_index.hip b/geometric-message-passing_amd/csrc/gmp_index.hip
--- a/geometric-message-passing_amd/csrc/gmp_index.hip
+++ b/geometric-message-passing_amd/csrc/gmp_index.hip
@@ -5,6 +5,7 @@
 #include <utility>
 
 #include "gmp_common.h"
+#include "gmp_segred.h"
 
 namespace gmp {
 
@@ -95,89 +96,6 @@
       out[e * F + c] = v;
     }
   }
-}
-
-struct RedVal {
-  float v;
-  int64_t arg;
-};
-
-template <int REDUCE>
-__device__ __forceinline__ void red_combine(float& acc, int64_t& arg, float x, int64_t xa) {
-  if (REDUCE == GMP_REDUCE_MAX) {
-    if (x > acc || (x == acc && xa < arg)) { acc = x; arg = xa; }
-  } else {
-    acc += x;
-  }
-}
-
-template <int VEC, int REDUCE>
-__device__ __forceinline__ void wave_reduce_rows(const float* __restrict__ src, int64_t F,
-                                                 const int64_t* __restrict__ perm, int64_t k_beg,
-                                                 int64_t k_end, int64_t n_items, int64_t c,
-                                                 int lpr, float (&acc)[VEC], int64_t (&arg)[VEC]) {
-  const int lane = threadIdx.x & 63;
-  const int R = 64 / lpr, sub = lane / lpr;
-#pragma unroll
-  for (int v = 0; v < VEC; ++v) {
-    acc[v] = (REDUCE == GMP_REDUCE_MAX) ? -INFINITY : 0.f;
-    arg[v] = n_items;
-  }
-  const bool active = c < F / VEC;
-  int64_t k = k_beg + sub;
-  for (; k + 3 * R < k_end; k += 4 * R) {
-    int64_t it[4];
-    float x[4][VEC];
-#pragma unroll
-    for (int u = 0; u < 4; ++u) it[u] = perm ? perm[k + u * R] : (k + u * R);
-#pragma unroll
-    for (int u = 0; u < 4; ++u) {
-      const float* p = src + it[u] * F + c * VEC;
-      if (!active) {
-#pragma unroll
-        for (int v = 0; v < VEC; ++v) x[u][v] = 0.f;
-      } else if constexpr (VEC == 4) {
-        float4 q = *reinterpret_cast<const float4*>(p);
-        x[u][0] = q.x; x[u][1] = q.y; x[u][2] = q.z; x[u][3] = q.w;
-      } else if constexpr (VEC == 2) {
-        float2 q = *reinterpret_cast<const float2*>(p);
-        x[u][0] = q.x; x[u][1] = q.y;
-      } else {
-        x[u][0] = p[0];
-      }
-    }
-#pragma unroll
-    for (int u = 0; u < 4; ++u)
-#pragma unroll
-      for (int v = 0; v < VEC; ++v) red_combine<REDUCE>(acc[v], arg[v], x[u][v], it[u]);
-  }
-  for (; k < k_end; k += R) {
-    const int64_t i = perm ? perm[k] : k;
-    if (active) {
-      const float* p = src + i * F + c * VEC;
-#pragma unroll
-      for (int v = 0; v < VEC; ++v) red_combine<REDUCE>(acc[v], arg[v], p[v], i);
-    }
-  }
-  for (int m = lpr; m < 64; m <<= 1) {
-#pragma unroll
-    for (int v = 0; v < VEC; ++v) {
-      const float ox = __shfl_xor(acc[v], m);
-      const int64_t oa = __shfl_xor(arg[v], m);
-      if (REDUCE == GMP_REDUCE_MAX) {
-        if (ox > acc[v] || (ox == acc[v] && oa < arg[v])) { acc[v] = ox; arg[v] = oa; }
-      } else {
-        const bool upper = (lane & m) != 0;
-        acc[v] = upper ? ox + acc[v] : acc[v] + ox;
-      }
-    }
-  }
-}
-
-__device__ __forceinline__ int lanes_per_row(int64_t cpr) {
-  int l = 1;
-  while (l < cpr && l < 64) l <<= 1;
-  return l;
 }
 
 template <int VEC, int REDUCE>
@@ -427,12 +345,7 @@
 }
 
 static int64_t split_parts(int64_t n_items, int64_t n_seg, int reduce) {
-  if (reduce == GMP_REDUCE_MAX || n_seg <= 0) return 1;
-  const int64_t avg = n_items / n_seg;
-  int64_t S = avg < 2048 ? 1 : ceil_div(avg, 1024);
-  if (n_seg < 2048 && n_items >= 16384)
-    S = std::max<int64_t>(S, std::min<int64_t>(ceil_div(2048, n_seg), 64));
-  return S > 4096 ? 4096 : S;
+  return segment_split_parts(n_items, n_seg, reduce);
 }
 
 size_t gmp_segment_reduce_workspace_size(int64_t n_items, int64_t n_seg, int64_t F, int reduce) {
@@ -476,7 +389,7 @@
       src, n_items, F, perm, rowptr, n_seg, out, argmax)
 #define LAUNCH_SEG_DISPATCH(RED)                                                               \
   do {                                                                                      \
-    if (F < 4 && n_items < 64 * n_seg)                                                      \
+    if (segment_thread_path(n_items, n_seg, F))                                             \
       segment_reduce_thread<RED><<<grid_for(n_seg * F, 256), 256, 0, s>>>(                 \
           src, n_items, F, perm, rowptr, n_seg, out, argmax);                               \
     else if (vec == 4) LAUNCH_SEG_LAUNCH(4, RED);                                              \
diff --git a/geometric-message-passing_amd/csrc/gmp_segred.h b/geometric-message-passing_amd/csrc/gmp_segred.h
--- /dev/null
+++ b/geometric-message-passing_amd/csrc/gmp_segred.h
@@ -0,0 +1,99 @@
+#pragma once
+
+#include <algorithm>
+
+#include "gmp_common.h"
+
+namespace gmp {
+
+template <int REDUCE>
+__device__ __forceinline__ void red_combine(float& acc, int64_t& arg, float x, int64_t xa) {
+  if (REDUCE == GMP_REDUCE_MAX) {
+    if (x > acc || (x == acc && xa < arg)) { acc = x; arg = xa; }
+  } else {
+    acc += x;
+  }
+}
+
+template <int VEC, int REDUCE>
+__device__ __forceinline__ void wave_reduce_rows(const float* __restrict__ src, int64_t F,
+                                                 const int64_t* __restrict__ perm, int64_t k_beg,
+                                                 int64_t k_end, int64_t n_items, int64_t c,
+                                                 int lpr, float (&acc)[VEC], int64_t (&arg)[VEC]) {
+  const int lane = threadIdx.x & 63;
+  const int R = 64 / lpr, sub = lane / lpr;
+#pragma unroll
+  for (int v = 0; v < VEC; ++v) {
+    acc[v] = (REDUCE == GMP_REDUCE_MAX) ? -INFINITY : 0.f;
+    arg[v] = n_items;
+  }
+  const bool active = c < F / VEC;
+  int64_t k = k_beg + sub;
+  for (; k + 3 * R < k_end; k += 4 * R) {
+    int64_t it[4];
+    float x[4][VEC];
+#pragma unroll
+    for (int u = 0; u < 4; ++u) it[u] = perm ? perm[k + u * R] : (k + u * R);
+#pragma unroll
+    for (int u = 0; u < 4; ++u) {
+      const float* p = src + it[u] * F + c * VEC;
+      if (!active) {
+#pragma unroll
+        for (int v = 0; v < VEC; ++v) x[u][v] = 0.f;
+      } else if constexpr (VEC == 4) {
+        float4 q = *reinterpret_cast<const float4*>(p);
+        x[u][0] = q.x; x[u][1] = q.y; x[u][2] = q.z; x[u][3] = q.w;
+      } else if constexpr (VEC == 2) {
+        float2 q = *reinterpret_cast<const float2*>(p);
+        x[u][0] = q.x; x[u][1] = q.y;
+      } else {
+        x[u][0] = p[0];
+      }
+    }
+#pragma unroll
+    for (int u = 0; u < 4; ++u)
+#pragma unroll
+      for (int v = 0; v < VEC; ++v) red_combine<REDUCE>(acc[v], arg[v], x[u][v], it[u]);
+  }
+  for (; k < k_end; k += R) {
+    const int64_t i = perm ? perm[k] : k;
+    if (active) {
+      const float* p = src + i * F + c * VEC;
+#pragma unroll
+      for (int v = 0; v < VEC; ++v) red_combine<REDUCE>(acc[v], arg[v], p[v], i);
+    }
+  }
+  for (int m = lpr; m < 64; m <<= 1) {
+#pragma unroll
+    for (int v = 0; v < VEC; ++v) {
+      const float ox = __shfl_xor(acc[v], m);
+      const int64_t oa = __shfl_xor(arg[v], m);
+      if (REDUCE == GMP_REDUCE_MAX) {
+        if (ox > acc[v] || (ox == acc[v] && oa < arg[v])) { acc[v] = ox; arg[v] = oa; }
+      } else {
+        const bool upper = (lane & m) != 0;
+        acc[v] = upper ? ox + acc[v] : acc[v] + ox;
+      }
+    }
+  }
+}
+
+__host__ __device__ __forceinline__ int lanes_per_row(int64_t cpr) {
+  int l = 1;
+  while (l < cpr && l < 64) l <<= 1;
+  return l;
+}
+
+inline int64_t segment_split_parts(int64_t n_items, int64_t n_seg, int reduce) {
+  if (reduce == GMP_REDUCE_MAX || n_seg <= 0) return 1;
+  const int64_t avg = n_items / n_seg;
+  int64_t S = avg < 2048 ? 1 : ceil_div(avg, 1024);
+  if (n_seg < 2048 && n_items >= 16384)
+    S = std::max<int64_t>(S, std::min<int64_t>(ceil_div(2048, n_seg), 64));
+  return S > 4096 ? 4096 : S;
+}
+inline bool segment_thread_path(int64_t n_items, int64_t n_seg, int64_t F) {
+  return F < 4 && n_items < 64 * n_seg;
+}
+
+}
diff --git a/geometric-message-passing_amd/csrc/torch/gmp_torch.cpp b/geometric-message-passing_amd/csrc/torch/gmp_torch.cpp
--- a/geometric-message-passing_amd/csrc/torch/gmp_torch.cpp
+++ b/geometric-message-passing_amd/csrc/torch/gmp_torch.cpp
@@ -298,7 +298,7 @@
     const Tensor& pos, const Tensor& rowptr, const Tensor& recv, const Tensor& send,
     const std::vector<Tensor>& params, int64_t act, bool msg_mean, const Tensor& xhat,
     const Tensor& rstd, const Tensor& g_m, const Tensor& g_p, const optional<Tensor>& amax,
-    bool pos_branch, bool pos_grad) {
+    bool pos_branch, bool pos_grad, bool wide_dA) {
   OpGuard g(pos, "egnn_edge_bwd");
   egnn_graph_checks(pos, rowptr, recv, send);
   f32(xhat, "xhat");
@@ -318,21 +318,53 @@
     TORCH_CHECK(amax->numel() >= 2, "gmp.egnn_edge_bwd: amax has 2 words");
   }
   auto o = fopt(pos);
-  Tensor dA = at::empty({N, d}, o), dpr = at::empty({pos_grad ? N : 0, 3}, o);
+  const int64_t ld = wide_dA ? 2 * d : d;
+  Tensor dA = at::empty({N, ld}, o), dpr = at::empty({pos_grad ? N : 0, 3}, o);
   Tensor dp1 = at::empty({E, d}, o), gd = at::empty({pos_grad ? E : 0, 3}, o);
   Tensor dp2 = at::empty({E, d}, o), dp3 = at::empty({pos_branch ? E : 0, d}, o);
   Tensor part = at::empty({gmp_egnn_edge_bwd_partials_rows(E, d), 8 * d + 1}, o);
-  check_rc(gmp_egnn_edge_bwd_ex_f32(
+  check_rc(gmp_egnn_edge_bwd_ld_f32(
                N, E, d, fp(pos), ip(rowptr), ip(recv), ip(send), &P, (int)act, msg_mean,
                E > 0 ? fp(xhat) : nullptr, (int)xhat.size(0), fp(rstd), fp(g_m),
-               pos_branch ? fp(g_p) : nullptr, fp(dA), pos_grad ? fp(dpr) : nullptr, fp(dp1),
+               pos_branch ? fp(g_p) : nullptr, fp(dA), ld, pos_grad ? fp(dpr) : nullptr, fp(dp1),
                pos_grad ? fp(gd) : nullptr, fp(dp2), pos_branch ? fp(dp3) : nullptr, fp(part),
                amax.has_value() ? reinterpret_cast<uint32_t*>(amax->data_ptr<int32_t>())
                                 : nullptr,
                (pos_branch ? 0u : GMP_EGNN_NO_POS_BRANCH) | (pos_grad ? 0u : GMP_EGNN_NO_POS_GRAD),
                cur_stream()),
-           "gmp_egnn_edge_bwd_ex_f32");
+           "gmp_egnn_edge_bwd_ld_f32");
   return {dA, dpr, dp1, gd, dp2, dp3, part};
+}
+
+Tensor egnn_send_bwd(const Tensor& dpre1, const optional<Tensor>& gdiff,
+                     const optional<Tensor>& dpos_recv, const Tensor& perm, const Tensor& rowptr,
+                     Tensor dAB) {
+  OpGuard g(dpre1, "egnn_send_bwd");
+  f32(dpre1, "dpre1");
+  i64(perm, "perm");
+  i64(rowptr, "rowptr");
+  f32(dAB, "dAB");
+  TORCH_CHECK(dpre1.dim() == 2 && dAB.dim() == 2 && dAB.size(1) == 2 * dpre1.size(1),
+              "gmp.egnn_send_bwd: dpre1 (E, d), dAB (N, 2d)");
+  const int64_t E = dpre1.size(0), d = dpre1.size(1), N = dAB.size(0);
+  numel(perm, E, "perm");
+  numel(rowptr, N + 1, "rowptr");
+  const bool gpos = gdiff.has_value() && gdiff->defined();
+  TORCH_CHECK(gpos == (dpos_recv.has_value() && dpos_recv->defined()),
+              "gmp.egnn_send_bwd: gdiff and dpos_recv come together");
+  if (gpos) {
+    f32(*gdiff, "gdiff");
+    f32(*dpos_recv, "dpos_recv");
+    shape(*gdiff, {E, 3}, "gdiff");
+    shape(*dpos_recv, {N, 3}, "dpos_recv");
+  }
+  Tensor dpos = at::empty({gpos ? N : 0, 3}, fopt(dpre1));
+  if (N == 0) return dpos;
+  check_rc(gmp_egnn_send_bwd_f32(N, E, d, fp(dpre1), cfp(gdiff), cfp(dpos_recv), ip(perm),
+                                 ip(rowptr), fp(dAB) + d, 2 * d, gpos ? fp(dpos) : nullptr,
+                                 cur_stream()),
+           "gmp_egnn_send_bwd_f32");
+  return dpos;
 }
 
 Tensor cfconv_aggregate(const Tensor& x, const Tensor& xidx, const Tensor& w, const Tensor& perm,
@@ -2057,13 +2089,18 @@
 std::tuple<Tensor, Tensor, Tensor, Tensor, Tensor, Tensor, Tensor> egnn_edge_bwd(
     const Tensor& pos, const Tensor&, const Tensor& recv, const Tensor&,
     const std::vector<Tensor>&, int64_t, bool, const Tensor& xhat, const Tensor&, const Tensor&,
-    const Tensor&, const optional<Tensor>&, bool pos_branch, bool pos_grad) {
+    const Tensor&, const optional<Tensor>&, bool pos_branch, bool pos_grad, bool wide_dA) {
   const int64_t N = pos.size(0), E = recv.numel(), d = xhat.size(2);
   auto o = pos.options();
-  return {at::empty({N, d}, o), at::empty({pos_grad ? N : 0, 3}, o), at::empty({E, d}, o),
-          at::empty({pos_grad ? E : 0, 3}, o), at::empty({E, d}, o),
+  return {at::empty({N, wide_dA ? 2 * d : d}, o), at::empty({pos_grad ? N : 0, 3}, o),
+          at::empty({E, d}, o), at::empty({pos_grad ? E : 0, 3}, o), at::empty({E, d}, o),
           at::empty({pos_branch ? E : 0, d}, o),
           at::empty({gmp_egnn_edge_bwd_partials_rows(E, d), 8 * d + 1}, o)};
+}
+Tensor egnn_send_bwd(const Tensor& dpre1, const optional<Tensor>& gdiff, const optional<Tensor>&,
+                     const Tensor&, const Tensor&, Tensor dAB) {
+  const bool gpos = gdiff.has_value() && gdiff->defined();
+  return at::empty({gpos ? dAB.size(0) : 0, 3}, dpre1.options());
 }
 Tensor cfconv_aggregate(const Tensor& x, const Tensor&, const Tensor&, const Tensor&,
                         const Tensor&, int64_t n_seg, const optional<Tensor>&) {
@@ -2408,9 +2445,11 @@
         "Tensor xhat, Tensor rstd)");
   m.def("egnn_edge_bwd(Tensor pos, Tensor rowptr, Tensor recv, Tensor send, Tensor[] params, "
         "int act, bool msg_mean, Tensor xhat, Tensor rstd, Tensor g_m_aggr, Tensor g_pos_aggr, "
-        "Tensor(a!)? amax=None, bool pos_branch=True, bool pos_grad=True) -> (Tensor dA, "
-        "Tensor dpos_recv, "
+        "Tensor(a!)? amax=None, bool pos_branch=True, bool pos_grad=True, bool wide_dA=False) "
+        "-> (Tensor dA, Tensor dpos_recv, "
         "Tensor dpre1, Tensor gdiff, Tensor dpre2, Tensor dpre3, Tensor partials)");
+  m.def("egnn_send_bwd(Tensor dpre1, Tensor? gdiff, Tensor? dpos_recv, Tensor perm, "
+        "Tensor rowptr, Tensor(a!) dAB) -> Tensor");
   m.def("cfconv_aggregate(Tensor x, Tensor xidx, Tensor w, Tensor perm, Tensor rowptr, "
         "int n_seg, Tensor? escale=None) -> Tensor");
   m.def("cfconv_wgrad(Tensor g, Tensor gidx, Tensor x, Tensor xidx, Tensor? escale=None) -> "
@@ -2564,6 +2603,7 @@
   m.impl("egnn_node_fwd", ns egnn_node_fwd);                              \
   m.impl("egnn_node_image", ns egnn_node_image);                          \
   m.impl("egnn_edge_bwd", ns egnn_edge_bwd);                              \
+  m.impl("egnn_send_bwd", ns egnn_send_bwd);                              \
   m.impl("cfconv_aggregate", ns cfconv_aggregate);                        \
   m.impl("cfconv_wgrad", ns cfconv_wgrad);                                \
   m.impl("ssp_fwd", ns ssp_fwd);                                          \
diff --git a/geometric-message-passing_amd/gmp_amd/_lib.py b/geometric-message-passing_amd/gmp_amd/_lib.py
--- a/geometric-message-passing_amd/gmp_amd/_lib.py
+++ b/geometric-message-passing_amd/gmp_amd/_lib.py
@@ -208,6 +208,12 @@
     "gmp_egnn_edge_bwd_ex_f32": (c_int, [c_i64, c_i64, c_i64, c_vp, c_vp, c_vp, c_vp,
                                          ctypes.POINTER(GmpEgnnParams), c_int, c_int, c_vp, c_int]
                                  + [c_vp] * 11 + [ctypes.c_uint32, c_vp]),
+    "gmp_egnn_edge_bwd_ld_f32": (c_int, [c_i64, c_i64, c_i64, c_vp, c_vp, c_vp, c_vp,
+                                         ctypes.POINTER(GmpEgnnParams), c_int, c_int, c_vp, c_int]
+                                 + [c_vp] * 4 + [c_i64] + [c_vp] * 7 + [ctypes.c_uint32, c_vp]),
+    "gmp_egnn_send_bwd_route": (c_int, [c_i64, c_i64, c_i64]),
+    "gmp_egnn_send_bwd_f32": (c_int, [c_i64, c_i64, c_i64, c_vp, c_vp, c_vp, c_vp, c_vp, c_vp,
+                                      c_i64, c_vp, c_vp]),
     "gmp_ssp_bwd2_f32": (c_int, [c_vp, c_vp, c_vp, c_i64, c_vp, c_vp, c_vp]),
     "gmp_schnet_featurize_bwd2_f32": (c_int, [c_vp, c_i64, c_vp, c_i64, c_int, c_vp, c_f32, c_f32]
                                       + [c_vp] * 9),
diff --git a/geometric-message-passing_amd/gmp_amd/ops.py b/geometric-message-passing_amd/gmp_amd/ops.py
--- a/geometric-message-passing_amd/gmp_amd/ops.py
+++ b/geometric-message-passing_amd/gmp_amd/ops.py
@@ -122,7 +122,16 @@
     return _lib.torch_ops().gather_rows(src2d, index)
 
 
-def segment_reduce(src2d, csr, reduce="sum", use_perm=True):
+def egnn_send_bwd(dpre1, csr, dAB, gdiff=None, dpos_recv=None):
+    _need_cuda(dpre1, dAB)
+    dpos = _lib.torch_ops().egnn_send_bwd(dpre1, gdiff, dpos_recv, csr.perm, csr.rowptr, dAB)
+    return dpos if gdiff is not None else None
+
+
+def segment_reduce(src2d, csr, reduce="sum", use_perm=True, egnn_send=None):
+    if egnn_send is not None:
+        dpre1, dAB, dpos_recv = egnn_send
+        return egnn_send_bwd(dpre1, csr, dAB, src2d, dpos_recv), None
     src2d = _f32c(src2d)
     _need_cuda(src2d)
     out, argmax = _lib.torch_ops().segment_reduce(src2d, csr.perm if use_perm else None,
@@ -627,6 +636,14 @@
         self.send = self.recv_csr.payload_sorted
         self.rowptr = self.recv_csr.rowptr
         self.send_csr = CSR(self.send, self.num_nodes)
+        self._send_routes = {}
+
+    def send_bwd_fused(self, d):
+        ok = self._send_routes.get(d)
+        if ok is None:
+            ok = self._send_routes[d] = _lib.load().gmp_egnn_send_bwd_route(
+                self.num_nodes, self.num_edges, d) == 1
+        return ok
 
     def check_range(self):
         self.recv_csr.check_range()
@@ -659,6 +676,12 @@
 EGNN_XHAT_PLANES = 2
 
 EGNN_SKIP_DEAD_POS = True
+
+EGNN_SEND_BWD_FUSED = True
+
+
+def _egnn_dh(dAB, W1, d):
+    return _mm_wt(dAB, torch.cat([W1[:, :d].t(), W1[:, d:2 * d].t()], 1))
 
 
 class EgnnMessageFn(torch.autograd.Function):
@@ -705,21 +728,33 @@
         else:
             g_p = torch.zeros((N, 3), **f) if g_p is None else _f32c(g_p)
         amax = torch.zeros(2, dtype=torch.int32, device=dev)
+        fused = (EGNN_SEND_BWD_FUSED and not compiling()
+                 and getattr(graph, "send_csr", None) is not None
+                 and graph.send_bwd_fused(d))
         with _timed("egnn_edge_bwd"):
             dA, dpos_recv, dpre1, gdiff, dpre2, dpre3, partials = \
                 _lib.torch_ops().egnn_edge_bwd(pos, graph.rowptr, graph.recv, graph.send,
                                                list(params), _lib.ACT[ctx.act],
                                                bool(ctx.msg_mean), xhat, rstd, g_m, g_p, amax,
-                                               pos_branch, pos_grad)
+                                               pos_branch, pos_grad, fused)
         xh1, xh2 = xhat[0], xhat[1]
-        dB, _ = segment_reduce(dpre1, graph.send_csr, "sum")
-        W1t = W1[:, :2 * d].t().contiguous()
-        dh = _mm_wt(dA, W1t[:d])
-        dh.addmm_(dB, W1t[d:].t())
         dpos = None
-        if pos_grad:
-            dpos_send, _ = segment_reduce(gdiff, graph.send_csr, "sum")
-            dpos = dpos_recv - dpos_send
+        if fused:
+            dAB = dA
+            if pos_grad:
+                dpos, _ = segment_reduce(gdiff, graph.send_csr, "sum",
+                                         egnn_send=(dpre1, dAB, dpos_recv))
+            else:
+                egnn_send_bwd(dpre1, graph.send_csr, dAB)
+            dh = _egnn_dh(dAB, W1, d)
+        else:
+            dB, _ = segment_reduce(dpre1, graph.send_csr, "sum")
+            W1t = W1[:, :2 * d].t().contiguous()
+            dh = _mm_wt(dA, W1t[:d])
+            dh.addmm_(dB, W1t[d:].t())
+            if pos_grad:
+                dpos_send, _ = segment_reduce(gdiff, graph.send_csr, "sum")
+                dpos = dpos_recv - dpos_send
 
         (_, b1, ln1w, ln1b, W2, b2, ln2w, ln2b, W3, b3, ln3w, ln3b, w4, b4) = params
         dW2, db2 = edge_outer_sum_act(dpre2, xh1, ln1w, ln1b, ctx.act, amax[0:1])
@@ -727,11 +762,18 @@
             dW3, db3 = edge_outer_sum_act(dpre3, xh2, ln2w, ln2b, ctx.act, amax[1:2])
         else:
             dW3, db3 = torch.zeros((d, d), **f), torch.zeros(d, **f)
-        with side_work(h, dA, dB, partials) as sw:
+        with side_work(h, dA, None if fused else dB, partials) as sw:
             dW1 = torch.empty((d, 2 * d + 1), **f)
-            db1 = torch.empty(d, **f)
-            outer_sum_into(dA, h, dW1[:, :d], db1)
-            outer_sum_into(dB, h, dW1[:, d:2 * d])
+            if fused:
+                dW1ab = torch.empty((2 * d, d), **f)
+                cs = torch.empty(2 * d, **f)
+                outer_sum_into(dAB, h, dW1ab, cs)
+                dW1[:, :2 * d].unflatten(1, (2, d)).copy_(dW1ab.view(2, d, d).transpose(0, 1))
+                db1 = cs[:d].clone()
+            else:
+                db1 = torch.empty(d, **f)
+                outer_sum_into(dA, h, dW1[:, :d], db1)
+                outer_sum_into(dB, h, dW1[:, d:2 * d])
             v = partials.sum(0)
             dln1w, dln1b, dln2w, dln2b, dln3w, dln3b, dw4, dw1d = v[:8 * d].view(8, d).unbind(0)
             dW1[:, 2 * d].copy_(dw1d)
diff --git a/include/gmp.h b/include/gmp.h
--- a/include/gmp.h
+++ b/include/gmp.h
@@ -124,6 +124,20 @@
                              float* dpos_recv, float* dpre1, float* gdiff, float* dpre2,
                              float* dpre3, float* vec_partials, uint32_t* amax, uint32_t flags,
                              void* stream);
+int gmp_egnn_edge_bwd_ld_f32(int64_t n_nodes, int64_t n_edges, int64_t d, const float* pos,
+                             const int64_t* rowptr, const int64_t* recv, const int64_t* send,
+                             const gmp_egnn_params* params, int act, int msg_mean,
+                             const float* save_xhat, int save_planes, const float* save_rstd,
+                             const float* g_m_aggr, const float* g_pos_aggr, float* dA,
+                             int64_t ld_dA, float* dpos_recv, float* dpre1, float* gdiff,
+                             float* dpre2, float* dpre3, float* vec_partials, uint32_t* amax,
+                             uint32_t flags, void* stream);
+
+int gmp_egnn_send_bwd_route(int64_t n_nodes, int64_t n_edges, int64_t d);
+int gmp_egnn_send_bwd_f32(int64_t n_nodes, int64_t n_edges, int64_t d, const float* dpre1,
+                          const float* gdiff, const float* dpos_recv, const int64_t* perm,
+                          const int64_t* rowptr, float* dB, int64_t ld_dB, float* dpos,
+                          void* stream);
 
 int gmp_wgrad_set_f32_mfma(int on);
 size_t gmp_edge_outer_sum_workspace_size(int64_t K, int64_t d);
```

Result: faster. 128.0 million (median of 5 runs) (+1.3%).
